# jorgeMFS/VCFX

Measured on AMD Instinct MI355X. Metric: variant-records/sec (and GB/s vs HBM roofline), 427K var × 2504 samp, higher is better.
Workload: dtype u8; 1 GPU; VCFX_allele_freq_calc -i (file path) on a device-resident 427409 x 2504 VCF shard per GPU: the walk (line ends + allele counts + rows composed in LDS) + the rows in file order; records_per_gpu=427409, samples=2504, bytes_per_gpu=4297544426, parallelism=record-sharded x1

## Files before the change

### include/vcfx_gpu.h

```cpp
#ifndef VCFX_GPU_H
#define VCFX_GPU_H
#include <stddef.h>
#include <stdint.h>

#ifdef __cplusplus
extern "C" {
#endif

typedef struct vcfxg_ctx vcfxg_ctx;

enum vcfxg_status {
    VCFXG_OK = 0,
    VCFXG_E_NODEV = -1,
    VCFXG_E_HIP = -2,
    VCFXG_E_ARG = -3,
    VCFXG_E_NOMEM = -4,
    VCFXG_E_STATE = -5,
    VCFXG_E_CAP = -6,
    VCFXG_E_DATA = -7
};

enum vcfxg_mode { VCFXG_MODE_FILE = 0, VCFXG_MODE_STDIN = 1 };

enum vcfxg_line_status {
    VCFXG_LINE_SKIP = 0,
    VCFXG_LINE_ROW = 1,
    VCFXG_LINE_DROP = 2,
    VCFXG_LINE_WARN = 3,
    VCFXG_LINE_HEADER = 4,
    VCFXG_LINE_RECHECK = 5
};

typedef struct {
    uint64_t n_lines;
    uint64_t rows;
    uint64_t data_lines;
    uint64_t warn_lines;
    uint64_t text_bytes;
    uint64_t general_records;
} vcfxg_summary;

const char *vcfxg_version(void);
int vcfxg_device_count(int *n);
int vcfxg_open(int device, vcfxg_ctx **out);
void vcfxg_close(vcfxg_ctx *ctx);
const char *vcfxg_last_error(const vcfxg_ctx *ctx);
void *vcfxg_stream(vcfxg_ctx *ctx);
int vcfxg_set_profiling(vcfxg_ctx *ctx, int enable);
int vcfxg_set_profiling_only(vcfxg_ctx *ctx, const char *kernel);
int vcfxg_kernel_ms(vcfxg_ctx *ctx, const char *kernel, float *ms);
int vcfxg_kernel_stats(vcfxg_ctx *ctx, const char *kernel, double *total_ms, uint64_t *launches);
int vcfxg_reset_kernel_stats(vcfxg_ctx *ctx);

int vcfxg_load_host(vcfxg_ctx *ctx, const char *host, size_t n);
int vcfxg_ingest_begin(vcfxg_ctx *ctx, size_t size_hint);
int vcfxg_ingest(vcfxg_ctx *ctx, const char *host, size_t n, int is_final_chunk);
int vcfxg_ingest_wait(vcfxg_ctx *ctx, size_t upto);
typedef struct {
    uint64_t src_off;
    uint32_t src_len;
    uint32_t out_len;
} vcfxg_bgzf_member;
int vcfxg_ingest_bgzf(vcfxg_ctx *ctx, const void *comp, size_t comp_n, const vcfxg_bgzf_member *members,
                      size_t n_members, const char *head, size_t head_n, uint64_t *bad_member);
int vcfxg_bgzf_stage(vcfxg_ctx *ctx, const void *host, size_t n, size_t offset, size_t comp_total);
int vcfxg_bgzf_inflate(vcfxg_ctx *ctx, const vcfxg_bgzf_member *members, size_t count);
uint64_t vcfxg_bgzf_handed_over(const vcfxg_ctx *ctx);
int vcfxg_host_alloc(vcfxg_ctx *ctx, size_t n, void **out);
void vcfxg_host_free(vcfxg_ctx *ctx, void *p);
int vcfxg_input_fetch(vcfxg_ctx *ctx, uint64_t offset, size_t n, void *host);
const void *vcfxg_input_device_ptr(vcfxg_ctx *ctx);

int vcfxg_index(vcfxg_ctx *ctx, size_t data_start, uint64_t *n_lines);
int vcfxg_line_ends(vcfxg_ctx *ctx, uint64_t first, uint64_t count, uint64_t *out);

int vcfxg_allele_freq(vcfxg_ctx *ctx, int mode, vcfxg_summary *out);
int vcfxg_allele_freq_region(vcfxg_ctx *ctx, size_t data_start, int mode, vcfxg_summary *out);
int vcfxg_genotype_query(vcfxg_ctx *ctx, const char *query, size_t qlen, int strict, int strip_cr,
                         vcfxg_summary *out);

typedef struct {
    int target;
    int op;
    int numeric;
    double value;
    const char *key;
    size_t key_len;
    const char *str;
    size_t str_len;
} vcfxg_criterion;

int vcfxg_record_filter(vcfxg_ctx *ctx, const vcfxg_criterion *crit, int n, int and_logic, vcfxg_summary *out);
#define VCFXG_RF_KEEP_CR 1
int vcfxg_record_filter_ex(vcfxg_ctx *ctx, const vcfxg_criterion *crit, int n, int and_logic, int flags,
                           vcfxg_summary *out);

int vcfxg_filter_query(vcfxg_ctx *ctx, const vcfxg_criterion *crit, int n, int and_logic, const char *query,
                       size_t qlen, int strict, vcfxg_summary *out);

int vcfxg_record_filter_region(vcfxg_ctx *ctx, size_t data_start, const vcfxg_criterion *crit, int n, int and_logic,
                               vcfxg_summary *out);
int vcfxg_genotype_query_region(vcfxg_ctx *ctx, size_t data_start, const char *query, size_t qlen, int strict,
                                int strip_cr, vcfxg_summary *out);
int vcfxg_filter_query_region(vcfxg_ctx *ctx, size_t data_start, const vcfxg_criterion *crit, int n, int and_logic,
                              const char *query, size_t qlen, int strict, vcfxg_summary *out);

int vcfxg_nonref_filter(vcfxg_ctx *ctx, int mode, vcfxg_summary *out);
int vcfxg_nonref_filter_region(vcfxg_ctx *ctx, size_t data_start, int mode, vcfxg_summary *out);

typedef struct {
    uint64_t text_offset;
    int32_t hom_ref, het, hom_alt;
    int32_t reserved;
} vcfxg_hwe_recheck;
int vcfxg_hwe_region(vcfxg_ctx *ctx, size_t data_start, int mode, vcfxg_summary *out);
int vcfxg_hwe_rechecks(vcfxg_ctx *ctx, vcfxg_hwe_recheck *out, uint64_t cap, uint64_t *n);

int vcfxg_dosage_region(vcfxg_ctx *ctx, size_t data_start, int mode, vcfxg_summary *out);

#define VCFXG_LINE_MISSING 6
int vcfxg_missing_region(vcfxg_ctx *ctx, size_t data_start, int mode, vcfxg_summary *out);

typedef struct {
    const uint32_t *sample;
    uint64_t m;
    const char *names;
    const uint64_t *name_off;
    int seq;
    int kind;
} vcfxg_ac_params;
int vcfxg_allele_counter(vcfxg_ctx *ctx, uint64_t first_line, uint64_t last_line, const vcfxg_ac_params *params,
                         vcfxg_summary *out);

typedef struct {
    uint32_t n_samples;
    const char *names;
    const uint64_t *name_off;
    int freq_mode;
    int skip_boundary;
    int count_boundary_as_used;
} vcfxg_ib_params;
int vcfxg_inbreeding_region(vcfxg_ctx *ctx, size_t data_start, int mode, const vcfxg_ib_params *params,
                            vcfxg_summary *out);
int vcfxg_inbreeding_samples(vcfxg_ctx *ctx, double *sum_exp, uint64_t *obs_het, uint64_t *used);

#define VCFXG_SX_EMPTY 0
#define VCFXG_SX_ROW 1
#define VCFXG_SX_SHORT 3
#define VCFXG_SX_HEADER 4
#define VCFXG_SX_NO_SAMPLES 5
#define VCFXG_SX_PRE 6
#define VCFXG_SX_CHROM 7
typedef struct {
    const uint32_t *cols;
    uint64_t m;
    int mode;
    int seen_chrom;
} vcfxg_sx_params;
int vcfxg_sample_extract(vcfxg_ctx *ctx, uint64_t first_line, uint64_t last_line, const vcfxg_sx_params *params,
                         vcfxg_summary *out);

#define VCFXG_MS_EMPTY 0
#define VCFXG_MS_COPY 1
#define VCFXG_MS_SPLIT 2
#define VCFXG_MS_HEADER 4
#define VCFXG_MS_INFO 0
#define VCFXG_MS_FORMAT 1
#define VCFXG_MS_NUM_OTHER 0
#define VCFXG_MS_NUM_A 1
#define VCFXG_MS_NUM_R 2
#define VCFXG_MS_NUM_G 3
#define VCFXG_MS_KEYS_LDS 32
#define VCFXG_MS_TABLE_LDS 16384
typedef struct {
    const char *id;
    uint32_t id_len;
    uint8_t section;
    uint8_t number;
} vcfxg_ms_entry;
typedef struct {
    const vcfxg_ms_entry *table;
    uint64_t n_entries;
    int mode;
} vcfxg_ms_params;
int vcfxg_multiallelic_split(vcfxg_ctx *ctx, uint64_t first_line, uint64_t last_line, const vcfxg_ms_params *params,
                             vcfxg_summary *out);
int vcfxg_ms_line_ranges(vcfxg_ctx *ctx, uint64_t first, uint64_t count, uint64_t *off);

#define VCFXG_FA_EMPTY 0
#define VCFXG_FA_COLUMN 1
#define VCFXG_FA_SKIPPED 3
#define VCFXG_FA_HEADER 4
#define VCFXG_FA_CHROM 7
#define VCFXG_FA_LINE 60
#define VCFXG_FA_TILE_SAMPLES 64
#define VCFXG_FA_TILE_COLUMNS 240
#define VCFXG_FA_TABLE 16
typedef struct {
    int mode;
    uint32_t n_samples;
    uint64_t first_col;
    uint64_t total_cols;
    const uint64_t *row_off;
    const uint64_t *skip;
} vcfxg_fa_params;
int vcfxg_fasta_scan(vcfxg_ctx *ctx, uint64_t first_line, uint64_t last_line, int mode, uint32_t n_samples,
                     vcfxg_summary *out);
int vcfxg_fasta_status(vcfxg_ctx *ctx, uint64_t first, uint64_t count, uint8_t *status, uint64_t *col);
int vcfxg_fasta_begin(vcfxg_ctx *ctx, uint64_t text_bytes);
int vcfxg_fasta(vcfxg_ctx *ctx, uint64_t first_line, uint64_t last_line, const vcfxg_fa_params *params,
                vcfxg_summary *out);

#define VCFXG_CC_CONCORDANT 1
#define VCFXG_CC_DISCORDANT 2
#define VCFXG_CC_NO_GENOTYPES 3
typedef struct {
    uint32_t n_samples;
    const uint32_t *mult;
    uint64_t n_mult;
    uint64_t threads;
} vcfxg_cc_params;
int vcfxg_concordance_region(vcfxg_ctx *ctx, size_t data_start, int mode, const vcfxg_cc_params *params,
                             vcfxg_summary *out);
int vcfxg_concordance_totals(const vcfxg_ctx *ctx, uint64_t totals[4]);
int vcfxg_chrom_lines(vcfxg_ctx *ctx, size_t data_start, uint64_t *starts, uint64_t cap, uint64_t *n);

#define VCFXG_DD_EMPTY 0
#define VCFXG_DD_KEPT 1
#define VCFXG_DD_DUP 2
#define VCFXG_DD_SHORT 3
#define VCFXG_DD_HEADER 4
#define VCFXG_DD_WINDOW 64
typedef struct {
    uint32_t hash_bits;
} vcfxg_dd_params;
int vcfxg_dedup(vcfxg_ctx *ctx, int mode, const vcfxg_dd_params *params, vcfxg_summary *out);
int vcfxg_dedup_status(vcfxg_ctx *ctx, uint64_t first, uint64_t count, uint8_t *status);
int vcfxg_dedup_counts(const vcfxg_ctx *ctx, uint64_t counts[6]);

#define VCFXG_SRT_EMPTY 0
#define VCFXG_SRT_KEPT 1
#define VCFXG_SRT_PRE 2
#define VCFXG_SRT_BAD 3
#define VCFXG_SRT_HEADER 4
#define VCFXG_SRT_WINDOW 64
typedef struct {
    int natural;
} vcfxg_srt_params;
int vcfxg_sort(vcfxg_ctx *ctx, int mode, const vcfxg_srt_params *params, vcfxg_summary *out);
int vcfxg_sort_status(vcfxg_ctx *ctx, uint64_t first, uint64_t count, uint8_t *status);
int vcfxg_sort_counts(const vcfxg_ctx *ctx, uint64_t counts[6]);
int vcfxg_sort_order(vcfxg_ctx *ctx, uint64_t first, uint64_t count, uint32_t *lines);
int vcfxg_sort_text(vcfxg_ctx *ctx, uint64_t first_out_line, uint64_t *lines_taken, uint64_t *bytes);

#define VCFXG_DF_EMPTY 0
#define VCFXG_DF_COMMON 1
#define VCFXG_DF_UNIQUE 2
#define VCFXG_DF_SKIPPED 3
#define VCFXG_DF_HEADER 4
#define VCFXG_DF_REPEAT 5
#define VCFXG_DF_WINDOW 64
#define VCFXG_DF_PATH_HASH 0
#define VCFXG_DF_PATH_BOUNDS 1
#define VCFXG_DF_PATH_WALK 2
typedef struct {
    uint64_t second_start;
    int assume_sorted;
    int natural;
    uint32_t hash_bits;
} vcfxg_df_params;
int vcfxg_diff(vcfxg_ctx *ctx, const vcfxg_df_params *params, vcfxg_summary *out);
int vcfxg_diff_status(vcfxg_ctx *ctx, uint64_t first, uint64_t count, uint8_t *status);
int vcfxg_diff_counts(const vcfxg_ctx *ctx, uint64_t counts[8]);
int vcfxg_diff_text(vcfxg_ctx *ctx, int side, uint64_t first_out, uint64_t *taken, uint64_t *bytes);

#define VCFXG_MG_EMPTY 0
#define VCFXG_MG_KEPT 1
#define VCFXG_MG_BAD 2
#define VCFXG_MG_HEADER 3
#define VCFXG_MG_DROPPED 4
#define VCFXG_MG_WINDOW 64
#define VCFXG_MG_PATH_SORT 0
#define VCFXG_MG_PATH_WALK 1
typedef struct {
    const uint64_t *file_start;
    uint32_t n_files;
    int assume_sorted;
    int natural;
} vcfxg_mg_params;
int vcfxg_merge(vcfxg_ctx *ctx, const vcfxg_mg_params *params, vcfxg_summary *out);
int vcfxg_merge_status(vcfxg_ctx *ctx, uint64_t first, uint64_t count, uint8_t *status);
int vcfxg_merge_counts(const vcfxg_ctx *ctx, uint64_t counts[8]);
int vcfxg_merge_files(vcfxg_ctx *ctx, uint64_t *first_line, uint64_t *bad);
int vcfxg_merge_order(vcfxg_ctx *ctx, uint64_t first, uint64_t count, uint32_t *lines);
int vcfxg_merge_text(vcfxg_ctx *ctx, uint64_t first_out_line, uint64_t *lines_taken, uint64_t *bytes);

int vcfxg_haplotype_phaser(vcfxg_ctx *ctx, size_t data_start, int mode, double threshold, uint32_t n_samples_hint,
                           vcfxg_summary *out);
int vcfxg_phaser_variants(vcfxg_ctx *ctx, uint8_t *flags, double *r2, uint64_t *entry_offsets);

int vcfxg_variant_count(vcfxg_ctx *ctx, int strip_cr, vcfxg_summary *out);

int vcfxg_ld_prepare(vcfxg_ctx *ctx, int n_samples, int id_dot_to_pos, const char *region_chrom, size_t region_len,
                     int has_region, int region_start, int region_end, int parse_mode, uint64_t *n_variants);
int vcfxg_ld_prepare_region(vcfxg_ctx *ctx, size_t data_start, int n_samples, int id_dot_to_pos,
                            const char *region_chrom, size_t region_len, int has_region, int region_start,
                            int region_end, int parse_mode, uint64_t *n_variants);
int vcfxg_ld_prefixes(vcfxg_ctx *ctx, char *text, size_t cap, uint64_t *offsets);
int vcfxg_ld_matrix(vcfxg_ctx *ctx, int gate, int printf4, uint64_t *cell_bytes);
int vcfxg_ld_stream_chunk(vcfxg_ctx *ctx, uint64_t j0, uint64_t j1, uint64_t window, double threshold, int max_dist,
                          uint64_t *n_pairs, uint64_t *text_bytes);
int vcfxg_ld_fetch_pairs(vcfxg_ctx *ctx, uint64_t first, uint64_t count, uint32_t *vi, uint32_t *vj, double *r2);
int vcfxg_selftest_mfma_i8(vcfxg_ctx *ctx, int *mismatches);
int vcfxg_selftest_mfma_fp4(vcfxg_ctx *ctx, int *mismatches);

int vcfxg_shard_cuts(const char *data, size_t n, size_t lo, int world, uint64_t *cuts);

typedef struct vcfxg_comm vcfxg_comm;
int vcfxg_comm_init(vcfxg_ctx *const *ctxs, int n, vcfxg_comm **out);
int vcfxg_comm_allreduce_u64(vcfxg_comm *comm, int rank, uint64_t *vals, size_t count);
int vcfxg_comm_uses_rccl(const vcfxg_comm *comm);
int vcfxg_comm_rccl_stats(vcfxg_comm *comm, uint64_t *calls, uint64_t *mismatches);
void vcfxg_comm_destroy(vcfxg_comm *comm);

int vcfxg_count_byte(vcfxg_ctx *ctx, uint64_t from, int byte, uint64_t *count);
const char *vcfxg_last_schedule(const vcfxg_ctx *ctx);
int vcfxg_last_af_depth(const vcfxg_ctx *ctx, int *rolling);

int vcfxg_fetch_text(vcfxg_ctx *ctx, char *host, size_t cap);
int vcfxg_fetch_text_range(vcfxg_ctx *ctx, uint64_t offset, size_t n, void *host);
int vcfxg_fetch_lines(vcfxg_ctx *ctx, uint64_t first, uint64_t count, int32_t *alt, int32_t *total,
                      uint8_t *status);

#ifdef __cplusplus
}
#endif
#endif
```

### vcfx_amd/csrc/gpu/vcfxg_af_walk.hip

```cpp
#include <algorithm>
#include <type_traits>

#include "vcfxg_af_walk_kernel.h"

namespace vcfxg {

#ifndef VCFXG_COMPACT_SUB
#define VCFXG_COMPACT_SUB 4
#endif
constexpr int kCompactSub = VCFXG_COMPACT_SUB, kCompactLanes = kWave / kCompactSub;
__global__ __launch_bounds__(256) void k_walk_compact(int64_t n_walkers, uint64_t cap_w,
                                                      const uint64_t *__restrict__ offs,
                                                      const uint32_t *__restrict__ wgt,
                                                      const uint64_t *__restrict__ le_b,
                                                      const int32_t *__restrict__ alt_b,
                                                      const int32_t *__restrict__ tot_b,
                                                      const int32_t *__restrict__ aux_b,
                                                      const uint32_t *__restrict__ rowpre_b,
                                                      const uint8_t *__restrict__ status_b,
                                                      const LineMeta *__restrict__ meta_b, uint64_t *line_end,
                                                      int32_t *alt, int32_t *tot, int32_t *aux, uint32_t *rowpre,
                                                      uint8_t *status, LineMeta *meta, uint64_t *n_lines,
                                                      unsigned long long *counters, const uint64_t *__restrict__ bpre) {
    __shared__ uint32_t red[256 / kWave];
    uint32_t g = 0;
    const int64_t nwaves = (int64_t)gridDim.x * (256 / kWave);
    const int sub = lane() / kCompactLanes, sl = lane() % kCompactLanes;
    for (int64_t w0 = ((int64_t)blockIdx.x * (256 / kWave) + threadIdx.x / kWave) * kCompactSub; w0 < n_walkers;
         w0 += nwaves * kCompactSub) {
        const int64_t w = w0 + sub;
        if (w >= n_walkers) continue;
        const uint64_t d0 = offs[w] + (bpre ? bpre[w / kWalkerScanBlock] : 0),
                       cnt = offs[w + 1] + (bpre ? bpre[(w + 1) / kWalkerScanBlock] : 0) - d0, s0 = (uint64_t)w * cap_w;
        g += sl == 0 ? (wgt[w] & 0xFFFFu) : 0u;
        for (uint64_t i = sl; i < cnt; i += kCompactLanes) {
            const uint64_t sl = s0 + i, d = d0 + i;
            line_end[d] = le_b[sl];
            alt[d] = alt_b[sl];
            tot[d] = tot_b[sl];
            if (aux_b) aux[d] = aux_b[sl];
            rowpre[d] = rowpre_b[sl];
            status[d] = status_b[sl];
            meta[d] = meta_b[sl];
        }
    }
    g = wave_sum(g);
    if (lane() == 0) red[threadIdx.x / kWave] = g;
    __syncthreads();
    if (threadIdx.x == 0) {
        uint32_t t = 0;
        for (int k = 0; k < 256 / kWave; k++) t += red[k];
        if (t) {
            atomicAdd(&counters[0], (unsigned long long)t);
            atomicAdd(&counters[1], (unsigned long long)t);
        }
        if (blockIdx.x == 0) *n_lines = offs[n_walkers] + (bpre ? bpre[n_walkers / kWalkerScanBlock] : 0);
    }
}

int64_t af_walkers(int64_t lo, int64_t hi, int64_t chunk) { return hi > lo ? (hi - lo + chunk - 1) / chunk : 0; }

hipError_t launch_af_walk(const char *buf, int64_t lo, int64_t hi, int64_t chunk, int mode, int64_t span0,
                          uint64_t cap_w, uint64_t *le_b, int32_t *alt_b, int32_t *tot_b, uint32_t *rowpre_b,
                          uint8_t *status_b, void *meta_b, uint64_t *wcount, uint32_t *wgt, unsigned *overflow,
                          hipStream_t s, int32_t *hwe_aux_b, const WalkTail *tail, bool dose, bool gt_first_walk,
                          bool dose_head, int depth, bool roll) {
    const WalkTail t = tail ? *tail : WalkTail{};
    const int64_t nw = af_walkers(lo, hi, chunk);
    if (!nw) return hipErrorInvalidValue;
    const bool af_gt_only = !gt_first_walk && !dose && !hwe_aux_b;
    if (roll ? !(af_gt_only && af_depth_compiled(depth)) : depth != kWalkUnroll) return hipErrorInvalidValue;
    const unsigned grid = (unsigned)((nw + kWalkWaves - 1) / kWalkWaves);
    if (gt_first_walk)
        hipLaunchKernelGGL(HIP_KERNEL_NAME(k_af_walk<AfOp, true>), dim3(grid), dim3(kWalkThreads), 0, s, buf, lo, hi,
                           chunk, nw, mode, span0, cap_w, le_b, alt_b, tot_b, nullptr, rowpre_b, status_b,
                           static_cast<LineMeta *>(meta_b), wcount, wgt, overflow, t);
    else if (dose && dose_head)
        hipLaunchKernelGGL(k_af_walk<DoseHeadOp>, dim3(grid), dim3(kWalkThreads), 0, s, buf, lo, hi, chunk, nw, mode,
                           span0, cap_w, le_b, alt_b, tot_b, nullptr, rowpre_b, status_b, static_cast<LineMeta *>(meta_b),
                           wcount, wgt, overflow, t);
    else if (dose)
        hipLaunchKernelGGL(k_af_walk<DoseWalkOp>, dim3(grid), dim3(kWalkThreads), 0, s, buf, lo, hi, chunk, nw, mode,
                           span0, cap_w, le_b, alt_b, tot_b, nullptr, rowpre_b, status_b, static_cast<LineMeta *>(meta_b),
                           wcount, wgt, overflow, t);
    else if (hwe_aux_b)
        hipLaunchKernelGGL(k_af_walk<HweOp>, dim3(grid), dim3(kWalkThreads), 0, s, buf, lo, hi, chunk, nw, mode, span0,
                           cap_w, le_b, alt_b, tot_b, hwe_aux_b, rowpre_b, status_b, static_cast<LineMeta *>(meta_b),
                           wcount, wgt, overflow, t);
    else {
        auto go = [&](auto kernel) {
            hipLaunchKernelGGL(kernel, dim3(grid), dim3(kWalkThreads), 0, s, buf, lo, hi, chunk, nw, mode, span0, cap_w,
                               le_b, alt_b, tot_b, nullptr, rowpre_b, status_b, static_cast<LineMeta *>(meta_b), wcount,
                               wgt, overflow, t);
        };
        if (!roll) go(k_af_walk<AfOp>);
        else if (depth == 6) go(k_af_walk<AfOp, false, 6, true>);
        else if (depth == 8) go(k_af_walk<AfOp, false, 8, true>);
        else if (depth == 10) go(k_af_walk<AfOp, false, 10, true>);
        else go(k_af_walk<AfOp, false, 12, true>);
    }
    return hipGetLastError();
}

hipError_t launch_walk_compact(int64_t n_walkers, uint64_t cap_w, const uint64_t *offs, const uint32_t *wgt,
                               const uint64_t *le_b, const int32_t *alt_b, const int32_t *tot_b,
                               const uint32_t *rowpre_b, const uint8_t *status_b, const void *meta_b,
                               uint64_t *line_end, int32_t *alt, int32_t *tot, uint32_t *rowpre, uint8_t *status,
                               void *meta, uint64_t *n_lines, unsigned long long *counters, hipStream_t s,
                               const int32_t *aux_b, int32_t *aux, const uint64_t *bpre) {
    const int64_t blocks = std::min<int64_t>((n_walkers + 256 / kWave - 1) / (256 / kWave), 512);
    hipLaunchKernelGGL(k_walk_compact, dim3((unsigned)std::max<int64_t>(blocks, 1)), dim3(256), 0, s, n_walkers, cap_w,
                       offs, wgt, le_b, alt_b, tot_b, aux_b, rowpre_b, status_b, static_cast<const LineMeta *>(meta_b),
                       line_end, alt, tot, aux, rowpre, status, static_cast<LineMeta *>(meta), n_lines, counters, bpre);
    return hipGetLastError();
}

}
```

### vcfx_amd/csrc/gpu/vcfxg_af_walk_kernel.h

```cpp
#pragma once
#include <algorithm>
#include <type_traits>

#include "vcfxg_device.h"
#include "vcfxg_gt.h"
#include "vcfxg_kernels.h"
#include "vcfxg_walk.h"

namespace vcfxg {

#ifndef VCFXG_WALK_UNROLL
#define VCFXG_WALK_UNROLL 6
#endif
constexpr int kWalkUnroll = VCFXG_WALK_UNROLL;
static_assert(kWalkUnroll == kAfDepthDefault, "launch_af_walk's default depth is the batch walks' unroll");
static_assert(kAfWaveStep == kWaveStep, "the host plan's wave-step");
#ifndef VCFXG_HWE_UNROLL
#define VCFXG_HWE_UNROLL 5
#endif
constexpr int kHweUnroll = VCFXG_HWE_UNROLL;
#ifndef VCFXG_CC_UNROLL
#define VCFXG_CC_UNROLL 4
#endif
constexpr int kCcUnroll = VCFXG_CC_UNROLL;
#ifndef VCFXG_GF_FLAGS
#define VCFXG_GF_FLAGS 1
#endif
constexpr bool kGfFlags = VCFXG_GF_FLAGS != 0;
#ifndef VCFXG_GF_UNROLL
#define VCFXG_GF_UNROLL 4
#endif
constexpr int kGfUnroll = VCFXG_GF_UNROLL;
#ifndef VCFXG_AF_XREC
#define VCFXG_AF_XREC 0
#endif
#ifndef VCFXG_AF_EXPT
#define VCFXG_AF_EXPT 0
#endif
#ifndef VCFXG_AF_EARLY
#define VCFXG_AF_EARLY 0
#endif
#define VCFXG_STR2(x) #x
#define VCFXG_STR(x) VCFXG_STR2(x)

template <class Op>
struct WalkRed;
template <>
struct WalkRed<AfOp> {
    static constexpr bool kAux = false;
    __device__ static AfOp make(const char *buf, int64_t ae) { return AfOp{buf, ae, 0}; }
    __device__ static void out(const AfOp &op, uint32_t &a, uint32_t &b, uint32_t &) {
        a = op.alt;
        b = op.tot;
    }
};
template <>
struct WalkRed<HweOp> {
    static constexpr bool kAux = true;
    __device__ static HweOp make(const char *buf, int64_t ae) { return HweOp{buf, ae}; }
    __device__ static void out(const HweOp &op, uint32_t &a, uint32_t &b, uint32_t &c) {
        a = op.c0;
        b = op.c1;
        c = op.c2;
    }
};

template <>
struct WalkRed<CcOp> {
    static constexpr bool kAux = false;
    __device__ static CcOp make(const char *, int64_t) { return CcOp{}; }
    __device__ static void out(const CcOp &op, uint32_t &a, uint32_t &b, uint32_t &) {
        a = op.N;
        b = op.U;
    }
};

template <>
struct WalkRed<DoseWalkOp> {
    static constexpr bool kAux = false;
    __device__ static DoseWalkOp make(const char *buf, int64_t ae) { return DoseWalkOp{buf, ae}; }
    __device__ static void out(const DoseWalkOp &op, uint32_t &a, uint32_t &b, uint32_t &) {
        a = op.ns;
        b = op.na;
    }
};

template <>
struct WalkRed<DoseHeadOp> : WalkRed<DoseWalkOp> {
    __device__ static DoseHeadOp make(const char *buf, int64_t ae) { return DoseHeadOp{{buf, ae}}; }
};

#ifndef VCFXG_AF_MINW
#define VCFXG_AF_MINW 5
#endif
#ifndef VCFXG_AF_DEEP_MINW
#define VCFXG_AF_DEEP_MINW 4
#endif
constexpr int af_walk_waves(bool gf, int depth) { return gf ? 4 : depth >= 10 ? VCFXG_AF_DEEP_MINW : VCFXG_AF_MINW; }
template <class Op, bool kGF = false, int kDepth = kWalkUnroll, bool kRoll = false>
__global__ __launch_bounds__(kWalkThreads)
#ifdef VCFXG_WALK_MAXW
__attribute__((amdgpu_waves_per_eu(1, VCFXG_WALK_MAXW)))
#else
__attribute__((amdgpu_waves_per_eu(af_walk_waves(kGF, kDepth))))
#endif
void k_af_walk(const char *__restrict__ buf, int64_t lo, int64_t hi, int64_t chunk, int64_t n_walkers, int mode,
               int64_t span0, uint64_t cap_w, uint64_t *__restrict__ le_o, int32_t *__restrict__ alt_o,
               int32_t *__restrict__ tot_o, int32_t *__restrict__ aux_o, uint32_t *__restrict__ rowpre_o,
               uint8_t *__restrict__ status_o, LineMeta *__restrict__ meta_o, uint64_t *__restrict__ wcount,
               uint32_t *__restrict__ wgt, unsigned *overflow, WalkTail tail) {
    typedef WalkRed<Op> R;
    constexpr bool kCc = std::is_same<Op, CcOp>::value;
    static_assert((kDepth == kWalkUnroll && !kRoll) || (std::is_same<Op, AfOp>::value && !kGF),
                  "k_af_walk: a depth of its own for the AF GT-only walk alone");
    static_assert((kDepth == kWalkUnroll && !kRoll) || !(VCFXG_AF_XREC || VCFXG_AF_EARLY),
                  "k_af_walk: the carried / early loads are batch-path experiments at kWalkUnroll");
    __shared__ uint4 win[kWalkWaves][2][kWave];
    constexpr bool kStageLds = std::is_same<Op, AfOp>::value;
    constexpr uint32_t kStgCap = kStageLds ? 2048u : 16u;
    __shared__ __attribute__((aligned(16))) char stg[kStageLds ? kWalkWaves : 1][kStgCap];
    const int wv = threadIdx.x / kWave;
    const int64_t wk = uniform64((int64_t)walk_block() * kWalkWaves + wv);
    if (wk >= n_walkers) return;
    const int strip_cr = mode == 0 ? 1 : 0;
    const int64_t cs = lo + wk * chunk;
    const int64_t ce = std::min<int64_t>(cs + chunk, hi);
    int64_t L, ce2;
    walker_lines(buf, lo, hi, cs, ce, L, ce2, chunk);
    const int64_t L0 = L;
    uint64_t wtext = 0;
    int64_t span = span0;
    uint8_t cr_prev = 0;
    uint64_t n = 0;
    uint32_t ngt = 0, ngf = 0;
    bool dirty = false;
    const uint64_t base = (uint64_t)wk * cap_w;
    uint64_t r_le = 0, r_S = 0;
    uint32_t r_alt = 0, r_tot = 0, r_aux = 0, r_pre = 0, r_k = 0;
    uint32_t r_h = 0;
    auto flush = [&](uint64_t first, uint32_t cnt) {
        if ((uint32_t)lane() < cnt) {
            const uint64_t o = base + first + lane();
            const uint8_t kind = (uint8_t)r_k;
            LineMeta m{};
            m.kind = kind;
            m.cr = (uint8_t)(r_k >> 16);
            m.pad = (R::kAux || kCc || std::is_same<Op, DoseHeadOp>::value) ? (uint8_t)r_h : 0;
            if (kind == kMetaGt) {
                m.S = r_S;
                m.rowpre = r_pre;
                m.sep = (uint8_t)(r_k >> 8);
            }
            le_o[o] = r_le;
            alt_o[o] = (int32_t)r_alt;
            tot_o[o] = (int32_t)r_tot;
            if (R::kAux) aux_o[o] = (int32_t)r_aux;
            rowpre_o[o] = kind == kMetaGt ? r_pre : 0u;
            status_o[o] = (uint8_t)(r_k >> 24);
            meta_o[o] = m;
        }
    };
    constexpr bool kXrec = VCFXG_AF_XREC && std::is_same<Op, AfOp>::value && !kGF;
    uint4 xv[kXrec ? kWalkUnroll : 1];
    int64_t xvb = -1;
    int cur = 0;
    int64_t A = L & ~(int64_t)15;
    if (L < ce2) prefetch_window(buf, A, hi, win[wv][cur]);
    constexpr bool kEarly = VCFXG_AF_EARLY && std::is_same<Op, AfOp>::value && !kGF && !kXrec;
    uint4 ev[kEarly ? kWalkUnroll : 1];
    const int64_t hlast = (hi - 1) & ~(int64_t)15;
    while (L < ce2) {
        if (n >= cap_w) {
            if (lane() == 0) atomicOr(overflow, 1u);
            break;
        }
        if constexpr (kEarly) {
#pragma unroll
            for (int u = 0; u < kWalkUnroll; u++) {
                const int64_t g = A + u * kWaveStep + kBlockBytes * lane();
                ev[u] = load16(buf, g < hi ? g : hlast);
            }
        }
        int64_t eA = kEarly ? A : -1;
        const int Lr = (int)(L - A);
        const uint4 *cw = win[wv][cur];
        int hr, N1r, r3 = 0, r4 = 0, r7 = 0, r8 = 0;
        uint32_t ntab, first, hflags = 0;
        auto take = [&](const int(&rt)[9], bool comma) {
            r4 = rt[4];
            r7 = rt[7];
            r8 = rt[8];
            if (R::kAux) {
                const bool empty = rt[0] == Lr || rt[1] == rt[0] + 1 || r4 == rt[3] + 1;
                hflags = (comma ? kHweAltComma : 0u) | (empty ? kHweEmptyField : 0u);
            }
            if (kCc) {
                r3 = rt[3];
                hflags = rt[0] == Lr ? kCcEmptyChrom : 0u;
            }
        };
        uint32_t w4 = 0;
        bool long_head = false;
        {
            if constexpr (kEarly) asm volatile("s_waitcnt vmcnt(" VCFXG_STR(VCFXG_WALK_UNROLL) ")" ::: "memory");
            else asm volatile("s_waitcnt vmcnt(0)" ::: "memory");
            w4 = reinterpret_cast<const uint32_t *>(cw)[lane()];
            hr = (int)std::min<int64_t>(hi - A, kWin);
            const uint32_t rg = range4(Lr, hr);
            N1r = first_match<4>(zero_bytes(w4 ^ kRepNl) & rg);
            int rt[9] = {};
            ntab = first_tabs<4>(zero_bytes(w4 ^ kRepTab) & rg, N1r >= 0 ? N1r : hr, rt);
            first = dword_byte(w4, Lr);
            if (ntab >= 9) take(rt, R::kAux && __ballot((zero_bytes(w4 ^ 0x2C2C2C2Cu) & range4(rt[3] + 1, rt[4])) != 0u));
        }
        if (N1r < 0 && ntab < 9 && first != '#' && hr == kWin) {
            prefetch_window(buf, A, hi, win[wv][cur], kWaveStep);
            long_head = true;
            const uint4 W = read_window(cw);
            const int b = 16 * lane();
            hr = (int)std::min<int64_t>(hi - A, kWaveStep);
            N1r = first_match<16>(eq_mask16(W, kRepNl) & range16(b, Lr, hr));
            int rt[9] = {};
            ntab = first_tabs<16>(eq_mask16(W, kRepTab) & range16(b, Lr, hr), N1r >= 0 ? N1r : hr, rt);
            if (ntab >= 9) take(rt, R::kAux && __ballot((eq_mask16(W, 0x2C2C2C2Cu) & range16(b, rt[3] + 1, rt[4])) != 0u));
        }
        auto wbyte = [&](int o) { return long_head ? slot_byte(cw, o) : dword_byte(w4, o); };
        const int64_t wend = A + hr;
        int64_t t4 = -1, t8 = -1;
        bool gt_head = false, gt_only = false;
        if (ntab >= 9 && first != '#') {
            t4 = A + r4;
            t8 = A + r8;
            if (r8 - r7 >= 3 && wbyte(r7 + 1) == 'G' && wbyte(r7 + 2) == 'T') {
                gt_only = r8 - r7 == 3;
                gt_head = gt_only || wbyte(r7 + 3) == ':';
            }
        }
        uint32_t cc_max = 0;
        if constexpr (kCc) {
            const int as = r3 + 1;
            if (gt_head && r4 > as && wbyte(as) != '.') {
                cc_max = 1;
                if (r4 - as > 1) {
                    const uint32_t cm = long_head ? eq_mask16(cw[lane()], 0x2C2C2C2Cu) & range16(16 * lane(), as, r4)
                                                  : zero_bytes(w4 ^ 0x2C2C2C2Cu) & range4(as, r4);
                    cc_max += wave_sum32((uint32_t)__popc(cm));
                }
            }
        }
        int64_t E;
        uint8_t cr = 0;
        bool predicted = false;
        const bool gf = kGF && N1r < 0 && gt_head && !gt_only;
        if (N1r >= 0) {
            E = A + N1r;
            cr = strip_cr && E > L && wbyte(N1r - 1) == '\r';
        } else if (gf) {
            E = hi;
        } else if (gt_only && span > 0 && t8 + 1 + span <= hi) {
            E = t8 + 1 + span;
            cr = cr_prev;
            predicted = true;
        } else {
            E = scan_nl(buf, wend, hi);
            cr = strip_cr && E > L && __builtin_amdgcn_readfirstlane(byte_at(buf, E - 1)) == '\r';
        }
        const uint32_t sep_w = gt_head && t8 + 2 < wend ? wbyte((int)(t8 + 2 - A)) : 0u;
        const int nxt = cur ^ 1;
        int64_t An = std::max<int64_t>(E - 1, 0) & ~(int64_t)15;
        bool pending = true;
        auto pre = [&]() {
            prefetch_window(buf, An, hi, win[wv][nxt]);
            pending = false;
        };
        uint8_t st = 0, kind = 0, sep = 0;
        uint32_t alt = 0, tot = 0, aux = 0, rowpre = 0;
        int64_t S = 0;
        bool ok = false;
        bool skip = std::is_same<Op, DoseHeadOp>::value && predicted;
        int64_t xuse = xvb;
        xvb = -1;
        auto sweep = [&]() {
            if constexpr (kGF) {
              if (gf) {
                S = t8 + 1;
                Op op = R::make(buf, hi);
                int64_t Eo = hi;
                uint8_t cro = 0;
                auto pre_e = [&](int64_t e) {
                    An = std::max<int64_t>(e - 1, 0) & ~(int64_t)15;
                    pre();
                };
                if constexpr (std::is_same<Op, AfOp>::value && kGfFlags)
                    ok = gt_first_af<kGfUnroll>(buf, S, hi, strip_cr, op, pre_e, Eo, cro);
                else
                    ok = gt_first<kWalkUnroll>(buf, S, hi, strip_cr, op, pre_e, Eo, cro);
                E = Eo;
                cr = cro;
                const int64_t ae = E - cr;
                kind = t8 < ae ? kMetaGt : kMetaFull;
                ok = ok && kind == kMetaGt;
                if (kind == kMetaGt) {
                    rowpre = (uint32_t)(t4 - L + 1);
                    sep = t8 + 2 >= ae ? 0
                          : t8 + 2 < wend ? (uint8_t)sep_w
                                          : (uint8_t)__builtin_amdgcn_readfirstlane(byte_at(buf, t8 + 2));
                    R::out(op, alt, tot, aux);
                }
                return;
              }
            }
            const int64_t ae = E - cr;
            if (ae <= L) kind = kMetaEmpty;
            else if (first == '#') kind = kMetaHeader;
            else if (gt_head && t8 < ae) kind = kMetaGt;
            else kind = kMetaFull;
            ok = false;
            if (kind == kMetaGt) {
                S = t8 + 1;
                rowpre = (uint32_t)(t4 - L + 1);
                sep = t8 + 2 >= ae ? 0
                      : t8 + 2 < wend ? (uint8_t)sep_w
                                      : (uint8_t)__builtin_amdgcn_readfirstlane(byte_at(buf, t8 + 2));
                Op op = R::make(buf, ae);
                if constexpr (kCc) op.max_allele = cc_max;
                if constexpr (kXrec) {
                    const int64_t use = xuse >= 0 && xuse <= S ? xuse : -1;
                    xuse = -1;
                    const int64_t nb = E + 1 < ce2 ? (E + 1) & ~(int64_t)15 : -1;
                    int64_t vbo;
                    ok = af_fixed_x<kWalkUnroll>(buf, S, ae, hi, op, sep, pre, xv, use, nb, vbo);
                    xvb = vbo;
                } else if constexpr (kEarly) {
                    const bool mine = eA >= 0 && eA <= S;
                    ok = af_fixed<kWalkUnroll>(buf, S, ae, op, sep, pre, mine ? ev : nullptr, mine ? eA : -1);
                    eA = -1;
                } else if constexpr (std::is_same<Op, AfOp>::value)
                    ok = af_fixed < kGF ? kGfUnroll : kDepth, kRoll > (buf, S, ae, op, sep, pre);
                else if constexpr (std::is_same<Op, DoseHeadOp>::value) {
                    if (skip) {
                        ok = (sep == '/' || sep == '|') && ae - S >= 3 && ((ae - S + 1) & 3) == 0;
                        op.ns = ok ? (uint32_t)((ae - S + 1) >> 2) : 0u;
                        op.na = 0;
                    } else {
                        ok = gt_fast<kWalkUnroll>(buf, S, ae, op, sep, pre);
                    }
                } else ok = gt_fast < std::is_same<Op, HweOp>::value ? kHweUnroll : kCc ? kCcUnroll : kWalkUnroll > (buf, S, ae, op, sep, pre);
                R::out(op, alt, tot, aux);
            }
        };
        sweep();
        if (pending) pre();
        if (predicted) {
            const uint4 *nw = win[wv][nxt];
            asm volatile("s_waitcnt vmcnt(0)" ::: "memory");
            const uint32_t be = slot_byte(nw, (int)(E - An)), be1 = slot_byte(nw, (int)(E - 1 - An));
            const bool endok = (E < hi ? be == '\n' : true) && ((strip_cr && be1 == '\r') == (cr != 0));
            if (!(ok && endok)) {
                const int64_t Et = scan_nl(buf, wend, hi);
                if (Et != E || !endok) {
                    skip = false;
                    E = Et;
                    cr = strip_cr && E > L && __builtin_amdgcn_readfirstlane(byte_at(buf, E - 1)) == '\r';
                    An = std::max<int64_t>(E - 1, 0) & ~(int64_t)15;
                    pending = true;
                    sweep();
                    if (pending) pre();
                }
            }
        }
        if constexpr (std::is_same<Op, DoseHeadOp>::value)
            if (skip && kind == kMetaGt) hflags |= kWalkUnswept;
        if (kind == kMetaGt) {
            if (ok) {
                st = 1;
                span = E - S;
                cr_prev = cr;
            } else {
                st = kAfPending;
            }
        }
        if ((uint32_t)lane() == (uint32_t)(n & 63)) {
            r_le = (uint64_t)E;
            r_S = (uint64_t)S;
            r_alt = alt;
            r_tot = tot;
            r_aux = aux;
            r_h = hflags;
            r_pre = rowpre;
            r_k = (uint32_t)kind | ((uint32_t)sep << 8) | ((uint32_t)cr << 16) | ((uint32_t)st << 24);
        }
        if constexpr (std::is_same<Op, AfOp>::value) {
            if (tail.stage && !(VCFXG_AF_EXPT & 1)) {
                if (kind == kMetaGt && ok && wtext + rowpre + 7u <= std::min<uint32_t>(tail.stage_cap, kStgCap)) {
                    uint32_t flo = 0x30303030u, fhi = 0x0A3030u;
                    if (!(VCFXG_AF_EXPT & 2)) af_freq_text(mode, (int32_t)alt, (int32_t)tot, flo, fhi);
                    auto *dst = reinterpret_cast<__attribute__((address_space(3))) char *>(
                                    reinterpret_cast<__attribute__((address_space(3))) char *>(
                                        (__attribute__((address_space(3))) void *)stg[kStageLds ? wv : 0])) +
                                wtext;
                    const unsigned char *src = reinterpret_cast<const unsigned char *>(cw) + (L - A);
                    for (uint32_t j0 = 0; j0 < rowpre + 7u; j0 += kWave) {
                        const uint32_t j = j0 + (uint32_t)lane();
                        if (j < rowpre) dst[j] = (char)src[j];
                        else if (j < rowpre + 7u) {
                            const uint32_t q = j - rowpre;
                            dst[j] = (char)((q < 4u ? flo >> (8u * q) : fhi >> (8u * (q - 4u))) & 0xFFu);
                        }
                    }
                } else if (kind == kMetaGt || kind == kMetaFull) {
                    dirty = true;
                }
            }
        }
        ngt += kind == kMetaGt ? 1u : 0u;
        if constexpr (kGF) ngf += gf && kind == kMetaGt && ok ? 1u : 0u;
        if (tail.wtext) {
            if (kind == kMetaGt) wtext += (uint64_t)rowpre + 7u;
            if (kind == kMetaFull || (kind == kMetaGt && !ok)) {
                if (lane() == 0) {
                    const unsigned long long e = atomicAdd(tail.cx_n, 1ull);
                    if (e < tail.cx_cap) tail.cx_list[e] = base + n;
                }
            }
        }
        n++;
        if ((n & 63) == 0) flush(n - 64, 64);
        L = E + 1;
        A = An;
        cur = nxt;
    }
// ... 25 lines not shown
```

### vcfx_amd/csrc/gpu/vcfxg_api.hip

```cpp
#include <hip/hip_runtime.h>
#include <hipcub/hipcub.hpp>

#include <fcntl.h>
#include <unistd.h>

#include "vcfxg_ctx.h"
#include "vcfxg_ld.h"

namespace vcfxg {

int fail(vcfxg_ctx *c, hipError_t e, const char *what) {
    if (c) {
        c->err = std::string(what) + ": " + hipGetErrorString(e);
    }
    return e == hipErrorOutOfMemory ? VCFXG_E_NOMEM : VCFXG_E_HIP;
}

int ensure(vcfxg_ctx *c, DevBuf &b, size_t bytes) {
    if (bytes <= b.cap) return VCFXG_OK;
    size_t nc = bytes < 4096 ? 4096 : bytes + bytes / 8;
    if (b.p) {
        HIPCHK(c, hipStreamSynchronize(c->stream));
        HIPCHK(c, hipFree(b.p));
        b.p = nullptr;
// ... 249 lines not shown
int vcfxg_load_host(vcfxg_ctx *c, const char *host, size_t n) {
    if (!c || (!host && n)) return VCFXG_E_ARG;
    int r = vcfxg_ingest_begin(c, n);
    if (!r) r = vcfxg_ingest(c, host, n, 1);
    return r;
}

int vcfxg_ingest_begin(vcfxg_ctx *c, size_t size_hint) {
    if (c) c->dense_pending = false;
    if (!c) return VCFXG_E_ARG;
    HIPCHK(c, hipSetDevice(c->device));
    if (c->copy_stream) HIPCHK(c, hipStreamSynchronize(c->copy_stream));
    for (int k = 0; k < vcfxg_ctx::kBgzStreams; k++)
        if (c->bgz_stream[k]) HIPCHK(c, hipStreamSynchronize(c->bgz_stream[k]));
    if (c->bgz_side.aux) HIPCHK(c, hipStreamSynchronize(c->bgz_side.aux));
    c->bgz_total = c->bgz_staged = 0;
    size_t fr = 0, tot = 0;
    if (hipMemGetInfo(&fr, &tot) == hipSuccess && size_hint > (fr + c->input.cap) / 2)
        size_hint = (fr + c->input.cap) / 2;
    int r = ensure(c, c->input, size_hint + kPad);
    if (r) return r;
    c->loaded = false;
    c->indexed = false;
    c->n = 0;
    c->ingesting = true;
    reset_hints(c);
    c->hints_pending = true;
    return VCFXG_OK;
}

static int ingest_mark(vcfxg_ctx *c, size_t upto);

int vcfxg_ingest(vcfxg_ctx *c, const char *host, size_t n, int is_final_chunk) {
    if (!c || (!host && n)) return VCFXG_E_ARG;
    if (!c->ingesting) return VCFXG_E_STATE;
    HIPCHK(c, hipSetDevice(c->device));
    if (c->n + n + kPad > c->input.cap) {
        size_t nc = std::max(c->input.cap * 2, c->n + n + kPad);
        void *np = nullptr;
        HIPCHK(c, hipMalloc(&np, nc));
        if (c->n) HIPCHK(c, hipMemcpyAsync(np, c->input.p, c->n, hipMemcpyDeviceToDevice, c->stream));
        HIPCHK(c, hipStreamSynchronize(c->stream));
        HIPCHK(c, hipFree(c->input.p));
        c->input.p = np;
        c->input.cap = nc;
    }
    if (n) HIPCHK(c, hipMemcpyAsync(static_cast<char *>(c->input.p) + c->n, host, n, hipMemcpyHostToDevice, c->stream));
    if (n && !is_final_chunk) {
        int r = ingest_mark(c, c->n + n);
        if (r) return r;
    }
    if (n && c->hints_pending) c->hints_pending = !load_hints(c, host, n);
    c->n += n;
    if (n) c->last_byte = (unsigned char)host[n - 1];
    if (!is_final_chunk) return VCFXG_OK;
    if (!c->n) c->last_byte = -1;
    HIPCHK(c, hipMemsetAsync(static_cast<char *>(c->input.p) + c->n, 0, kPad, c->stream));
    HIPCHK(c, hipStreamSynchronize(c->stream));
    for (auto &pe : c->ingest_ev) c->ingest_ev_free.push_back(pe.second);
    c->ingest_ev.clear();
    c->hints_pending = false;
    c->ingesting = false;
    c->loaded = true;
    c->indexed = false;
    return VCFXG_OK;
}

static int ingest_mark(vcfxg_ctx *c, size_t upto) {
    hipEvent_t e = nullptr;
    if (!c->ingest_ev_free.empty()) {
        e = c->ingest_ev_free.back();
        c->ingest_ev_free.pop_back();
    } else {
        HIPCHK(c, hipEventCreateWithFlags(&e, hipEventDisableTiming));
    }
    HIPCHK(c, hipEventRecord(e, c->stream));
    c->ingest_ev.push_back({upto, e});
    return VCFXG_OK;
}

int vcfxg_ingest_wait(vcfxg_ctx *c, size_t upto) {
    if (!c) return VCFXG_E_ARG;
    size_t k = 0;
    while (k < c->ingest_ev.size() && c->ingest_ev[k].first <= upto) k++;
    if (k == 0) return VCFXG_OK;
    HIPCHK(c, hipEventSynchronize(c->ingest_ev[k - 1].second));
    for (size_t i = 0; i < k; i++) c->ingest_ev_free.push_back(c->ingest_ev[i].second);
    c->ingest_ev.erase(c->ingest_ev.begin(), c->ingest_ev.begin() + (long)k);
    return VCFXG_OK;
}

int vcfxg_count_byte(vcfxg_ctx *c, uint64_t from, int byte, uint64_t *count) {
    if (!c || !count || byte < 0 || byte > 255) return VCFXG_E_ARG;
    if (!c->loaded) return VCFXG_E_STATE;
    HIPCHK(c, hipSetDevice(c->device));
    *count = 0;
    if (from >= c->n) return VCFXG_OK;
    int r = ensure(c, c->byte_cnt, 8);
    if (r) return r;
    HIPCHK(c, hipMemsetAsync(c->byte_cnt.p, 0, 8, c->stream));
    prof_begin(c, "count_byte");
    HIPCHK(c, vcfxg::launch_count_byte(P<uint8_t>(c->input), from, c->n, (uint8_t)byte,
                                       P<unsigned long long>(c->byte_cnt), c->stream));
    prof_end(c, "count_byte");
    static thread_local uint64_t h;
    HIPCHK(c, hipMemcpyAsync(&h, c->byte_cnt.p, 8, hipMemcpyDeviceToHost, c->stream));
    HIPCHK(c, hipStreamSynchronize(c->stream));
    prof_collect(c);
    *count = h;
    return VCFXG_OK;
}

int vcfxg_host_alloc(vcfxg_ctx *c, size_t n, void **out) {
    if (!c || !out) return VCFXG_E_ARG;
    *out = nullptr;
    HIPCHK(c, hipSetDevice(c->device));
    HIPCHK(c, hipHostMalloc(out, n ? n : 1, hipHostMallocDefault));
    return VCFXG_OK;
}

void vcfxg_host_free(vcfxg_ctx *c, void *p) {
    if (c && p) (void)hipHostFree(p);
}

int vcfxg_input_fetch(vcfxg_ctx *c, uint64_t offset, size_t n, void *host) {
    if (!c || (!host && n)) return VCFXG_E_ARG;
    if (!c->loaded) return VCFXG_E_STATE;
    if (offset > c->n || n > c->n - offset) return VCFXG_E_ARG;
    if (!n) return VCFXG_OK;
    HIPCHK(c, hipSetDevice(c->device));
    HIPCHK(c, hipMemcpyAsync(host, static_cast<const char *>(c->input.p) + offset, n, hipMemcpyDeviceToHost, c->stream));
    HIPCHK(c, hipStreamSynchronize(c->stream));
    return VCFXG_OK;
}

const void *vcfxg_input_device_ptr(vcfxg_ctx *c) { return c && c->loaded ? c->input.p : nullptr; }

int vcfxg_index(vcfxg_ctx *c, size_t data_start, uint64_t *n_lines) {
    if (c) c->dense_pending = false;
    if (!c) return VCFXG_E_ARG;
    c->dd_done = false;
    c->srt_done = false;
    c->df_done = false;
    c->mg_done = false;
    c->ms_done = false;
    c->fa_scanned = c->fa_begun = false;
    if (!c->loaded) return VCFXG_E_STATE;
    if (data_start > c->n) data_start = c->n;
    HIPCHK(c, hipSetDevice(c->device));
    const int64_t lo = (int64_t)data_start, hi = (int64_t)c->n;
    const int64_t nc = vcfxg::idx_wchunks(lo, hi);
    int r = ensure(c, c->idx_counts, sizeof(uint32_t) * (size_t)(nc + 1));
    if (!r) r = ensure(c, c->idx_offs, sizeof(uint64_t) * (size_t)(nc + 1));
    if (!r) r = ensure(c, c->idx_pos, sizeof(uint64_t) * (size_t)nc * vcfxg::idx_pos_cap() + 64);
    if (r) return r;
    const char *buf = P<char>(c->input);
    unsigned *overflow = reinterpret_cast<unsigned *>(P<uint64_t>(c->idx_pos) + (size_t)nc * vcfxg::idx_pos_cap());
    HIPCHK(c, hipMemsetAsync(overflow, 0, 8, c->stream));
    prof_begin(c, "line_count");
    HIPCHK(c, vcfxg::launch_idx_count(buf, lo, hi, P<uint32_t>(c->idx_counts), P<uint64_t>(c->idx_pos), overflow,
                                      c->stream));
    prof_end(c, "line_count");
    HIPCHK(c, hipMemsetAsync(P<uint32_t>(c->idx_counts) + nc, 0, sizeof(uint32_t), c->stream));
    r = exclusive_scan(c, P<uint32_t>(c->idx_counts), P<uint64_t>(c->idx_offs), (size_t)nc + 1);
    if (r) return r;
    static thread_local uint64_t total;
    static thread_local unsigned ovf;
    HIPCHK(c, hipMemcpyAsync(&total, P<uint64_t>(c->idx_offs) + nc, sizeof total, hipMemcpyDeviceToHost, c->stream));
    HIPCHK(c, hipMemcpyAsync(&ovf, overflow, sizeof ovf, hipMemcpyDeviceToHost, c->stream));
    HIPCHK(c, hipStreamSynchronize(c->stream));
    const bool tail = hi > lo && c->last_byte != '\n';
    const uint64_t nl = total + (tail ? 1 : 0);
    r = ensure(c, c->line_end, sizeof(uint64_t) * (size_t)(nl + 1));
    if (r) return r;
    if (ovf) {
        prof_begin(c, "line_emit");
        HIPCHK(c, vcfxg::launch_idx_emit(buf, lo, hi, P<uint64_t>(c->idx_offs), P<uint64_t>(c->line_end), c->stream));
        prof_end(c, "line_emit");
    } else {
        prof_begin(c, "line_compact");
        HIPCHK(c, vcfxg::launch_nl_compact(lo, hi, P<uint32_t>(c->idx_counts), P<uint64_t>(c->idx_offs),
                                           P<uint64_t>(c->idx_pos), P<uint64_t>(c->line_end), c->stream));
        prof_end(c, "line_compact");
    }
    static thread_local uint64_t tail_end, nl_host;
    tail_end = (uint64_t)hi;
    nl_host = nl;
    if (tail)
        HIPCHK(c, hipMemcpyAsync(P<uint64_t>(c->line_end) + total, &tail_end, sizeof(uint64_t), hipMemcpyHostToDevice,
                                 c->stream));
    HIPCHK(c, hipMemcpyAsync(c->d_nlines.p, &nl_host, sizeof(uint64_t), hipMemcpyHostToDevice, c->stream));
    HIPCHK(c, hipStreamSynchronize(c->stream));
    prof_collect(c);
    c->data_start = data_start;
    c->n_lines = nl;
    c->indexed = true;
    if (n_lines) *n_lines = nl;
    return VCFXG_OK;
}

int vcfxg_line_ends(vcfxg_ctx *c, uint64_t first, uint64_t count, uint64_t *out) {
    if (!c || (!out && count)) return VCFXG_E_ARG;
    if (!c->indexed) return VCFXG_E_STATE;
    DENSE(c);
    if (first + count > c->n_lines) return VCFXG_E_ARG;
    if (!count) return VCFXG_OK;
    HIPCHK(c, hipMemcpyAsync(out, P<uint64_t>(c->line_end) + first, count * sizeof(uint64_t), hipMemcpyDeviceToHost,
                             c->stream));
    HIPCHK(c, hipStreamSynchronize(c->stream));
    return VCFXG_OK;
}

int vcfxg_selftest_mfma_i8(vcfxg_ctx *c, int *mismatches) {
    if (!c || !mismatches) return VCFXG_E_ARG;
    HIPCHK(c, hipSetDevice(c->device));
    std::vector<int8_t> A(32 * 32), B(32 * 32);
    for (int i = 0; i < 32 * 32; i++) {
        A[i] = (int8_t)((i * 7 + 3) % 5 - 2);
        B[i] = (int8_t)((i * 11 + 1) % 7 - 3);
    }
    int r = ensure(c, c->scan_tmp, 8192);
    if (r) return r;
    char *d = P<char>(c->scan_tmp);
    HIPCHK(c, hipMemcpyAsync(d, A.data(), 1024, hipMemcpyHostToDevice, c->stream));
    HIPCHK(c, hipMemcpyAsync(d + 1024, B.data(), 1024, hipMemcpyHostToDevice, c->stream));
    HIPCHK(c, vcfxg::launch_mfma_i8_selftest((int8_t *)d, (int8_t *)(d + 1024), (int *)(d + 2048), c->stream));
    std::vector<int> C(32 * 32);
    HIPCHK(c, hipMemcpyAsync(C.data(), d + 2048, 4096, hipMemcpyDeviceToHost, c->stream));
    HIPCHK(c, hipStreamSynchronize(c->stream));
    int bad = 0;
    for (int i = 0; i < 32; i++)
        for (int j = 0; j < 32; j++) {
            int s = 0;
            for (int k = 0; k < 32; k++) s += A[i * 32 + k] * B[j * 32 + k];
            bad += s != C[i * 32 + j];
        }
    *mismatches = bad;
    return VCFXG_OK;
}

int vcfxg_selftest_mfma_fp4(vcfxg_ctx *c, int *mismatches) {
    if (!c || !mismatches) return VCFXG_E_ARG;
    HIPCHK(c, hipSetDevice(c->device));
    std::vector<int> A(32 * 64), B(32 * 64);
    for (int i = 0; i < 32 * 64; i++) {
        A[i] = (i * 7 + 3) % 3;
        B[i] = (i * 11 + i / 64 + 1) % 3;
    }
    std::vector<uint8_t> Ap(1024), Bp(1024);
    for (int i = 0; i < 1024; i++) {
        Ap[i] = (uint8_t)((2 * A[2 * i]) | ((2 * A[2 * i + 1]) << 4));
        Bp[i] = (uint8_t)((2 * B[2 * i]) | ((2 * B[2 * i + 1]) << 4));
    }
    int r = ensure(c, c->scan_tmp, 8192);
    if (r) return r;
    char *d = P<char>(c->scan_tmp);
    HIPCHK(c, hipMemcpyAsync(d, Ap.data(), 1024, hipMemcpyHostToDevice, c->stream));
    HIPCHK(c, hipMemcpyAsync(d + 1024, Bp.data(), 1024, hipMemcpyHostToDevice, c->stream));
    HIPCHK(c, vcfxg::launch_mfma_f4_selftest((uint8_t *)d, (uint8_t *)(d + 1024), (float *)(d + 2048), c->stream));
    std::vector<float> C(32 * 32);
    HIPCHK(c, hipMemcpyAsync(C.data(), d + 2048, 4096, hipMemcpyDeviceToHost, c->stream));
    HIPCHK(c, hipStreamSynchronize(c->stream));
    int bad = 0;
    for (int i = 0; i < 32; i++)
        for (int j = 0; j < 32; j++) {
            int sum = 0;
            for (int k = 0; k < 64; k++) sum += A[i * 64 + k] * B[j * 64 + k];
            bad += (float)sum != C[i * 32 + j];
        }
    *mismatches = bad;
    return VCFXG_OK;
}

int vcfxg_fetch_text(vcfxg_ctx *c, char *host, size_t cap) {
    if (!c || (!host && c->text_bytes)) return VCFXG_E_ARG;
    if (cap < c->text_bytes) return VCFXG_E_CAP;
    if (!c->text_bytes) return VCFXG_OK;
    HIPCHK(c, hipMemcpyAsync(host, c->text.p, c->text_bytes, hipMemcpyDeviceToHost, c->stream));
    HIPCHK(c, hipStreamSynchronize(c->stream));
    return VCFXG_OK;
}

int vcfxg_shard_cuts(const char *data, size_t n, size_t lo, int world, uint64_t *cuts) {
    if ((!data && n) || world < 1 || !cuts || lo > n) return VCFXG_E_ARG;
    cuts[0] = lo;
    for (int i = 1; i < world; i++) {
        size_t p = lo + (size_t)((unsigned __int128)(n - lo) * (unsigned)i / (unsigned)world);
        if (p < cuts[i - 1]) p = cuts[i - 1];
        if (p > lo && p < n && data[p - 1] != '\n') {
            const void *nl = memchr(data + p, '\n', n - p);
            p = nl ? (size_t)((const char *)nl - data) + 1 : n;
        }
        cuts[i] = p < n ? p : n;
    }
    cuts[world] = n;
    return VCFXG_OK;
}

const char *vcfxg_last_schedule(const vcfxg_ctx *c) { return c ? c->last_schedule : ""; }
int vcfxg_last_af_depth(const vcfxg_ctx *c, int *rolling) {
    if (rolling) *rolling = c && c->last_af_roll ? 1 : 0;
    return c ? c->last_af_depth : 0;
}
uint64_t vcfxg_bgzf_handed_over(const vcfxg_ctx *c) { return c ? c->bgz_handed : 0; }

int vcfxg_fetch_text_range(vcfxg_ctx *c, uint64_t offset, size_t n, void *host) {
    if (!c || (!host && n)) return VCFXG_E_ARG;
    if (offset > c->text_bytes || n > c->text_bytes - offset) return VCFXG_E_ARG;
    if (!n) return VCFXG_OK;
    HIPCHK(c, hipMemcpyAsync(host, P<char>(c->text) + offset, n, hipMemcpyDeviceToHost, c->stream));
    HIPCHK(c, hipStreamSynchronize(c->stream));
    return VCFXG_OK;
}

int vcfxg_fetch_lines(vcfxg_ctx *c, uint64_t first, uint64_t count, int32_t *alt, int32_t *total, uint8_t *status) {
    if (!c) return VCFXG_E_ARG;
    if (!c->indexed) return VCFXG_E_STATE;
    DENSE(c);
    if (first + count > c->n_lines) return VCFXG_E_ARG;
    if (!count) return VCFXG_OK;
    if (alt) HIPCHK(c, hipMemcpyAsync(alt, P<int32_t>(c->alt) + first, 4 * count, hipMemcpyDeviceToHost, c->stream));
    if (total) HIPCHK(c, hipMemcpyAsync(total, P<int32_t>(c->tot) + first, 4 * count, hipMemcpyDeviceToHost, c->stream));
    if (status) HIPCHK(c, hipMemcpyAsync(status, P<uint8_t>(c->status) + first, count, hipMemcpyDeviceToHost, c->stream));
    HIPCHK(c, hipStreamSynchronize(c->stream));
    return VCFXG_OK;
}

}
```

### vcfx_amd/csrc/gpu/vcfxg_api_af.hip

```cpp
#include "vcfxg_ctx.h"

namespace vcfxg {

int ensure_dense(vcfxg_ctx *c) {
    if (!c->dense_pending) return VCFXG_OK;
    c->dense_pending = false;
    const uint64_t L = c->n_lines;
    int r = dense_buffers(c, L);
    if (!r) r = ensure(c, c->scratch_small, 64);
    if (r) return r;
    return walk_compact(c, c->dense_nw, c->dense_cap_w, P<unsigned long long>(c->scratch_small), false,
                        P<uint64_t>(c->wk_bs));
}

}

using namespace vcfxg;

extern "C" {

static int af_rows(vcfxg_ctx *c, int mode, vcfxg_summary *out);

int vcfxg_allele_freq(vcfxg_ctx *c, int mode, vcfxg_summary *out) {
    if (!c || (mode != VCFXG_MODE_FILE && mode != VCFXG_MODE_STDIN)) return VCFXG_E_ARG;
    if (!c->indexed) return VCFXG_E_STATE;
    DENSE(c);
    HIPCHK(c, hipSetDevice(c->device));
    const uint64_t L = c->n_lines;
    int r = af_buffers(c, L);
    if (r) return r;
    const char *buf = P<char>(c->input);
    const uint64_t *nl_dev = P<uint64_t>(c->d_nlines);
    HIPCHK(c, hipMemsetAsync(c->counters.p, 0, 64, c->stream));
    r = ensure(c, c->af_meta, vcfxg::af_meta_bytes() * (L + 1));
    if (r) return r;
    prof_begin(c, "af_records");
    HIPCHK(c, vcfxg::launch_af_meta_sweep(buf, (int64_t)c->data_start, P<uint64_t>(c->line_end), nl_dev, L, mode,
                                          c->af_meta.p, P<int32_t>(c->alt), P<int32_t>(c->tot), P<uint32_t>(c->rowpre),
                                          P<uint8_t>(c->status), P<unsigned long long>(c->counters), c->stream));
    prof_end(c, "af_records");
    return af_rows(c, mode, out);
}


static int af_region_async(vcfxg_ctx *c, size_t data_start, int mode, vcfxg_summary *out) {
    if (c) c->dense_pending = false;
    HIPCHK(c, hipSetDevice(c->device));
    const int64_t lo = (int64_t)data_start, hi = (int64_t)c->n;
    const int64_t nc = vcfxg::idx_wchunks(lo, hi);
    if (!nc) {
        int r = vcfxg_index(c, data_start, nullptr);
        return r ? r : vcfxg_allele_freq(c, mode, out);
    }
    const size_t pcap = (size_t)vcfxg::idx_pos_cap();
    const uint64_t bound = (uint64_t)nc * pcap + 2;
    const uint64_t cap = c->af_line_cap ? std::min<uint64_t>(c->af_line_cap + 1, bound) : bound;
    int r = ensure(c, c->idx_counts, sizeof(uint32_t) * (size_t)(nc + 1));
    if (!r) r = ensure(c, c->idx_offs, sizeof(uint64_t) * (size_t)(nc + 1));
    if (!r) r = ensure(c, c->idx_pos, sizeof(uint64_t) * (size_t)nc * pcap + 64);
    if (!r) r = ensure(c, c->line_end, 8 * (cap + 1));
    if (!r) r = af_buffers(c, cap);
    if (!r) r = ensure(c, c->af_meta, vcfxg::af_meta_bytes() * (cap + 1));
    if (!r) r = ensure(c, c->async_small, 128);
    if (r) return r;
    const char *buf = P<char>(c->input);
    uint64_t *small = P<uint64_t>(c->async_small);
    unsigned *idx_ovf = reinterpret_cast<unsigned *>(small + 2), *failf = idx_ovf + 1;
    HIPCHK(c, hipMemsetAsync(small, 0, 32, c->stream));
    HIPCHK(c, hipMemsetAsync(c->counters.p, 0, 64, c->stream));
    prof_begin(c, "line_count");
    HIPCHK(c, vcfxg::launch_idx_count(buf, lo, hi, P<uint32_t>(c->idx_counts), P<uint64_t>(c->idx_pos), idx_ovf,
                                      c->stream));
    prof_end(c, "line_count");
    HIPCHK(c, hipMemsetAsync(P<uint32_t>(c->idx_counts) + nc, 0, sizeof(uint32_t), c->stream));
    r = exclusive_scan(c, P<uint32_t>(c->idx_counts), P<uint64_t>(c->idx_offs), (size_t)nc + 1);
    if (r) return r;
    prof_begin(c, "line_compact");
    HIPCHK(c, vcfxg::launch_nl_compact_cap(lo, hi, P<uint32_t>(c->idx_counts), P<uint64_t>(c->idx_offs),
                                           P<uint64_t>(c->idx_pos), P<uint64_t>(c->line_end), cap, c->stream));
    HIPCHK(c, vcfxg::launch_idx_finish(P<uint64_t>(c->idx_offs), nc, idx_ovf, c->last_byte != '\n' ? 1 : 0, hi, cap,
                                       P<uint64_t>(c->line_end), small + 1, failf, c->stream));
    HIPCHK(c, hipMemcpyAsync(c->d_nlines.p, small + 1, 8, hipMemcpyDeviceToDevice, c->stream));
    prof_end(c, "line_compact");
    prof_begin(c, "af_records");
    HIPCHK(c, vcfxg::launch_af_meta_sweep_range(buf, lo, P<uint64_t>(c->line_end), small, cap, mode, c->af_meta.p,
                                                P<int32_t>(c->alt), P<int32_t>(c->tot), P<uint32_t>(c->rowpre),
                                                P<uint8_t>(c->status), P<unsigned long long>(c->counters), c->stream));
    HIPCHK(c, vcfxg::launch_af_complex(buf, lo, P<uint64_t>(c->line_end), P<uint64_t>(c->d_nlines), cap, mode,
                                       c->af_meta.p, P<int32_t>(c->alt), P<int32_t>(c->tot), P<uint32_t>(c->rowpre),
                                       P<uint8_t>(c->status), P<unsigned long long>(c->counters), c->stream));
    prof_end(c, "af_records");
    prof_begin(c, "af_rows");
    HIPCHK(c, vcfxg::launch_af_rowlen(P<uint32_t>(c->rowpre), P<uint8_t>(c->status), P<uint64_t>(c->d_nlines), cap,
                                      P<uint64_t>(c->rowlen), c->stream));
    r = exclusive_scan(c, P<uint64_t>(c->rowlen), P<uint64_t>(c->rowoff), (size_t)cap + 1);
    if (r) return r;
    HIPCHK(c, vcfxg::launch_af_summary(P<uint64_t>(c->d_nlines), P<uint64_t>(c->rowoff),
                                       P<unsigned long long>(c->counters), failf, small + 4, c->stream));
    prof_end(c, "af_rows");
    static thread_local uint64_t sm[7];
    HIPCHK(c, hipMemcpyAsync(sm, small + 4, sizeof sm, hipMemcpyDeviceToHost, c->stream));
    HIPCHK(c, hipStreamSynchronize(c->stream));
    if (sm[6]) {
        prof_collect(c);
        c->af_line_cap = 0;
        r = vcfxg_index(c, data_start, nullptr);
        if (!r) r = vcfxg_allele_freq(c, mode, out);
        if (!r) c->af_line_cap = c->n_lines;
        return r;
    }
    const uint64_t L = sm[0], text = sm[1];
    c->af_line_cap = std::max<uint64_t>(c->af_line_cap, L);
    r = ensure(c, c->text, text + 1);
    if (r) return r;
    prof_begin(c, "af_format");
    HIPCHK(c, vcfxg::launch_af_format(buf, lo, P<uint64_t>(c->line_end), P<uint64_t>(c->d_nlines), L, mode,
                                      P<int32_t>(c->alt), P<int32_t>(c->tot), P<uint32_t>(c->rowpre),
                                      P<uint8_t>(c->status), P<uint64_t>(c->rowoff), P<char>(c->text), c->stream));
    prof_end(c, "af_format");
    prof_collect(c);
    c->data_start = data_start;
    c->n_lines = L;
    c->indexed = true;
    c->text_bytes = text;
    if (out) {
        out->n_lines = L;
        out->rows = sm[2];
        out->data_lines = sm[3];
        out->warn_lines = sm[4];
        out->general_records = sm[5];
        out->text_bytes = text;
    }
    return VCFXG_OK;
}

static int af_region_walk(vcfxg_ctx *c, size_t data_start, int mode, vcfxg_summary *out, bool gf = false) {
    if (c) c->dense_pending = false;
    HIPCHK(c, hipSetDevice(c->device));
    const WalkPlan pl = walk_plan(c, data_start);
    const int64_t lo = pl.lo, hi = pl.hi, C = pl.C, nw = pl.nw;
    if (!nw) {
        int r = vcfxg_index(c, data_start, nullptr);
        return r ? r : vcfxg_allele_freq(c, mode, out);
    }
    const uint64_t cap_w = pl.cap_w, cap = pl.cap;
    if (!pl.fits_gt16) {
        c->walk_overflowed = true;
        return note_schedule(c, "af_two_sweep"), af_region_async(c, data_start, mode, out);
    }
    int r = walk_buffers(c, pl);
    if (!r) r = ensure(c, c->wk_text, 8 * (size_t)(nw + 1));
    if (!r) r = ensure(c, c->wk_toff, 8 * (size_t)(nw + 1));
    if (!r) r = ensure(c, c->wk_start, 8 * (size_t)(nw + 1));
    if (!r) r = ensure(c, c->wk_cx, 8 * cap);
    const int64_t nbs = (nw + vcfxg::kWalkerScanBlock - 1) / vcfxg::kWalkerScanBlock;
    if (!r) r = ensure(c, c->wk_bs, 8 * (size_t)(5 * nbs + 4));
    if (!r) r = ensure(c, c->af_small, 128);
    constexpr uint32_t kStageCap = 2048;
    if (!r) r = ensure(c, c->wk_stage, (size_t)kStageCap * (size_t)nw);
    if (!r) r = ensure(c, c->wk_dirty, (size_t)nw);
    if (r) return r;
    r = ensure_sum_host(c);
    if (r) return r;
    const char *buf = P<char>(c->input);
    uint64_t *bpre_a = P<uint64_t>(c->wk_bs), *bpre_b = bpre_a + nbs + 1, *bsum = bpre_b + nbs + 1;
    uint64_t *small = P<uint64_t>(c->af_small);
    unsigned *ovf = reinterpret_cast<unsigned *>(small);
    unsigned long long *cx_n = reinterpret_cast<unsigned long long *>(small + 1);
    unsigned long long *cnt = reinterpret_cast<unsigned long long *>(small + 2);
    if (c->af_small_dirty) HIPCHK(c, hipMemsetAsync(small, 0, 128, c->stream));
    c->af_small_dirty = true;
    vcfxg::WalkTail tail;
    tail.wtext = P<uint64_t>(c->wk_text);
    tail.wstart = P<uint64_t>(c->wk_start);
    tail.cx_list = P<uint64_t>(c->wk_cx);
    tail.cx_n = cx_n;
    tail.cx_cap = cap;
    tail.stage = P<char>(c->wk_stage);
    tail.stage_cap = kStageCap;
    tail.wdirty = P<uint8_t>(c->wk_dirty);
    const int depth = gf ? vcfxg::kAfDepthDefault : pl.af_depth;
    const bool roll = !gf && pl.af_roll;
    if (!gf) c->last_af_depth = depth, c->last_af_roll = roll;
    prof_begin(c, "af_walk");
    HIPCHK(c, vcfxg::launch_af_walk(buf, lo, hi, C, mode, c->hint_span, cap_w, P<uint64_t>(c->wk_le),
                                    P<int32_t>(c->wk_alt), P<int32_t>(c->wk_tot), P<uint32_t>(c->wk_rowpre),
                                    P<uint8_t>(c->wk_status), c->wk_meta.p, P<uint64_t>(c->wk_count),
                                    P<uint32_t>(c->wk_gt), ovf, c->stream, nullptr, &tail, false, gf, false, depth,
                                    roll));
    prof_end(c, "af_walk");
    prof_begin(c, "af_complex");
    const uint64_t cx_grid_lines = std::min<uint64_t>(cap, std::max<uint64_t>(c->cx_hint, 64));
    HIPCHK(c, vcfxg::launch_af_cx(buf, mode, cap_w, tail.cx_list, cx_n, cap, cx_grid_lines, tail.wstart,
                                  P<uint64_t>(c->wk_le), c->wk_meta.p, P<int32_t>(c->wk_alt), P<int32_t>(c->wk_tot),
                                  P<uint32_t>(c->wk_rowpre), P<uint8_t>(c->wk_status), tail.wtext, cnt, c->stream));
    prof_end(c, "af_complex");
    prof_begin(c, "af_rows");
    uint64_t *sm = c->sum_host;
    HIPCHK(c, vcfxg::launch_walker_scan(nw, P<uint64_t>(c->wk_count), tail.wtext, P<uint32_t>(c->wk_gt),
                                        P<uint64_t>(c->wk_offs), P<uint64_t>(c->wk_toff), bpre_a, bpre_b, bsum,
                                        reinterpret_cast<unsigned *>(small + 6), cnt, ovf, P<uint64_t>(c->d_nlines),
                                        c->sum_dev, c->stream, small));
    prof_end(c, "af_rows");
    const uint64_t tcap = std::max<uint64_t>(c->text_hint, 1u << 16);
    r = ensure(c, c->text, tcap + 1);
    if (r) return r;
    prof_begin(c, "af_format");
    HIPCHK(c, vcfxg::launch_af_format_w(buf, mode, nw, cap_w, P<uint64_t>(c->wk_count), P<uint64_t>(c->wk_toff),
                                        bpre_b, tail.wstart, P<uint64_t>(c->wk_le), P<int32_t>(c->wk_alt),
                                        P<int32_t>(c->wk_tot), P<uint32_t>(c->wk_rowpre), P<uint8_t>(c->wk_status),
                                        P<char>(c->text), tcap, c->stream, &tail));
    prof_end(c, "af_format");
    HIPCHK(c, hipStreamSynchronize(c->stream));
    c->af_small_dirty = false;
    c->cx_hint = sm[7];
    if (sm[6]) {
        prof_collect(c);
        c->walk_overflowed = true;
        return af_region_async(c, data_start, mode, out);
    }
    const uint64_t L = sm[0], text = sm[1];
    c->text_hint = text;
    if (text > tcap) {
        r = ensure(c, c->text, text + 1);
        if (r) return r;
        prof_begin(c, "af_format");
        HIPCHK(c, vcfxg::launch_af_format_w(buf, mode, nw, cap_w, P<uint64_t>(c->wk_count), P<uint64_t>(c->wk_toff),
                                            bpre_b, tail.wstart, P<uint64_t>(c->wk_le), P<int32_t>(c->wk_alt),
                                            P<int32_t>(c->wk_tot), P<uint32_t>(c->wk_rowpre),
                                            P<uint8_t>(c->wk_status), P<char>(c->text), ~0ull, c->stream, &tail));
        prof_end(c, "af_format");
    }
    prof_collect(c);
    c->data_start = data_start;
    c->n_lines = L;
    c->indexed = true;
    c->text_bytes = text;
    c->dense_nw = nw;
    c->dense_cap_w = cap_w;
    c->dense_pending = true;
    if (out) {
        out->n_lines = L;
        out->rows = sm[2];
        out->data_lines = sm[3];
        out->warn_lines = sm[4];
        out->general_records = sm[5];
        out->text_bytes = text;
    }
    return VCFXG_OK;
}

int vcfxg_allele_freq_region(vcfxg_ctx *c, size_t data_start, int mode, vcfxg_summary *out) {
    if (!c || (mode != VCFXG_MODE_FILE && mode != VCFXG_MODE_STDIN)) return VCFXG_E_ARG;
    if (!c->loaded) return VCFXG_E_STATE;
    if (data_start > c->n) data_start = c->n;
    if (c->af_path == 7) return note_schedule(c, "af_walk"), af_region_walk(c, data_start, mode, out);
    if (c->af_path == 8) return note_schedule(c, "af_two_sweep"), af_region_async(c, data_start, mode, out);
    if (c->af_path == 3) {
        note_schedule(c, "af_two_sweep_sync");
        int r = vcfxg_index(c, data_start, nullptr);
        return r ? r : vcfxg_allele_freq(c, mode, out);
    }
    if (walk_wanted(c, true))
        return note_schedule(c, "af_walk"), af_region_walk(c, data_start, mode, out);
    static const bool gf_ok = [] {
        const char *e = getenv("VCFXG_AF_GF_WALK");
        return !(e && e[0] == '0');
    }();
    if (gf_ok && c->hint_gt_first && walk_wanted(c, false))
        return note_schedule(c, "af_walk_gt_first"), af_region_walk(c, data_start, mode, out, true);
    return note_schedule(c, "af_two_sweep"), af_region_async(c, data_start, mode, out);
}

static int af_rows(vcfxg_ctx *c, int mode, vcfxg_summary *out) {
    const uint64_t L = c->n_lines;
    const char *buf = P<char>(c->input);
    const uint64_t *nl_dev = P<uint64_t>(c->d_nlines);
    int r;
    prof_begin(c, "af_rows");
    HIPCHK(c, vcfxg::launch_af_rowlen(P<uint32_t>(c->rowpre), P<uint8_t>(c->status), nl_dev, L, P<uint64_t>(c->rowlen),
                                      c->stream));
    HIPCHK(c, hipMemsetAsync(P<uint64_t>(c->rowlen) + L, 0, 8, c->stream));
    r = exclusive_scan(c, P<uint64_t>(c->rowlen), P<uint64_t>(c->rowoff), (size_t)L + 1);
    if (r) return r;
    prof_end(c, "af_rows");
    static thread_local uint64_t host_tail[5];
    HIPCHK(c, hipMemcpyAsync(&host_tail[0], P<uint64_t>(c->rowoff) + L, 8, hipMemcpyDeviceToHost, c->stream));
    HIPCHK(c, hipMemcpyAsync(&host_tail[1], c->counters.p, 32, hipMemcpyDeviceToHost, c->stream));
    HIPCHK(c, hipStreamSynchronize(c->stream));
    const uint64_t text = host_tail[0];
    r = ensure(c, c->text, text + 1);
    if (r) return r;
    prof_begin(c, "af_format");
    HIPCHK(c, vcfxg::launch_af_format(buf, (int64_t)c->data_start, P<uint64_t>(c->line_end), nl_dev, L, mode,
                                      P<int32_t>(c->alt), P<int32_t>(c->tot), P<uint32_t>(c->rowpre),
                                      P<uint8_t>(c->status), P<uint64_t>(c->rowoff), P<char>(c->text), c->stream));
    prof_end(c, "af_format");
    HIPCHK(c, hipStreamSynchronize(c->stream));
    prof_collect(c);
    c->text_bytes = text;
    if (out) {
        out->n_lines = L;
        out->rows = host_tail[1];
        out->data_lines = host_tail[2];
        out->warn_lines = host_tail[3];
        out->general_records = host_tail[4];
        out->text_bytes = text;
    }
    return VCFXG_OK;
}

}
```

### vcfx_amd/csrc/gpu/vcfxg_api_walk.hip

```cpp
#include "vcfxg_ctx.h"

#ifndef VCFXG_AF_DEPTH_LIVE
#define VCFXG_AF_DEPTH_LIVE 0
#endif

namespace vcfxg {

WalkPlan walk_plan(const vcfxg_ctx *c, size_t data_start, int64_t chunk) {
    WalkPlan p;
    p.lo = (int64_t)data_start;
    p.hi = (int64_t)c->n;
    p.C = chunk ? chunk : c->walk_chunk;
    p.nw = af_walkers(p.lo, p.hi, p.C);
    p.cap_w = (uint64_t)(2 * p.C / std::max<int64_t>(c->hint_line, 64)) + 16;
    p.cap = (uint64_t)p.nw * p.cap_w;
    p.fits_gt16 = p.cap_w <= 0xFFFF;
    int knob = c->af_depth_knob;
#if VCFXG_AF_DEPTH_LIVE
    knob = getenv("VCFXG_AF_DEPTH") ? atoi(getenv("VCFXG_AF_DEPTH")) : 0;
#endif
    af_sweep_plan(c->hint_span, knob, p.af_depth, p.af_roll);
    return p;
}

static constexpr int kMeasuredDepth[kAfDepthMax + 1] = {0, 0, 0, 0, 0, 0, 0, 0, 0, 0, 10, 0, 0};
void af_sweep_plan(int64_t span, int knob, int &depth, bool &roll) {
    depth = kAfDepthDefault;
    roll = false;
#if VCFXG_AF_DEPTH_LIVE
    if (knob == 1) return;
#endif
    if (af_depth_compiled(knob)) {
        depth = knob;
        roll = true;
        return;
    }
    if (span <= 0) return;
    const int64_t steps = (span + 15 + kAfWaveStep - 1) / kAfWaveStep;
    if (steps <= kAfDepthMax && af_depth_compiled(kMeasuredDepth[steps])) {
        depth = kMeasuredDepth[steps];
        roll = true;
    }
}

bool walk_wanted(const vcfxg_ctx *c, bool need_gt_only) {
    return c->hint_line >= 512 && (!need_gt_only || c->hint_gt_only) && !c->walk_overflowed;
}

bool af_knob_allows_walk(const vcfxg_ctx *c) { return c->af_path != 3 && c->af_path != 8; }

int af_buffers(vcfxg_ctx *c, uint64_t L) {
    int r = ensure(c, c->alt, 4 * (L + 1));
    if (!r) r = ensure(c, c->tot, 4 * (L + 1));
    if (!r) r = ensure(c, c->rowpre, 4 * (L + 1));
    if (!r) r = ensure(c, c->status, L + 1);
    if (!r) r = ensure(c, c->rowlen, 8 * (L + 1));
    if (!r) r = ensure(c, c->rowoff, 8 * (L + 1));
    return r;
}

int ensure_sum_host(vcfxg_ctx *c) {
    if (c->sum_host) return VCFXG_OK;
    HIPCHK(c, hipHostMalloc(reinterpret_cast<void **>(&c->sum_host), 256, hipHostMallocMapped | hipHostMallocCoherent));
    std::memset(c->sum_host, 0, 256);
    HIPCHK(c, hipHostGetDevicePointer(reinterpret_cast<void **>(&c->sum_dev), c->sum_host, 0));
    return VCFXG_OK;
}

int walk_buffers(vcfxg_ctx *c, const WalkPlan &p) {
    int r = ensure(c, c->wk_le, 8 * p.cap);
    if (!r) r = ensure(c, c->wk_alt, 4 * p.cap);
    if (!r) r = ensure(c, c->wk_tot, 4 * p.cap);
    if (!r) r = ensure(c, c->wk_rowpre, 4 * p.cap);
    if (!r) r = ensure(c, c->wk_status, p.cap);
    if (!r) r = ensure(c, c->wk_meta, af_meta_bytes() * p.cap);
    if (!r) r = ensure(c, c->wk_count, 8 * (size_t)(p.nw + 1));
    if (!r) r = ensure(c, c->wk_offs, 8 * (size_t)(p.nw + 1));
    if (!r) r = ensure(c, c->wk_gt, 4 * (size_t)p.nw);
    return r;
}

int dense_buffers(vcfxg_ctx *c, uint64_t L) {
    int r = ensure(c, c->line_end, 8 * (L + 1));
    if (!r) r = af_buffers(c, L);
    if (!r) r = ensure(c, c->af_meta, af_meta_bytes() * (L + 1));
    return r;
}

int walk_compact(vcfxg_ctx *c, int64_t nw, uint64_t cap_w, unsigned long long *counters, bool aux,
                 const uint64_t *bpre) {
    HIPCHK(c, launch_walk_compact(nw, cap_w, P<uint64_t>(c->wk_offs), P<uint32_t>(c->wk_gt), P<uint64_t>(c->wk_le),
                                  P<int32_t>(c->wk_alt), P<int32_t>(c->wk_tot), P<uint32_t>(c->wk_rowpre),
                                  P<uint8_t>(c->wk_status), c->wk_meta.p, P<uint64_t>(c->line_end), P<int32_t>(c->alt),
                                  P<int32_t>(c->tot), P<uint32_t>(c->rowpre), P<uint8_t>(c->status), c->af_meta.p,
                                  P<uint64_t>(c->d_nlines), counters, c->stream, aux ? P<int32_t>(c->wk_aux) : nullptr,
                                  aux ? P<int32_t>(c->hwe_aux) : nullptr, bpre));
    return VCFXG_OK;
}

int af_walk_to_dense(vcfxg_ctx *c, const WalkPlan &p, int mode, const char *prof_name, size_t small_zero, bool aux,
                     bool dose, bool head, bool cc) {
    int r = walk_buffers(c, p);
    if (!r && aux) r = ensure(c, c->wk_aux, 4 * p.cap);
    if (!r) r = ensure(c, c->wk_small, 128);
    if (!r) r = dense_buffers(c, p.cap);
    if (!r && aux) r = ensure(c, c->hwe_aux, 4 * (p.cap + 1));
    if (r) return r;
    HIPCHK(c, hipMemsetAsync(c->wk_small.p, 0, small_zero, c->stream));
    HIPCHK(c, hipMemsetAsync(P<uint64_t>(c->wk_count) + p.nw, 0, 8, c->stream));
    prof_begin(c, prof_name);
    if (cc)
        HIPCHK(c, launch_cc_walk(P<char>(c->input), p.lo, p.hi, p.C, mode, c->hint_span, p.cap_w, P<uint64_t>(c->wk_le),
                                 P<int32_t>(c->wk_alt), P<int32_t>(c->wk_tot), P<uint32_t>(c->wk_rowpre),
                                 P<uint8_t>(c->wk_status), c->wk_meta.p, P<uint64_t>(c->wk_count), P<uint32_t>(c->wk_gt),
                                 P<unsigned>(c->wk_small), c->stream));
    else
        HIPCHK(c, launch_af_walk(P<char>(c->input), p.lo, p.hi, p.C, mode, c->hint_span, p.cap_w, P<uint64_t>(c->wk_le),
                             P<int32_t>(c->wk_alt), P<int32_t>(c->wk_tot), P<uint32_t>(c->wk_rowpre),
                             P<uint8_t>(c->wk_status), c->wk_meta.p, P<uint64_t>(c->wk_count), P<uint32_t>(c->wk_gt),
                             P<unsigned>(c->wk_small), c->stream, aux ? P<int32_t>(c->wk_aux) : nullptr, nullptr, dose,
                             false, head, kAfDepthDefault, false));
    prof_end(c, prof_name);
    prof_begin(c, "walk_compact");
    r = exclusive_scan(c, P<uint64_t>(c->wk_count), P<uint64_t>(c->wk_offs), (size_t)p.nw + 1);
    if (r) return r;
    r = walk_compact(c, p.nw, p.cap_w, P<unsigned long long>(c->counters), aux, nullptr);
    if (r) return r;
    prof_end(c, "walk_compact");
    return VCFXG_OK;
}

int fq_walk_to_dense(vcfxg_ctx *c, const WalkPlan &p, int what, int strip_cr, const RfArgs &ra, const char *q_dev,
                     int qlen, int strict, int qa, int qb, const char *walk_name, const char *rest_name) {
    const bool tabs = what == kFqRF || what == kFqBoth, meta = what != kFqRF;
    const size_t mb = af_meta_bytes();
    int r = ensure(c, c->wk_le, 8 * p.cap);
    if (!r) r = ensure(c, c->wk_status, p.cap);
    if (!r && meta) r = ensure(c, c->wk_meta, mb * p.cap);
    if (!r && tabs) r = ensure(c, c->wk_tabs, 16 * p.cap);
    if (!r && tabs) r = ensure(c, c->rf_tabs, 16 * (p.cap + 1));
    if (!r) r = ensure(c, c->wk_count, 8 * (size_t)(p.nw + 1));
    if (!r) r = ensure(c, c->wk_offs, 8 * (size_t)(p.nw + 1));
    if (!r) r = ensure(c, c->fq_small, 128);
    if (!r) r = ensure(c, c->line_end, 8 * (p.cap + 1));
    if (!r) r = ensure(c, c->status, p.cap + 1);
    if (!r && meta) r = ensure(c, c->af_meta, mb * (p.cap + 1));
    if (!r) r = ensure_sum_host(c);
    if (r) return r;
    if (c->fq_small_dirty) HIPCHK(c, hipMemsetAsync(c->fq_small.p, 0, 128, c->stream));
    c->fq_small_dirty = true;
    prof_begin(c, walk_name);
    HIPCHK(c, launch_fq_walk(what, P<char>(c->input), p.lo, p.hi, p.C, strip_cr, c->hint_span, p.cap_w, ra,
                             q_dev, qlen, strict, qa, qb, P<uint64_t>(c->wk_le), P<uint8_t>(c->wk_status),
                             c->wk_meta.p, c->wk_tabs.p, P<uint64_t>(c->wk_count), P<unsigned>(c->fq_small), c->stream));
    prof_end(c, walk_name);
    prof_begin(c, rest_name);
    r = exclusive_scan(c, P<uint64_t>(c->wk_count), P<uint64_t>(c->wk_offs), (size_t)p.nw + 1);
    if (r) return r;
    HIPCHK(c, launch_fq_compact(what, p.nw, p.cap_w, P<uint64_t>(c->wk_offs), P<uint64_t>(c->wk_le),
                                P<uint8_t>(c->wk_status), c->wk_meta.p, c->wk_tabs.p, P<uint64_t>(c->line_end),
                                P<uint8_t>(c->status), c->af_meta.p, c->rf_tabs.p, P<uint64_t>(c->d_nlines), c->stream));
    return VCFXG_OK;
}

int fq_walk_done(vcfxg_ctx *c) {
    HIPCHK(c, launch_fq_done(P<unsigned long long>(c->fq_small) + 1, P<uint64_t>(c->d_nlines), P<uint64_t>(c->fq_small),
                             c->sum_dev + 8, c->stream));
    HIPCHK(c, hipStreamSynchronize(c->stream));
    c->fq_small_dirty = false;
    return VCFXG_OK;
}

}
```

### vcfx_amd/csrc/gpu/vcfxg_cc.hip

```cpp
#include "vcfx_gpu.h"
#include "vcfxg_af_walk_kernel.h"

namespace vcfxg {

constexpr int kCcThreads = 256;
constexpr int kCcWaves = kCcThreads / kWave;
constexpr int kCcSetWords = 128 * 128 / 32;
constexpr uint32_t kCcInvalid = ~0u, kCcEnd = 0x100u;

__device__ __forceinline__ uint32_t cc_parse(const char *__restrict__ buf, int64_t p, int64_t ae, uint32_t max_allele) {
    auto at = [&](int64_t q) -> uint32_t {
        if (q >= ae) return kCcEnd;
        const uint32_t c = byte_at(buf, q);
        return c == ':' || c == '\t' ? kCcEnd : c;
    };
    uint32_t c = at(p);
    if (c == kCcEnd || c == '.') return kCcInvalid;
    uint32_t a1 = 0, a2 = 0;
    while (c - '0' < 10u) {
        a1 = a1 * 10u + (c - '0');
        if (a1 > 1000u) a1 = 1000u;
        c = at(++p);
    }
    if (c != '/' && c != '|') return kCcInvalid;
    c = at(++p);
    if (c == kCcEnd || c == '.') return kCcInvalid;
    while (c - '0' < 10u) {
        a2 = a2 * 10u + (c - '0');
        if (a2 > 1000u) a2 = 1000u;
        c = at(++p);
    }
    if (a1 > max_allele || a2 > max_allele || a1 > 127u || a2 > 127u) return kCcInvalid;
    const uint32_t lo = a1 < a2 ? a1 : a2, hi = a1 < a2 ? a2 : a1;
    return (lo << 7) | hi;
}

__device__ __forceinline__ void cc_line(const char *__restrict__ buf, int64_t ls, int64_t le, int mode, uint32_t ns,
                                        const uint32_t *__restrict__ mult, uint32_t n_mult, int64_t *lds,
                                        uint32_t *set, bool &data, uint8_t &st, uint32_t &N, uint32_t &U,
                                        uint32_t &rowpre) {
    data = false;
    st = 0;
    N = U = rowpre = 0;
    int64_t ae = le;
    if (mode == VCFXG_MODE_FILE && ae > ls && byte_at(buf, ae - 1) == '\r') ae--;
    if (ae <= ls || byte_at(buf, ls) == '#') return;
    data = true;
    int64_t t[5];
    const int nt5 = head_tabs(buf, ls, ae, 5, t, lds);
    if (nt5 < 4) return;
    if (mode == VCFXG_MODE_FILE) {
        if (nt5 == 4 && t[3] + 1 >= ae) return;
        if (t[0] == ls) return;
    }
    const int64_t alt_s = t[3] + 1, alt_e = nt5 >= 5 ? t[4] : ae;
    uint32_t max_allele = 0;
    if (alt_e > alt_s && byte_at(buf, alt_s) != '.') {
        max_allele = 1;
        for (int64_t w = alt_s; w < alt_e; w += kWave) {
            const int64_t p = w + lane();
            max_allele += (uint32_t)__popcll(__ballot(p < alt_e && byte_at(buf, p) == ','));
        }
    }
    uint32_t n_valid = 0, n_new = 0, tabs = 0;
    for (int64_t w = ls & ~(int64_t)15; w < ae; w += kWaveStep) {
        const int64_t blk = w + (int64_t)lane() * kBlockBytes;
        uint32_t m = 0;
        if (blk < ae) m = eq_mask16(load16(buf, blk), kRepTab) & range_mask16(blk, ls, ae);
        const uint32_t c = (uint32_t)__popc(m);
        const uint32_t incl = wave_incl_scan(c);
        uint32_t k = tabs + incl - c;
        tabs += wave_bcast(incl, kWave - 1);
        while (m) {
            const int j = __builtin_ctz(m);
            m &= m - 1u;
            const uint32_t col = k + 1;
            k++;
            if (col < 9) continue;
            const uint32_t s = col - 9;
            const uint32_t mu = mult ? (s < n_mult ? mult[s] : 0u) : (s < ns ? 1u : 0u);
            if (!mu) continue;
            const uint32_t key = cc_parse(buf, blk + j + 1, ae, max_allele);
            if (key == kCcInvalid) continue;
            n_valid += mu;
            const uint32_t bit = 1u << (key & 31u);
            if (!(atomicOr(&set[key >> 5], bit) & bit)) n_new++;
        }
    }
    __builtin_amdgcn_fence(__ATOMIC_RELEASE, "wavefront");
    __builtin_amdgcn_wave_barrier();
    for (int k = lane(); k < kCcSetWords; k += kWave) set[k] = 0u;
    __builtin_amdgcn_fence(__ATOMIC_RELEASE, "wavefront");
    __builtin_amdgcn_wave_barrier();
    if (mode == VCFXG_MODE_STDIN) {
        const uint32_t need = ns + 9u > 8u ? ns + 9u : 8u;
        if (tabs + 1u < need) return;
    }
    N = wave_sum(n_valid);
    U = wave_sum(n_new);
    st = N == 0 ? kCcNoGt : (U == 1 ? kCcSame : kCcDiff);
    rowpre = (uint32_t)(alt_e - ls);
}

__global__ __launch_bounds__(kCcThreads) void k_cc_lines(const char *__restrict__ buf, int64_t data_start,
                                                         const uint64_t *__restrict__ line_end,
                                                         const uint64_t *n_lines_p, int mode, uint32_t ns,
                                                         const uint32_t *__restrict__ mult, uint32_t n_mult,
                                                         const LineMeta *__restrict__ meta, int32_t *__restrict__ n_o,
                                                         int32_t *__restrict__ u_o, uint32_t *__restrict__ rowpre_o,
                                                         uint8_t *__restrict__ status_o, uint32_t *__restrict__ isdata_o,
                                                         unsigned long long *__restrict__ counters) {
    __shared__ int64_t scratch[kCcWaves][16];
    __shared__ uint32_t sets[kCcWaves][kCcSetWords];
    const int wv = threadIdx.x / kWave;
    int64_t *lds = scratch[wv];
    uint32_t *set = sets[wv];
    for (int k = lane(); k < kCcSetWords; k += kWave) set[k] = 0u;
    __builtin_amdgcn_fence(__ATOMIC_RELEASE, "wavefront");
    __builtin_amdgcn_wave_barrier();
    const uint64_t n_lines = *n_lines_p;
    const uint64_t wid = (uint64_t)uniform64((int64_t)((blockIdx.x * (uint64_t)blockDim.x + threadIdx.x) / kWave));
    const uint64_t nw = (gridDim.x * (uint64_t)blockDim.x) / kWave;
    uint32_t cnt[4] = {0, 0, 0, 0};
    for (uint64_t l0 = wid * kWave; l0 < n_lines; l0 += nw * kWave) {
        const uint64_t mine = l0 + lane();
        bool todo_me = mine < n_lines;
        if (meta && todo_me) {
            const LineMeta m = meta[mine];
            const uint8_t ws = status_o[mine];
            if (m.kind == kMetaEmpty || m.kind == kMetaHeader) {
                todo_me = false;
                status_o[mine] = 0;
                isdata_o[mine] = 0u;
            } else if (m.kind == kMetaGt && ws == 1) {
                const int64_t ae = (int64_t)line_end[mine] - m.cr;
                if ((uint64_t)(ae - (int64_t)m.S + 1) == 4ull * ns) {
                    todo_me = false;
                    uint8_t st = 0;
                    if (!(mode == VCFXG_MODE_FILE && (m.pad & kCcEmptyChrom))) {
                        const uint32_t N = (uint32_t)n_o[mine], U = (uint32_t)u_o[mine];
                        st = N == 0 ? kCcNoGt : (U == 1 ? kCcSame : kCcDiff);
                        cnt[0] += st == kCcSame;
                        cnt[1] += st == kCcDiff;
                        cnt[2] += st == kCcNoGt;
                    }
                    status_o[mine] = st;
                    rowpre_o[mine] = m.rowpre - 1u;
                    isdata_o[mine] = 1u;
                }
            }
        }
        uint64_t todo = __ballot(todo_me);
        while (todo) {
            const int k = __builtin_ctzll(todo);
            todo &= todo - 1ull;
            const uint64_t li = l0 + k;
            const int64_t ls = li ? (int64_t)line_end[li - 1] + 1 : data_start, le = (int64_t)line_end[li];
            bool data;
            uint8_t st;
            uint32_t N, U, rp;
            cc_line(buf, ls, le, mode, ns, mult, n_mult, lds, set, data, st, N, U, rp);
            if (lane() == 0) {
                cnt[0] += st == kCcSame;
                cnt[1] += st == kCcDiff;
                cnt[2] += st == kCcNoGt;
                cnt[3] += data ? 1u : 0u;
                status_o[li] = st;
                n_o[li] = (int32_t)N;
                u_o[li] = (int32_t)U;
                rowpre_o[li] = rp;
                isdata_o[li] = data ? 1u : 0u;
            }
        }
    }
    __shared__ uint32_t red[kCcWaves][4];
    for (int k = 0; k < 4; k++) {
        const uint32_t t = wave_sum(cnt[k]);
        if (lane() == 0) red[wv][k] = t;
    }
    __syncthreads();
    if (threadIdx.x < 4) {
        uint32_t t = 0;
        for (int k = 0; k < kCcWaves; k++) t += red[k][threadIdx.x];
        if (t) atomicAdd(&counters[threadIdx.x], (unsigned long long)t);
    }
}

__global__ void k_cc_chrom(const char *__restrict__ buf, int64_t data_start, const uint64_t *__restrict__ line_end,
                           const uint64_t *n_lines_p, uint64_t *__restrict__ out, uint64_t cap, unsigned long long *n) {
    const uint64_t n_lines = *n_lines_p;
    for (uint64_t i = blockIdx.x * (uint64_t)blockDim.x + threadIdx.x; i < n_lines;
         i += gridDim.x * (uint64_t)blockDim.x) {
        const int64_t ls = i ? (int64_t)line_end[i - 1] + 1 : data_start, le = (int64_t)line_end[i];
        if (le - ls < 6 || buf[ls] != '#' || buf[ls + 1] != 'C' || buf[ls + 2] != 'H' || buf[ls + 3] != 'R' ||
            buf[ls + 4] != 'O' || buf[ls + 5] != 'M')
            continue;
        const unsigned long long k = atomicAdd(n, 1ull);
        if (k < cap) out[k] = (uint64_t)ls;
    }
}

__device__ __forceinline__ uint32_t dec_digits(uint32_t v) {
    uint32_t d = 1;
    while (v >= 10u) {
        v /= 10u;
        d++;
    }
    return d;
}

__device__ __forceinline__ uint64_t cc_rank(uint64_t o, uint64_t n, uint64_t T) {
    if (!T) return o;
    const uint64_t Te = T < n ? T : n, q = n / Te, r = n % Te, t = o % Te;
    return t * q + (t < r ? t : r) + o / Te;
}

__global__ void k_cc_rowlen(const uint64_t *n_lines_p, uint64_t T, const uint64_t *__restrict__ ord,
                            const uint32_t *__restrict__ isdata, const uint8_t *__restrict__ status,
                            const int32_t *__restrict__ nn, const int32_t *__restrict__ uu,
                            const uint32_t *__restrict__ rowpre, uint64_t *__restrict__ len) {
    const uint64_t n_lines = *n_lines_p;
    const uint64_t nd = ord[n_lines];
    for (uint64_t i = blockIdx.x * (uint64_t)blockDim.x + threadIdx.x; i < n_lines;
         i += gridDim.x * (uint64_t)blockDim.x) {
        if (!isdata[i]) continue;
        uint64_t l = 0;
        const uint8_t st = status[i];
        if (st == kCcNoGt) l = (uint64_t)rowpre[i] + 3u + 2u + 12u + 1u;
        else if (st) l = (uint64_t)rowpre[i] + 3u + dec_digits((uint32_t)nn[i]) + dec_digits((uint32_t)uu[i]) + 10u + 1u;
        len[cc_rank(ord[i], nd, T)] = l;
    }
}

__global__ void k_cc_summary(const uint64_t *n_lines_p, const uint64_t *__restrict__ ord,
                             const uint64_t *__restrict__ off, const unsigned long long *__restrict__ counters,
                             const unsigned *fail, uint64_t *__restrict__ out) {
    const uint64_t n_lines = *n_lines_p, nd = ord[n_lines];
    out[0] = nd;
    out[1] = off[nd];
    for (int k = 0; k < 4; k++) out[2 + k] = counters[k];
    out[6] = n_lines;
    out[7] = fail ? *fail : 0u;
}

__device__ __forceinline__ char *put_dec(char *o, uint32_t v) {
    const uint32_t d = dec_digits(v);
    for (uint32_t k = d; k-- > 0;) {
        o[k] = (char)('0' + v % 10u);
        v /= 10u;
    }
    return o + d;
}

__global__ void k_cc_format(const char *__restrict__ buf, int64_t data_start, const uint64_t *__restrict__ line_end,
                            const uint64_t *n_lines_p, uint64_t T, const uint64_t *__restrict__ ord,
                            const uint8_t *__restrict__ status, const int32_t *__restrict__ nn,
                            const int32_t *__restrict__ uu, const uint32_t *__restrict__ rowpre,
                            const uint64_t *__restrict__ off, char *__restrict__ out, uint64_t cap) {
    const uint64_t n_lines = *n_lines_p;
    const uint64_t nd = ord[n_lines];
    for (uint64_t i = blockIdx.x * (uint64_t)blockDim.x + threadIdx.x; i < n_lines;
         i += gridDim.x * (uint64_t)blockDim.x) {
        const uint8_t st = status[i];
        if (!st) continue;
        const int64_t ls = i ? (int64_t)line_end[i - 1] + 1 : data_start;
        const uint64_t rk = cc_rank(ord[i], nd, T);
        if (off[rk + 1] > cap) continue;
        char *o = out + off[rk];
        const uint32_t pl = rowpre[i];
        for (uint32_t k = 0; k < pl; k++) o[k] = buf[ls + k];
        o += pl;
        *o++ = '\t';
        o = put_dec(o, st == kCcNoGt ? 0u : (uint32_t)nn[i]);
        *o++ = '\t';
        o = put_dec(o, st == kCcNoGt ? 0u : (uint32_t)uu[i]);
        *o++ = '\t';
        const char *w = st == kCcSame ? "CONCORDANT" : (st == kCcDiff ? "DISCORDANT" : "NO_GENOTYPES");
        while (*w) *o++ = *w++;
        *o = '\n';
    }
}

static unsigned cc_grid(uint64_t n, uint64_t per, unsigned cap) {
    uint64_t g = (n + per - 1) / per;
    if (g < 1) g = 1;
    return (unsigned)(g > cap ? cap : g);
}

hipError_t launch_cc_walk(const char *buf, int64_t lo, int64_t hi, int64_t chunk, int mode, int64_t span0,
                          uint64_t cap_w, uint64_t *le_b, int32_t *alt_b, int32_t *tot_b, uint32_t *rowpre_b,
                          uint8_t *status_b, void *meta_b, uint64_t *wcount, uint32_t *wgt, unsigned *overflow,
                          hipStream_t s) {
    const int64_t nw = af_walkers(lo, hi, chunk);
    if (!nw) return hipErrorInvalidValue;
    hipLaunchKernelGGL(k_af_walk<CcOp>, dim3((unsigned)((nw + kWalkWaves - 1) / kWalkWaves)), dim3(kWalkThreads), 0, s,
                       buf, lo, hi, chunk, nw, mode, span0, cap_w, le_b, alt_b, tot_b, nullptr, rowpre_b, status_b,
                       static_cast<LineMeta *>(meta_b), wcount, wgt, overflow, WalkTail{});
    return hipGetLastError();
}

hipError_t launch_cc_lines(const char *buf, int64_t data_start, const uint64_t *line_end, const uint64_t *n_lines_dev,
                           uint64_t n_lines_host, int mode, uint32_t ns, const uint32_t *mult, uint32_t n_mult,
                           const void *meta, int32_t *n_o, int32_t *u_o, uint32_t *rowpre, uint8_t *status,
                           uint32_t *isdata, unsigned long long *counters, hipStream_t s) {
    if (!n_lines_host) return hipSuccess;
    const unsigned grid = cc_grid((n_lines_host + kWave - 1) / kWave, kCcWaves, meta ? 1024 : 8192);
    hipLaunchKernelGGL(k_cc_lines, dim3(grid), dim3(kCcThreads), 0, s, buf, data_start, line_end, n_lines_dev, mode, ns,
                       mult, n_mult, static_cast<const LineMeta *>(meta), n_o, u_o, rowpre, status, isdata, counters);
    return hipGetLastError();
}

hipError_t launch_cc_chrom(const char *buf, int64_t data_start, const uint64_t *line_end, const uint64_t *n_lines_dev,
                           uint64_t n_lines_host, uint64_t *out, uint64_t cap, unsigned long long *n, hipStream_t s) {
    if (!n_lines_host) return hipSuccess;
    hipLaunchKernelGGL(k_cc_chrom, dim3(cc_grid(n_lines_host, 256, 1024)), dim3(256), 0, s, buf, data_start, line_end,
                       n_lines_dev, out, cap, n);
    return hipGetLastError();
}

hipError_t launch_cc_rowlen(const uint64_t *n_lines_dev, uint64_t n_lines_host, uint64_t T, const uint64_t *ord,
                            const uint32_t *isdata, const uint8_t *status, const int32_t *nn, const int32_t *uu,
                            const uint32_t *rowpre, uint64_t *len, hipStream_t s) {
    if (!n_lines_host) return hipSuccess;
    hipLaunchKernelGGL(k_cc_rowlen, dim3(cc_grid(n_lines_host, 256, 1024)), dim3(256), 0, s, n_lines_dev, T, ord, isdata,
                       status, nn, uu, rowpre, len);
    return hipGetLastError();
}

hipError_t launch_cc_summary(const uint64_t *n_lines_dev, const uint64_t *ord, const uint64_t *off,
                             const unsigned long long *counters, const unsigned *fail, uint64_t *out, hipStream_t s) {
    hipLaunchKernelGGL(k_cc_summary, dim3(1), dim3(1), 0, s, n_lines_dev, ord, off, counters, fail, out);
    return hipGetLastError();
}

hipError_t launch_cc_format(const char *buf, int64_t data_start, const uint64_t *line_end, const uint64_t *n_lines_dev,
                            uint64_t n_lines_host, uint64_t T, const uint64_t *ord, const uint8_t *status,
                            const int32_t *nn, const int32_t *uu, const uint32_t *rowpre, const uint64_t *off, char *out,
                            uint64_t text_cap, hipStream_t s) {
    if (!n_lines_host) return hipSuccess;
    hipLaunchKernelGGL(k_cc_format, dim3(cc_grid(n_lines_host, 256, 4096)), dim3(256), 0, s, buf, data_start, line_end,
                       n_lines_dev, T, ord, status, nn, uu, rowpre, off, out, text_cap);
    return hipGetLastError();
}

}
```

### vcfx_amd/csrc/gpu/vcfxg_ctx.h

```cpp
#pragma once
#include <hip/hip_runtime.h>

#include <algorithm>
#include <cstdio>
#include <cstdlib>
#include <cstring>
#include <map>
#include <string>
#include <vector>

#include "vcfx_gpu.h"
#include "vcfxg_kernels.h"
#include "vcfxg_rf.h"

struct DevBuf {
    void *p = nullptr;
    size_t cap = 0;
};

struct vcfxg_ctx {
    int device = 0;
    hipStream_t stream = nullptr;
    std::string err;
    DevBuf input;
    size_t n = 0;
    int last_byte = -1;
    bool loaded = false;
    bool ingesting = false;
    bool hints_pending = false;
    const char *last_schedule = "";
    std::vector<std::pair<size_t, hipEvent_t>> ingest_ev;
    std::vector<hipEvent_t> ingest_ev_free;
    DevBuf idx_counts, idx_offs, idx_pos, line_end, d_nlines, scan_tmp;
    size_t data_start = 0;
    uint64_t n_lines = 0;
    bool indexed = false;
    DevBuf alt, tot, rowpre, status, rowlen, rowoff, text, counters, query, crit, pool;
    std::string query_host, crit_host, pool_host;
    DevBuf ld_G, ld_lines, ld_vidx, ld_valid, ld_Gc, ld_vars, ld_plen, ld_poff, ld_prefix, ld_cid, ld_blocks, ld_cnt,
        ld_off, ld_pairs, ld_fast, ld_gflag, ld_Gp, ld_rowoff, ld_Gv, ld_Gq, dose_meta;
    DevBuf ld_wcnt, ld_wval, ld_vbase, ld_small, ld_pend;
    size_t bgz_total = 0, bgz_staged = 0;
    uint64_t bgz_handed = 0;
    uint64_t bgz_launched = 0, bgz_out = 0;
    hipStream_t copy_stream = nullptr;
    hipEvent_t bgz_copy_ev = nullptr;
    static constexpr int kBgzStreams = 2;
    hipStream_t bgz_stream[kBgzStreams] = {};
    hipEvent_t bgz_ev[kBgzStreams] = {};
    int bgz_next = 0;
    bool ld_gc_ready = false;
    bool ld_vq = false;
    int n_cu = 0;
    DevBuf async_small;
    DevBuf ld_temp, ld_quarters, ld_stage_ctr;
    uint64_t ld_temp_cap = 0;
    uint64_t ld_stage_cap_fixed = getenv("VCFXG_LD_STAGE_CAP") ? strtoull(getenv("VCFXG_LD_STAGE_CAP"), nullptr, 10) : 0;
    DevBuf af_meta;
    DevBuf wk_le, wk_alt, wk_tot, wk_rowpre, wk_status, wk_meta, wk_count, wk_offs, wk_gt, wk_small;
    DevBuf wk_tabs, rf_tabs;
    DevBuf wk_text, wk_toff, wk_start, wk_cx, wk_bs, scratch_small, byte_cnt;
    DevBuf af_small;
    bool af_small_dirty = true;
    DevBuf wk_stage, wk_dirty;
    uint64_t *sum_host = nullptr, *sum_dev = nullptr;
    uint64_t cx_hint = ~0ull;
    DevBuf fq_small;
    bool fq_small_dirty = true;
    uint64_t fq_lines_hint = 0;
    std::string query_dev, crit_dev, pool_dev;
    void *query_dev_p = nullptr, *crit_dev_p = nullptr, *pool_dev_p = nullptr;
    bool dense_pending = false;
    int64_t dense_nw = 0;
    uint64_t dense_cap_w = 0;
    DevBuf hwe_aux, wk_aux, hwe_rc;
    DevBuf ac_eff, ac_noff, ac_names, ac_scratch, ac_etab, ac_nib;
    std::vector<uint32_t> ac_eff_host;
    std::vector<uint64_t> ac_noff_host;
    std::string ac_names_host;
    std::vector<uint8_t> ac_etab_host;
    DevBuf ph_G, ph_isvar, ph_info, ph_vnum, ph_vline, ph_flags, ph_r2;
    uint64_t ph_nvar = 0;
    uint64_t hwe_rc_n = 0;
    DevBuf ib_codes, ib_meta, ib_tab, ib_packed, ib_cnt, ib_offs, ib_sum, ib_obs, ib_used, ib_carried, ib_small;
    uint32_t ib_ns = 0;
    DevBuf sx_mask;
    std::vector<uint32_t> sx_mask_host;
    uint64_t sx_block = getenv("VCFXG_SX_BLOCK")
                            ? std::min<uint64_t>(std::max<uint64_t>(strtoull(getenv("VCFXG_SX_BLOCK"), nullptr, 10), 1), 1u << 24)
                            : 65536;
    DevBuf cc_mult, cc_isdata, cc_ord, cc_chrom, cc_small;
    uint64_t cc_totals[4] = {0, 0, 0, 0};
    DevBuf dd_tabs, dd_pos, dd_hash, dd_queue, dd_isdata, dd_ord, dd_k0, dd_k1, dd_v0, dd_v1, dd_tmp, dd_hp, dd_head,
        dd_left;
    uint64_t dd_counts[6] = {0, 0, 0, 0, 0, 0};
    bool dd_done = false;
    DevBuf srt_pos, srt_aux, srt_w0, srt_queue, srt_written, srt_ord, srt_k0, srt_k1, srt_v0, srt_v1, srt_tmp, srt_len,
        srt_off, srt_src;
    uint64_t srt_counts[6] = {0, 0, 0, 0, 0, 0};
    uint64_t srt_nw = 0;
    bool srt_done = false, srt_in_v1 = false;
    std::vector<uint64_t> srt_off_host;
    uint64_t srt_block = getenv("VCFXG_SRT_BLOCK")
                             ? std::min<uint64_t>(std::max<uint64_t>(strtoull(getenv("VCFXG_SRT_BLOCK"), nullptr, 10), 1), 1ull << 36)
                             : 256ull << 20;
    int srt_nt = getenv("VCFXG_SRT_NT") ? atoi(getenv("VCFXG_SRT_NT")) & 3 : 3;
    DevBuf df_tabs, df_klen, df_koff, df_ntok, df_posv, df_natv, df_nsuf, df_hash, df_isdata, df_ord, df_queue, df_ktext,
        df_line, df_k0, df_k1, df_v0, df_v1, df_tmp, df_hp, df_head, df_rep, df_first2, df_left, df_state, df_uflag, df_uord,
        df_len, df_off, df_src, df_sum;
    uint64_t df_counts[8] = {0, 0, 0, 0, 0, 0, 0, 0};
    uint64_t df_nu = 0, df_nu1 = 0;
    bool df_done = false;
    std::vector<uint64_t> df_off_host;
    uint64_t df_block = getenv("VCFXG_DF_BLOCK")
                            ? std::min<uint64_t>(std::max<uint64_t>(strtoull(getenv("VCFXG_DF_BLOCK"), nullptr, 10), 1), 1ull << 36)
                            : 256ull << 20;
    uint64_t df_walk_steps = getenv("VCFXG_DF_WALK_STEPS")
                                 ? std::min<uint64_t>(std::max<uint64_t>(strtoull(getenv("VCFXG_DF_WALK_STEPS"), nullptr, 10), 1), 1ull << 24)
                                 : 1ull << 20;
    DevBuf mg_file, mg_pos, mg_w0, mg_ks, mg_kl, mg_pn, mg_num, mg_queue, mg_written, mg_ord, mg_fmeta, mg_k0, mg_k1, mg_v0,
        mg_v1, mg_tmp, mg_len, mg_off, mg_src, mg_state;
    uint64_t mg_counts[8] = {0, 0, 0, 0, 0, 0, 0, 0};
    uint64_t mg_nw = 0;
    uint32_t mg_files = 0;
    bool mg_done = false, mg_in_v1 = false;
    std::vector<uint64_t> mg_off_host;
    uint64_t mg_walk_steps = getenv("VCFXG_MG_WALK_STEPS")
                                 ? std::min<uint64_t>(std::max<uint64_t>(strtoull(getenv("VCFXG_MG_WALK_STEPS"), nullptr, 10), 1), 1ull << 24)
                                 : 1ull << 20;
    DevBuf ms_tab, ms_geom, ms_cost, ms_costoff, ms_rowbase, ms_lineoff, ms_small;
    std::vector<uint32_t> ms_tab_host;
    uint64_t ms_l0 = 0, ms_n = 0;
    bool ms_done = false;
    uint64_t ms_block = getenv("VCFXG_MS_BLOCK")
                            ? std::min<uint64_t>(std::max<uint64_t>(strtoull(getenv("VCFXG_MS_BLOCK"), nullptr, 10), 1), 1u << 24)
                            : 65536;
    DevBuf fa_flag, fa_col, fa_meta, fa_M, fa_rowoff, fa_skip;
    uint64_t fa_l0 = 0, fa_n = 0, fa_cols = 0, fa_text = 0;
    bool fa_scanned = false, fa_begun = false;
    uint64_t fa_block = getenv("VCFXG_FA_BLOCK")
                            ? std::min<uint64_t>(std::max<uint64_t>(strtoull(getenv("VCFXG_FA_BLOCK"), nullptr, 10), 1), 1u << 24)
                            : 65536;
    uint64_t ms_bytes = getenv("VCFXG_MS_BYTES") ? std::max<uint64_t>(strtoull(getenv("VCFXG_MS_BYTES"), nullptr, 10), 1)
                                                 : 512ull << 20;
    uint64_t ib_block = getenv("VCFXG_IB_BLOCK")
                            ? std::min<uint64_t>(std::max<uint64_t>(strtoull(getenv("VCFXG_IB_BLOCK"), nullptr, 10), 1), 1u << 24)
                            : 65536;
    int64_t hwe_ulps = getenv("VCFXG_HWE_ULPS") ? atoll(getenv("VCFXG_HWE_ULPS")) : 16;
    int64_t walk_chunk = getenv("VCFXG_WALK_CHUNK")
                             ? std::min<int64_t>(std::max<int64_t>(atol(getenv("VCFXG_WALK_CHUNK")), 4096), 8 << 20)
                             : 128 * 1024;
    bool walk_overflowed = false;
    bool dose_head_failed = false;
    bool ph_head_failed = false;
    int64_t hint_span = 0, hint_line = 0;
    bool hint_gt_only = false;
    bool hint_gt_first = false;
    uint64_t af_line_cap = 0;
    int af_path = getenv("VCFXG_AF_FUSED") ? atoi(getenv("VCFXG_AF_FUSED")) : 0;
    int af_depth_knob = getenv("VCFXG_AF_DEPTH") ? atoi(getenv("VCFXG_AF_DEPTH")) : 0;
    int last_af_depth = 0;
    bool last_af_roll = false;
    int fq_path = getenv("VCFXG_FQ_WALK") ? atoi(getenv("VCFXG_FQ_WALK")) : 0;
    std::vector<uint8_t> ld_gflag_host;
    uint64_t ld_m = 0, ld_prefix_bytes = 0, ld_np = 0;
    int ld_kpad = 64, ld_ns = 0, ld_kp4 = 64;
    bool ld_chrom_ids = false;
    std::vector<uint32_t> ld_cid_host, ld_blocks_host;
    uint64_t ld_plan_key[5] = {0, 0, 0, 0, 0};
    std::vector<uint8_t> ld_plan_gf;
    uint32_t ld_plan_n[4] = {0, 0, 0, 0};
    bool ld_sp = false;
    uint64_t ld_mp = 0;
    DevBuf ld_moff, ld_midx, ld_mvar, ld_gt16, ld_sprec, ld_midx16;
    DevBuf bgz_in, bgz_mem, bgz_off, bgz_stat, bgz_small, bgz_perm;
    DevBuf bgz_tok[kBgzStreams + 1];
    vcfxg::InflateSide bgz_side;
    void *ld_plan_dev = nullptr;
    uint64_t text_bytes = 0;
    uint64_t text_hint = 0;
    bool profiling = false;
    std::string prof_only;
    struct ProfRec {
        const char *name;
        hipEvent_t a, b;
    };
    std::vector<hipEvent_t> ev_free;
    std::vector<ProfRec> ev_open, pending;
    std::map<std::string, float> ms;
    std::map<std::string, std::pair<double, uint64_t>> acc;
};

namespace vcfxg {

constexpr size_t kPad = 256;

int fail(vcfxg_ctx *c, hipError_t e, const char *what);
#define HIPCHK(ctx, x)                                          \
    do {                                                        \
        hipError_t e_ = (x);                                    \
        if (e_ != hipSuccess) return vcfxg::fail(ctx, e_, #x);  \
    } while (0)
int ensure(vcfxg_ctx *c, DevBuf &b, size_t bytes);
template <typename T>
T *P(DevBuf &b) {
    return reinterpret_cast<T *>(b.p);
}
void prof_begin(vcfxg_ctx *c, const char *name);
void prof_end(vcfxg_ctx *c, const char *name);
void prof_collect(vcfxg_ctx *c);
int exclusive_scan(vcfxg_ctx *c, const uint32_t *in, uint64_t *out, size_t n);
int exclusive_scan(vcfxg_ctx *c, const uint64_t *in, uint64_t *out, size_t n);
void note_schedule(vcfxg_ctx *c, const char *what);
bool load_hints(vcfxg_ctx *c, const char *h, size_t n);

int ensure_dense(vcfxg_ctx *c);
#define DENSE(c)                          \
    do {                                  \
        int rd_ = vcfxg::ensure_dense(c); \
        if (rd_) return rd_;              \
    } while (0)

int af_buffers(vcfxg_ctx *c, uint64_t L);
int ensure_sum_host(vcfxg_ctx *c);
struct WalkPlan {
    int64_t lo, hi, C, nw;
    uint64_t cap_w, cap;
    bool fits_gt16;
    int af_depth;
    bool af_roll;
};
WalkPlan walk_plan(const vcfxg_ctx *c, size_t data_start, int64_t chunk = 0);
void af_sweep_plan(int64_t span, int knob, int &depth, bool &roll);
bool walk_wanted(const vcfxg_ctx *c, bool need_gt_only);
bool af_knob_allows_walk(const vcfxg_ctx *c);
int walk_buffers(vcfxg_ctx *c, const WalkPlan &p);
int dense_buffers(vcfxg_ctx *c, uint64_t L);
int walk_compact(vcfxg_ctx *c, int64_t nw, uint64_t cap_w, unsigned long long *counters, bool aux,
                 const uint64_t *bpre);
int af_walk_to_dense(vcfxg_ctx *c, const WalkPlan &p, int mode, const char *prof_name, size_t small_zero, bool aux,
                     bool dose, bool head, bool cc = false);
int fq_walk_to_dense(vcfxg_ctx *c, const WalkPlan &p, int what, int strip_cr, const RfArgs &ra, const char *q_dev,
                     int qlen, int strict, int qa, int qb, const char *walk_name, const char *rest_name);
int fq_walk_done(vcfxg_ctx *c);

}
```

### vcfx_amd/csrc/gpu/vcfxg_kernels.h

```cpp
#pragma once
#include <hip/hip_runtime.h>
#include <stdint.h>

namespace vcfxg {

enum : uint8_t { kMetaEmpty = 0, kMetaGt = 1, kMetaFull = 2, kMetaHeader = 3, kMetaGated = 4 };
struct LineMeta {
    uint64_t S;
    uint32_t rowpre;
    uint8_t kind;
    uint8_t sep;
    uint8_t cr;
    uint8_t pad;
};
constexpr uint8_t kAfPending = 0xFF;
constexpr uint8_t kGqPending = 0xFE;
constexpr uint8_t kRfPending = 0xFD;
constexpr uint8_t kGqFull = 0xFC;
constexpr uint8_t kHweAltComma = 1, kHweEmptyField = 2;
constexpr uint8_t kWalkUnswept = 4;
constexpr uint8_t kCcEmptyChrom = 8;

int idx_pos_cap();
struct BgzfMember {
    uint64_t src_off;
    uint32_t src_len;
    uint32_t out_len;
};
struct Crc1k {
    uint32_t v[32];
};
void crc32_zero1k_basis(Crc1k *z);
struct InflateSide {
    hipStream_t aux = nullptr;
    hipEvent_t ev[2] = {};
};
hipError_t launch_inflate(int which, const uint8_t *comp, const BgzfMember *mem, const uint64_t *out_off,
                          uint64_t n_members, uint8_t *out, uint32_t *mstat, unsigned long long *first_bad,
                          const Crc1k &z1k, hipStream_t s, uint64_t mbase = 0, uint32_t *tok = nullptr,
                          uint64_t tok_members = 0, const uint32_t *perm = nullptr, const InflateSide *side = nullptr);
constexpr uint32_t kTokCap = 6144;
hipError_t launch_count_byte(const uint8_t *buf, uint64_t lo, uint64_t hi, uint8_t byte, unsigned long long *out,
                             hipStream_t s);
int64_t idx_wchunks(int64_t lo, int64_t hi);
hipError_t launch_idx_count(const char *buf, int64_t lo, int64_t hi, uint32_t *counts, uint64_t *pos,
                            unsigned *overflow, hipStream_t s);
hipError_t launch_idx_emit(const char *buf, int64_t lo, int64_t hi, const uint64_t *offs, uint64_t *line_end,
                           hipStream_t s);
hipError_t launch_nl_compact(int64_t lo, int64_t hi, const uint32_t *counts, const uint64_t *offs, const uint64_t *pos,
                             uint64_t *line_end, hipStream_t s);
hipError_t launch_af_records(const char *buf, int64_t data_start, const uint64_t *line_end, const uint64_t *n_lines_dev,
                             uint64_t n_lines_host, int mode, int32_t *alt, int32_t *tot, uint32_t *rowpre,
                             uint8_t *status, unsigned long long *counters, hipStream_t s);
size_t af_meta_bytes();
hipError_t launch_af_meta_sweep(const char *buf, int64_t data_start, const uint64_t *line_end,
                                const uint64_t *n_lines_dev, uint64_t n_lines_host, int mode, void *meta, int32_t *alt,
                                int32_t *tot, uint32_t *rowpre, uint8_t *status, unsigned long long *counters,
                                hipStream_t s);
hipError_t launch_af_meta_sweep_range(const char *buf, int64_t data_start, const uint64_t *line_end,
                                      const uint64_t *range, uint64_t max_lines, int mode, void *meta, int32_t *alt,
                                      int32_t *tot, uint32_t *rowpre, uint8_t *status, unsigned long long *counters,
                                      hipStream_t s);
int64_t idx_wchunk_bytes();
int64_t af_walkers(int64_t lo, int64_t hi, int64_t chunk);
struct WalkTail {
    uint64_t *wtext = nullptr;
    uint64_t *wstart = nullptr;
    uint64_t *cx_list = nullptr;
    unsigned long long *cx_n = nullptr;
    uint64_t cx_cap = 0;
    char *stage = nullptr;
    uint32_t stage_cap = 0;
    uint8_t *wdirty = nullptr;
};
constexpr int kAfDepthDefault = 6, kAfDepthMax = 12;
constexpr int kAfWaveStep = 1024;
constexpr bool af_depth_compiled(int d) { return d == 6 || d == 8 || d == 10 || d == 12; }
hipError_t launch_af_walk(const char *buf, int64_t lo, int64_t hi, int64_t chunk, int mode, int64_t span0,
                          uint64_t cap_w, uint64_t *le_b, int32_t *alt_b, int32_t *tot_b, uint32_t *rowpre_b,
                          uint8_t *status_b, void *meta_b, uint64_t *wcount, uint32_t *wgt, unsigned *overflow,
                          hipStream_t s, int32_t *hwe_aux_b = nullptr, const WalkTail *tail = nullptr,
                          bool dose = false, bool gt_first_walk = false, bool dose_head = false,
                          int depth = kAfDepthDefault, bool roll = false);
hipError_t launch_cc_walk(const char *buf, int64_t lo, int64_t hi, int64_t chunk, int mode, int64_t span0,
                          uint64_t cap_w, uint64_t *le_b, int32_t *alt_b, int32_t *tot_b, uint32_t *rowpre_b,
                          uint8_t *status_b, void *meta_b, uint64_t *wcount, uint32_t *wgt, unsigned *overflow,
                          hipStream_t s);
hipError_t launch_af_cx(const char *buf, int mode, uint64_t cap_w, const uint64_t *list, const unsigned long long *list_n,
                        uint64_t list_cap, uint64_t list_cap_host, const uint64_t *wstart, const uint64_t *le_b,
                        const void *meta_b, int32_t *alt_b, int32_t *tot_b, uint32_t *rowpre_b, uint8_t *status_b,
                        uint64_t *wtext, unsigned long long *counters, hipStream_t s);
constexpr int kWalkerScanBlock = 1024;
hipError_t launch_walker_scan(int64_t nw, const uint64_t *wcount, const uint64_t *wtext, const uint32_t *wgt,
                              uint64_t *woff, uint64_t *wtoff, uint64_t *bpre_a, uint64_t *bpre_b, uint64_t *bsum,
                              unsigned *done, unsigned long long *counters, const unsigned *fail, uint64_t *n_lines,
                              uint64_t *summary, hipStream_t s, uint64_t *reset = nullptr);
hipError_t launch_af_format_w(const char *buf, int mode, int64_t nw, uint64_t cap_w, const uint64_t *wcount,
                              const uint64_t *wtoff, const uint64_t *bpre_b, const uint64_t *wstart,
                              const uint64_t *le_b, const int32_t *alt_b, const int32_t *tot_b, const uint32_t *rowpre_b,
                              const uint8_t *status_b, char *out, uint64_t cap, hipStream_t s, const WalkTail *tail = nullptr);
hipError_t launch_walk_compact(int64_t n_walkers, uint64_t cap_w, const uint64_t *offs, const uint32_t *wgt,
                               const uint64_t *le_b, const int32_t *alt_b, const int32_t *tot_b,
                               const uint32_t *rowpre_b, const uint8_t *status_b, const void *meta_b,
                               uint64_t *line_end, int32_t *alt, int32_t *tot, uint32_t *rowpre, uint8_t *status,
                               void *meta, uint64_t *n_lines, unsigned long long *counters, hipStream_t s,
                               const int32_t *aux_b = nullptr, int32_t *aux = nullptr, const uint64_t *bpre = nullptr);
hipError_t launch_af_complex(const char *buf, int64_t data_start, const uint64_t *line_end,
                             const uint64_t *n_lines_dev, uint64_t n_lines_host, int mode, const void *meta,
                             int32_t *alt, int32_t *tot, uint32_t *rowpre, uint8_t *status,
                             unsigned long long *counters, hipStream_t s);
hipError_t launch_nr_complex(const char *buf, int64_t data_start, const uint64_t *line_end,
                             const uint64_t *n_lines_dev, uint64_t n_lines_host, int mode, uint8_t *status,
                             unsigned long long *counters, hipStream_t s);
hipError_t launch_nr_records(const char *buf, int64_t data_start, const uint64_t *line_end,
                             const uint64_t *n_lines_dev, uint64_t n_lines_host, int mode, uint8_t *status,
                             unsigned long long *counters, hipStream_t s);
hipError_t launch_gq_records(const char *buf, int64_t data_start, const uint64_t *line_end,
                             const uint64_t *n_lines_dev, uint64_t n_lines_host, int strip_cr, const char *q_dev,
                             int qlen, int strict, int qa, int qb, uint8_t *status, unsigned long long *counters,
                             hipStream_t s, const uint8_t *gate, void *meta = nullptr);
hipError_t launch_gq_complex(const char *buf, int64_t data_start, const uint64_t *line_end,
                             const uint64_t *n_lines_dev, uint64_t n_lines_host, int strip_cr, const char *q_dev,
                             int qlen, int strict, int qa, int qb, const void *meta, uint8_t *status,
                             unsigned long long *counters, const uint8_t *gate, hipStream_t s);
hipError_t launch_nl_compact_cap(int64_t lo, int64_t hi, const uint32_t *counts, const uint64_t *offs,
                                 const uint64_t *pos, uint64_t *line_end, uint64_t cap, hipStream_t s);
hipError_t launch_idx_finish(const uint64_t *offs, int64_t nchunks, const unsigned *idx_overflow, int tail, int64_t hi,
                             uint64_t cap, uint64_t *line_end, uint64_t *n_lines, unsigned *fail, hipStream_t s);
hipError_t launch_af_summary(const uint64_t *n_lines, const uint64_t *rowoff, const unsigned long long *counters,
                             const unsigned *fail, uint64_t *out, hipStream_t s);
hipError_t launch_af_rowlen(const uint32_t *rowpre, const uint8_t *status, const uint64_t *n_lines_dev,
                            uint64_t n_lines_host, uint64_t *len, hipStream_t s);
hipError_t launch_hwe_lines(const char *buf, int64_t data_start, const uint64_t *line_end, const uint64_t *n_lines_dev,
                            uint64_t n_lines_host, int mode, const void *meta, int32_t *c0, int32_t *c1, int32_t *c2,
                            uint32_t *rowpre, uint8_t *status, unsigned long long *counters, hipStream_t s);
hipError_t launch_hwe_rowlen(const uint64_t *n_lines_dev, uint64_t n_lines_host, int mode, const void *meta,
                             const uint32_t *rowpre, uint8_t *status, uint64_t *len, unsigned long long *counters,
                             hipStream_t s);
hipError_t launch_hwe_format(const char *buf, int64_t data_start, const uint64_t *line_end, const uint64_t *n_lines_dev,
                             uint64_t n_lines_host, int mode, const int32_t *c0, const int32_t *c1, const int32_t *c2,
                             const uint32_t *rowpre, const uint8_t *status, const uint64_t *off, char *out,
                             uint64_t text_cap, int64_t ulps, void *rc, unsigned long long *rc_n, uint64_t rc_cap,
                             hipStream_t s);
size_t dose_meta_bytes();
hipError_t launch_dose_len(const char *buf, int64_t data_start, const uint64_t *line_end, const uint64_t *n_lines_dev,
                           uint64_t n_lines_host, int mode, uint8_t *status, uint64_t *len, void *meta,
                           unsigned long long *counters, hipStream_t s, bool pending_only = false);
hipError_t launch_dose_from_walk(const uint64_t *line_end, const uint64_t *n_lines_dev, uint64_t n_lines_host,
                                 const void *walk_meta, const int32_t *ns, const int32_t *na, uint8_t *status,
                                 uint64_t *len, void *meta, unsigned long long *counters, hipStream_t s);
hipError_t launch_dose_fmt(const char *buf, int64_t data_start, const uint64_t *line_end, const uint64_t *n_lines_dev,
                           uint64_t n_lines_host, const uint8_t *status, const void *meta, const uint64_t *off,
                           char *out, uint64_t cap, uint64_t slow_rows, hipStream_t s, unsigned *bad = nullptr,
                           uint64_t na_rows = ~0ull);
constexpr uint8_t kMdFlag = 6;
hipError_t launch_md_lines(const char *buf, int64_t data_start, int64_t n_input, const uint64_t *line_end,
                           const uint64_t *n_lines_dev, uint64_t n_lines_host, int mode, uint8_t *status,
                           int32_t *info_s, int32_t *info_e, unsigned long long *counters, hipStream_t s,
                           int walk = 0);
size_t ac_meta_bytes();
int ac_threads();
hipError_t launch_ac_len(const char *buf, int64_t data_start, const uint64_t *line_end, uint64_t l0, uint64_t l1,
                         unsigned blocks, const uint32_t *eff, const uint64_t *noff, const char *names,
                         uint32_t *scratch, uint32_t m, uint32_t scap, int seq, int kind, int ident, int direct,
                         uint32_t *nib, uint8_t *status, uint64_t *len, void *meta, unsigned long long *counters,
                         hipStream_t s);
hipError_t launch_ac_fmt(const char *buf, int64_t data_start, const uint64_t *line_end, uint64_t l0, uint64_t l1,
                         unsigned blocks, const uint32_t *eff, const uint64_t *noff, const char *names,
                         uint32_t *scratch, uint32_t m, uint32_t scap, int seq, int kind, uint32_t sel_lds,
                         int ident, int direct, const uint8_t *status, const void *meta, const uint64_t *off,
                         char *out, hipStream_t s);
hipError_t launch_ac_rows(const char *buf, int64_t data_start, const uint64_t *line_end, uint64_t l0, uint64_t l1,
                          unsigned blocks, const uint32_t *eff, uint32_t m, int ident, const void *etab, uint32_t L,
                          const uint32_t *nib, const void *meta, const uint64_t *off, char *out, hipStream_t s);
size_t ac_rows_lds(uint32_t m, int ident);
size_t ac_rows_lds_max();
int ac_rows_threads();
enum : uint8_t { kPhSkip = 0, kPhVar = 1, kPhFew = 3, kPhHeader = 4, kPhPos = 7, kPhNoGt = 8 };
size_t ph_line_bytes();
hipError_t launch_ph_lines(const char *buf, int64_t data_start, const uint64_t *line_end, const uint64_t *n_lines_dev,
                           uint64_t n_lines_host, int mode, uint32_t kpad, int8_t *G, uint8_t *status, uint32_t *isvar,
                           void *info, unsigned long long *counters, hipStream_t s, const void *walk_meta = nullptr,
                           unsigned *bad = nullptr);
hipError_t launch_ph_compact(const uint32_t *isvar, const uint64_t *vnum, const uint64_t *n_lines_dev,
                             uint64_t n_lines_host, uint64_t *vline, uint64_t *n_var, hipStream_t s);
hipError_t launch_ph_pairs(const char *buf, const uint64_t *vline, const uint64_t *n_var_dev, uint64_t n_var_host,
                           const void *info, const int8_t *G, uint32_t kpad, double thr, uint8_t *flags, uint64_t *len,
                           double *r2, hipStream_t s);
hipError_t launch_ph_fmt(const char *buf, const uint64_t *vline, const uint64_t *n_var_dev, uint64_t n_var_host,
                         const void *info, const uint64_t *off, char *out, hipStream_t s);
hipError_t launch_af_format(const char *buf, int64_t data_start, const uint64_t *line_end, const uint64_t *n_lines_dev,
                            uint64_t n_lines_host, int mode, const int32_t *alt, const int32_t *tot,
                            const uint32_t *rowpre, const uint8_t *status, const uint64_t *off, char *out,
                            hipStream_t s, uint64_t text_cap = ~0ull);

size_t ib_meta_bytes();
size_t ib_rec_bytes();
hipError_t launch_ib_walk(const char *buf, int64_t lo, int64_t hi, int64_t chunk, int64_t w0, int64_t nw, uint32_t G,
                          uint32_t cap_w, int mode, uint32_t ns, uint32_t ld, int8_t *codes, void *meta, uint32_t *cnt,
                          unsigned *ovf, unsigned long long *counters, hipStream_t s);
hipError_t launch_ib_lines(const char *buf, int64_t data_start, const uint64_t *line_end, uint64_t l0, uint32_t n,
                           int mode, uint32_t ns, uint32_t ld, int8_t *codes, void *meta, uint32_t *cnt,
                           unsigned long long *counters, hipStream_t s);
hipError_t launch_ib_table(const void *meta, const uint32_t *cnt, uint32_t *offs, uint32_t G, uint32_t cap_w,
                           int global_freq, void *rec, hipStream_t s);
size_t ib_packed_bytes(uint64_t slots, uint32_t ns);
hipError_t launch_ib_pack(const int8_t *codes, uint32_t ld, const void *rec, const uint32_t *n_rec, uint64_t slots,
                          void *packed, uint32_t ns, hipStream_t s);
hipError_t launch_ib_chain(const void *rec, const uint32_t *n_rec, uint64_t slots, const void *packed, uint32_t ns,
                           int mode, int skip_boundary, int count_boundary, double *sum_exp, uint64_t *obs_het,
                           uint64_t *used, int32_t *carried, hipStream_t s);
hipError_t launch_ib_rows(const double *sum_exp, const uint64_t *obs_het, const uint64_t *used, uint32_t ns,
                          const char *names, const uint64_t *noff, char *out, uint64_t *text_bytes, hipStream_t s);

enum : uint8_t { kSxEmpty = 0, kSxRow = 1, kSxShort = 3, kSxHeader = 4, kSxNoSample = 5, kSxPre = 6, kSxChrom = 7 };
int sx_threads();
uint32_t sx_stage_bytes();
hipError_t launch_sx_len(const char *buf, int64_t data_start, const uint64_t *line_end, uint64_t l0, uint64_t l1,
                         unsigned blocks, const uint32_t *mask, uint32_t nwords, uint32_t lastk, uint32_t m,
                         int stdin_mode, int seen, uint8_t *status, uint64_t *len, unsigned long long *counters,
                         hipStream_t s);
hipError_t launch_sx_write(const char *buf, int64_t data_start, const uint64_t *line_end, uint64_t l0, uint64_t l1,
                           unsigned blocks, const uint32_t *mask, uint32_t nwords, uint32_t lastk, uint32_t m,
                           int stdin_mode, int seen, const uint8_t *status, const uint64_t *off, char *out,
                           hipStream_t s);

enum : uint8_t { kCcSame = 1, kCcDiff = 2, kCcNoGt = 3 };
hipError_t launch_cc_lines(const char *buf, int64_t data_start, const uint64_t *line_end, const uint64_t *n_lines_dev,
                           uint64_t n_lines_host, int mode, uint32_t ns, const uint32_t *mult, uint32_t n_mult,
                           const void *meta, int32_t *n_o, int32_t *u_o, uint32_t *rowpre, uint8_t *status,
                           uint32_t *isdata, unsigned long long *counters, hipStream_t s);
hipError_t launch_cc_chrom(const char *buf, int64_t data_start, const uint64_t *line_end, const uint64_t *n_lines_dev,
                           uint64_t n_lines_host, uint64_t *out, uint64_t cap, unsigned long long *n, hipStream_t s);
hipError_t launch_cc_rowlen(const uint64_t *n_lines_dev, uint64_t n_lines_host, uint64_t T, const uint64_t *ord,
                            const uint32_t *isdata, const uint8_t *status, const int32_t *nn, const int32_t *uu,
                            const uint32_t *rowpre, uint64_t *len, hipStream_t s);
hipError_t launch_cc_summary(const uint64_t *n_lines_dev, const uint64_t *ord, const uint64_t *off,
                             const unsigned long long *counters, const unsigned *fail, uint64_t *out, hipStream_t s);
hipError_t launch_cc_format(const char *buf, int64_t data_start, const uint64_t *line_end, const uint64_t *n_lines_dev,
                            uint64_t n_lines_host, uint64_t T, const uint64_t *ord, const uint8_t *status,
                            const int32_t *nn, const int32_t *uu, const uint32_t *rowpre, const uint64_t *off, char *out,
                            uint64_t text_cap, hipStream_t s);

enum : uint8_t { kDdEmpty = 0, kDdKept = 1, kDdDup = 2, kDdShort = 3, kDdHeader = 4 };
constexpr int kDdWindow = 64;
hipError_t launch_dd_key(const char *buf, int64_t data_start, int64_t n, const uint64_t *line_end, uint64_t L,
                         int stdin_mode, uint8_t *status, uint32_t *isdata, uint64_t *tabs, int32_t *pos, uint64_t *hash,
                         uint32_t *queue, unsigned long long *counters, hipStream_t s);
hipError_t launch_dd_gather(uint64_t L, const uint32_t *isdata, const uint64_t *ord, const uint64_t *hash,
                            uint32_t hash_bits, uint64_t *keys, uint32_t *vals, hipStream_t s);
hipError_t launch_dd_heads(uint64_t nd, const uint64_t *keys, uint32_t *hp, hipStream_t s);
hipError_t launch_dd_verify(const char *buf, int64_t data_start, const uint64_t *line_end, int stdin_mode,
                            const uint64_t *tabs, const int32_t *pos, uint64_t nd, const uint64_t *keys, const uint32_t *vals,
                            const uint32_t *head, uint8_t *status, uint8_t *left, unsigned long long *counters,
                            hipStream_t s);
hipError_t launch_dd_count(uint64_t L, const uint8_t *status, unsigned long long *counters, hipStream_t s);

enum : uint8_t { kMsEmpty = 0, kMsCopy = 1, kMsSplit = 2, kMsHeader = 4 };
enum : uint32_t { kMsOther = 0, kMsA = 1, kMsR = 2, kMsG = 3 };
enum : uint32_t { kMsInfo = 0, kMsFormat = 1 };
constexpr uint32_t kMsKeysLds = 32;
constexpr uint32_t kMsTableLds = 16384;
constexpr int kMsGeom = 10;
hipError_t launch_ms_scan(const char *buf, int64_t data_start, const uint64_t *line_end, uint64_t l0, uint64_t n,
                          int stdin_mode, uint8_t *status, int32_t *alt, uint32_t *geom, uint64_t *cost, hipStream_t s);
hipError_t launch_ms_cut(const uint64_t *costoff, const uint64_t *rowbase, uint64_t n, uint64_t budget, uint64_t *small,
                         hipStream_t s);
hipError_t launch_ms_len(const char *buf, int64_t data_start, const uint64_t *line_end, uint64_t l0, uint64_t n,
                         int stdin_mode, const uint32_t *table, uint32_t table_bytes, uint32_t entries, uint64_t rows,
                         const uint64_t *rowbase, const int32_t *alt, const uint32_t *geom, uint64_t *len,
                         unsigned long long *counters, hipStream_t s);
hipError_t launch_ms_write(const char *buf, int64_t data_start, const uint64_t *line_end, uint64_t l0, uint64_t n,
                           int stdin_mode, const uint32_t *table, uint32_t table_bytes, uint32_t entries, uint64_t rows,
                           const uint64_t *rowbase, const int32_t *alt, const uint32_t *geom, const uint64_t *off,
                           char *out, hipStream_t s);
hipError_t launch_ms_ranges(uint64_t l0, uint64_t n, const uint8_t *status, const uint64_t *rowbase,
                            const uint64_t *rowoff, uint64_t *lineoff, unsigned long long *counters, hipStream_t s);

enum : uint8_t { kFaEmpty = 0, kFaColumn = 1, kFaSkipped = 3, kFaHeader = 4, kFaChrom = 7 };
constexpr uint32_t kFaLine = 60;
constexpr uint32_t kFaTileSamples = 64;
constexpr uint32_t kFaTileCols = 240;
constexpr uint32_t kFaTable = 16;
struct FaMeta {
    uint32_t S, E, alt_s, alt_e;
    int32_t gi;
    uint32_t pad[3];
    uint8_t tab[16];
};
static_assert(sizeof(FaMeta) == 48, "FaMeta: twelve words");
hipError_t launch_fa_scan(const char *buf, int64_t data_start, const uint64_t *line_end, uint64_t l0, uint64_t n,
                          int stdin_mode, uint32_t n_samples, uint8_t *status, uint32_t *flag, FaMeta *meta,
                          unsigned long long *counters, hipStream_t s);
hipError_t launch_fa_bases(const char *buf, int64_t data_start, const uint64_t *line_end, uint64_t l0, uint64_t n,
                           const uint8_t *status, const uint64_t *col, const FaMeta *meta, uint32_t n_samples,
                           uint64_t pitch, uint8_t *M, unsigned long long *counters, hipStream_t s);
hipError_t launch_fa_transpose(const uint8_t *M, uint64_t pitch, uint64_t ncols, uint32_t n_samples, uint64_t first_col,
                               uint64_t total_cols, const uint64_t *row_off, const uint64_t *skip, char *text,
                               hipStream_t s);

enum : uint8_t { kSrtEmpty = 0, kSrtKept = 1, kSrtPre = 2, kSrtBad = 3, kSrtHeader = 4 };
constexpr int kSrtWindow = 64;
hipError_t launch_srt_key(const char *buf, int64_t data_start, const uint64_t *line_end, uint64_t L, int stdin_mode,
                          int natural, uint8_t *status, int32_t *pos, uint32_t *aux, uint64_t *w0, uint32_t *queue,
                          unsigned long long *counters, hipStream_t s);
hipError_t launch_srt_class(uint64_t L, int stdin_mode, int natural, uint8_t *status, const uint32_t *aux,
                            uint32_t *written, unsigned long long *counters, hipStream_t s);
hipError_t launch_srt_scatter(uint64_t L, int stdin_mode, int natural, const uint8_t *status, const uint32_t *written,
                              const uint64_t *ord, const int32_t *pos, const uint32_t *aux, uint64_t *keys,
                              uint32_t *vals, hipStream_t s);
hipError_t launch_srt_word(const char *buf, int64_t data_start, const uint64_t *line_end, uint64_t nw, int stdin_mode,
                           uint32_t w, uint32_t shift, const uint32_t *vals, const uint8_t *status, const uint32_t *aux,
                           const uint64_t *w0, uint64_t *keys, hipStream_t s);
hipError_t launch_srt_len(int64_t data_start, const uint64_t *line_end, uint64_t nw, const uint32_t *order,
                          uint64_t *len, uint64_t *src, hipStream_t s);
hipError_t launch_srt_gather(const char *buf, const uint64_t *off, const uint64_t *src, uint64_t first, uint64_t k,
                             uint64_t bytes, int nt, char *text, hipStream_t s);

enum : uint8_t { kDfEmpty = 0, kDfCommon = 1, kDfUnique = 2, kDfSkipped = 3, kDfHeader = 4, kDfRepeat = 5, kDfData = 6 };
constexpr int kDfWindow = 64;
struct DfLines {
    const char *buf;
    int64_t data_start;
    const uint64_t *line_end;
    uint64_t L;
    uint8_t *status;
    uint32_t *isdata, *ntok;
    uint64_t *tabs, *klen, *nsuf;
    int64_t *posv, *natv;
};
hipError_t launch_df_cut(const uint64_t *line_end, int64_t data_start, uint64_t L, uint64_t second_start,
                         unsigned long long *counters, hipStream_t s);
hipError_t launch_df_key(const DfLines &D, int natural, uint32_t *queue, unsigned long long *counters, hipStream_t s);
hipError_t launch_df_text(const DfLines &D, const uint64_t *ord, const uint64_t *koff, char *ktext, uint64_t *hash,
                          uint32_t *line, uint32_t *queue, unsigned long long *counters, hipStream_t s);
hipError_t launch_df_pairs(uint64_t nd, const uint32_t *line, const uint64_t *hash, uint32_t hash_bits, uint64_t *keys,
                           uint32_t *vals, hipStream_t s);
hipError_t launch_df_classes(const char *ktext, const uint64_t *koff, const uint64_t *klen, uint64_t nd, const uint64_t *keys,
                             const uint32_t *vals, const uint32_t *head, uint32_t *rep, uint32_t *first2, uint8_t *left,
                             uint8_t *status, unsigned long long *counters, hipStream_t s);
hipError_t launch_df_ordered(const DfLines &D, int natural, const uint32_t *line, uint64_t n1, uint64_t nd,
                             unsigned long long *counters, hipStream_t s);
hipError_t launch_df_bounds(const DfLines &D, int natural, const uint32_t *line, uint64_t n1, uint64_t nd, hipStream_t s);
hipError_t launch_df_walk(const DfLines &D, int natural, const uint32_t *line, uint64_t n1, uint64_t nd, uint64_t steps,
                          uint64_t *state, hipStream_t s);
hipError_t launch_df_drain(const uint32_t *line, uint64_t n1, uint64_t nd, const uint64_t *state, uint8_t *status,
                           hipStream_t s);
hipError_t launch_df_flag(uint64_t L, const uint8_t *status, uint32_t *uflag, hipStream_t s);
hipError_t launch_df_place(uint64_t L, const uint32_t *uflag, const uint64_t *uord, const uint64_t *koff,
                           const uint64_t *klen, uint64_t *len, uint64_t *src, hipStream_t s);
hipError_t launch_df_sum(uint64_t L, const uint64_t *ord, const uint64_t *uord, const unsigned long long *counters,
                         uint64_t *sum, hipStream_t s);

enum : uint8_t { kMgEmpty = 0, kMgKept = 1, kMgBad = 2, kMgHeader = 3, kMgDropped = 4 };
enum { kMgPartPos = 0, kMgPartLen = 1, kMgPartWord = 2, kMgPartNum = 3, kMgPartPrefix = 4 };
constexpr int kMgWindow = 64;
struct MgLines {
    const char *buf;
    const uint64_t *line_end;
    uint64_t L;
    uint32_t K;
    int sorted, natural;
    uint8_t *status;
    uint32_t *file, *pn;
    uint64_t *w0, *ks, *kl, *num;
    int64_t *pos;
    const uint64_t *file_start;
    uint64_t *first_line, *first_hash, *first_data, *bad, *cur, *end;
};
hipError_t launch_mg_cut(const MgLines &M, hipStream_t s);
hipError_t launch_mg_key(const MgLines &M, uint32_t *queue, unsigned long long *counters, hipStream_t s);
hipError_t launch_mg_class(const MgLines &M, uint32_t *written, unsigned long long *counters, hipStream_t s);
hipError_t launch_mg_scatter(uint64_t L, const uint32_t *written, const uint64_t *ord, uint32_t *vals, hipStream_t s);
hipError_t launch_mg_part(const MgLines &M, uint64_t nw, int part, uint64_t w, uint32_t shift, const uint32_t *vals,
                          uint64_t *keys, hipStream_t s);
hipError_t launch_mg_ordered(const MgLines &M, uint64_t nw, const uint32_t *line, unsigned long long *counters,
                             hipStream_t s);
hipError_t launch_mg_walk_init(const MgLines &M, const uint64_t *ord, const uint32_t *line, uint32_t *out,
                               const unsigned long long *counters, uint64_t *state, hipStream_t s);
hipError_t launch_mg_walk(const MgLines &M, const uint32_t *line, uint32_t *out, uint64_t steps, uint64_t *state,
                          hipStream_t s);

}
```

### vcfx_amd/engine.py

```python
import ctypes
import os

from . import GPU_LIB

VCFXG_OK = 0
MODE_FILE, MODE_STDIN = 0, 1
STATUS = {0: "skip", 1: "row", 2: "drop", 3: "warn", 4: "header"}


class Summary(ctypes.Structure):
    _fields_ = [("n_lines", ctypes.c_uint64), ("rows", ctypes.c_uint64), ("data_lines", ctypes.c_uint64),
                ("warn_lines", ctypes.c_uint64), ("text_bytes", ctypes.c_uint64),
                ("general_records", ctypes.c_uint64)]


class AcParams(ctypes.Structure):
    _fields_ = [("sample", ctypes.c_void_p), ("m", ctypes.c_uint64), ("names", ctypes.c_char_p),
                ("name_off", ctypes.c_void_p), ("seq", ctypes.c_int), ("kind", ctypes.c_int)]


class IbParams(ctypes.Structure):
    _fields_ = [("n_samples", ctypes.c_uint32), ("names", ctypes.c_char_p), ("name_off", ctypes.c_void_p),
                ("freq_mode", ctypes.c_int), ("skip_boundary", ctypes.c_int),
                ("count_boundary_as_used", ctypes.c_int)]


class SxParams(ctypes.Structure):
    _fields_ = [("cols", ctypes.c_void_p), ("m", ctypes.c_uint64), ("mode", ctypes.c_int),
                ("seen_chrom", ctypes.c_int)]


class MsEntry(ctypes.Structure):
    _fields_ = [("id", ctypes.c_char_p), ("id_len", ctypes.c_uint32), ("section", ctypes.c_uint8),
                ("number", ctypes.c_uint8)]


class MsParams(ctypes.Structure):
    _fields_ = [("table", ctypes.c_void_p), ("n_entries", ctypes.c_uint64), ("mode", ctypes.c_int)]


class FaParams(ctypes.Structure):
    _fields_ = [("mode", ctypes.c_int), ("n_samples", ctypes.c_uint32), ("first_col", ctypes.c_uint64),
                ("total_cols", ctypes.c_uint64), ("row_off", ctypes.c_void_p), ("skip", ctypes.c_void_p)]


class DfParams(ctypes.Structure):
    _fields_ = [("second_start", ctypes.c_uint64), ("assume_sorted", ctypes.c_int), ("natural", ctypes.c_int),
                ("hash_bits", ctypes.c_uint32)]


class MgParams(ctypes.Structure):
    _fields_ = [("file_start", ctypes.c_void_p), ("n_files", ctypes.c_uint32), ("assume_sorted", ctypes.c_int),
                ("natural", ctypes.c_int)]


class CcParams(ctypes.Structure):
    _fields_ = [("n_samples", ctypes.c_uint32), ("mult", ctypes.c_void_p), ("n_mult", ctypes.c_uint64),
                ("threads", ctypes.c_uint64)]


class Criterion(ctypes.Structure):
    _fields_ = [("target", ctypes.c_int), ("op", ctypes.c_int), ("numeric", ctypes.c_int), ("value", ctypes.c_double),
                ("key", ctypes.c_char_p), ("key_len", ctypes.c_size_t), ("str", ctypes.c_char_p),
                ("str_len", ctypes.c_size_t)]


POS, QUAL, FILTER, INFO = 0, 1, 2, 3
GT, GE, LT, LE, EQ, NE = 0, 1, 2, 3, 4, 5


_P, _VP, _S, _U64, _I = ctypes.c_char_p, ctypes.c_void_p, ctypes.c_size_t, ctypes.c_uint64, ctypes.c_int
SIGNATURES = {
    "vcfxg_version": (_P, []),
    "vcfxg_device_count": (_I, [ctypes.POINTER(_I)]),
    "vcfxg_open": (_I, [_I, ctypes.POINTER(_VP)]),
    "vcfxg_close": (None, [_VP]),
    "vcfxg_last_error": (_P, [_VP]),
    "vcfxg_stream": (_VP, [_VP]),
    "vcfxg_set_profiling": (_I, [_VP, _I]),
    "vcfxg_set_profiling_only": (_I, [_VP, _P]),
    "vcfxg_kernel_ms": (_I, [_VP, _P, ctypes.POINTER(ctypes.c_float)]),
    "vcfxg_kernel_stats": (_I, [_VP, _P, ctypes.POINTER(ctypes.c_double), ctypes.POINTER(_U64)]),
    "vcfxg_reset_kernel_stats": (_I, [_VP]),
    "vcfxg_load_host": (_I, [_VP, _VP, _S]),
    "vcfxg_ingest_begin": (_I, [_VP, _S]),
    "vcfxg_ingest": (_I, [_VP, _VP, _S, _I]),
    "vcfxg_ingest_wait": (_I, [_VP, _S]),
    "vcfxg_ingest_bgzf": (_I, [_VP, _VP, _S, _VP, _S, _VP, _S, ctypes.POINTER(_U64)]),
    "vcfxg_bgzf_stage": (_I, [_VP, _VP, _S, _S, _S]),
    "vcfxg_bgzf_inflate": (_I, [_VP, _VP, _S]),
    "vcfxg_host_alloc": (_I, [_VP, _S, ctypes.POINTER(_VP)]),
    "vcfxg_host_free": (None, [_VP, _VP]),
    "vcfxg_input_device_ptr": (_VP, [_VP]),
    "vcfxg_input_fetch": (_I, [_VP, _U64, _S, _VP]),
    "vcfxg_index": (_I, [_VP, _S, ctypes.POINTER(_U64)]),
    "vcfxg_line_ends": (_I, [_VP, _U64, _U64, _VP]),
    "vcfxg_allele_freq": (_I, [_VP, _I, ctypes.POINTER(Summary)]),
    "vcfxg_allele_freq_region": (_I, [_VP, _S, _I, ctypes.POINTER(Summary)]),
    "vcfxg_genotype_query": (_I, [_VP, _P, _S, _I, _I, ctypes.POINTER(Summary)]),
    "vcfxg_record_filter": (_I, [_VP, _VP, _I, _I, ctypes.POINTER(Summary)]),
    "vcfxg_record_filter_ex": (_I, [_VP, _VP, _I, _I, _I, ctypes.POINTER(Summary)]),
    "vcfxg_variant_count": (_I, [_VP, _I, ctypes.POINTER(Summary)]),
    "vcfxg_nonref_filter": (_I, [_VP, _I, ctypes.POINTER(Summary)]),
    "vcfxg_nonref_filter_region": (_I, [_VP, _S, _I, ctypes.POINTER(Summary)]),
    "vcfxg_hwe_region": (_I, [_VP, _S, _I, ctypes.POINTER(Summary)]),
    "vcfxg_hwe_rechecks": (_I, [_VP, _VP, _U64, ctypes.POINTER(_U64)]),
    "vcfxg_dosage_region": (_I, [_VP, _S, _I, ctypes.POINTER(Summary)]),
    "vcfxg_missing_region": (_I, [_VP, _S, _I, ctypes.POINTER(Summary)]),
    "vcfxg_allele_counter": (_I, [_VP, _U64, _U64, _VP, ctypes.POINTER(Summary)]),
    "vcfxg_inbreeding_region": (_I, [_VP, _S, _I, _VP, ctypes.POINTER(Summary)]),
    "vcfxg_inbreeding_samples": (_I, [_VP, _VP, _VP, _VP]),
    "vcfxg_sample_extract": (_I, [_VP, _U64, _U64, _VP, ctypes.POINTER(Summary)]),
    "vcfxg_concordance_region": (_I, [_VP, _S, _I, _VP, ctypes.POINTER(Summary)]),
    "vcfxg_concordance_totals": (_I, [_VP, _VP]),
    "vcfxg_chrom_lines": (_I, [_VP, _S, _VP, _U64, ctypes.POINTER(_U64)]),
    "vcfxg_dedup": (_I, [_VP, _I, _VP, ctypes.POINTER(Summary)]),
    "vcfxg_dedup_status": (_I, [_VP, _U64, _U64, _VP]),
    "vcfxg_dedup_counts": (_I, [_VP, _VP]),
    "vcfxg_sort": (_I, [_VP, _I, _VP, ctypes.POINTER(Summary)]),
    "vcfxg_sort_status": (_I, [_VP, _U64, _U64, _VP]),
    "vcfxg_sort_counts": (_I, [_VP, _VP]),
    "vcfxg_sort_order": (_I, [_VP, _U64, _U64, _VP]),
    "vcfxg_sort_text": (_I, [_VP, _U64, ctypes.POINTER(_U64), ctypes.POINTER(_U64)]),
    "vcfxg_diff": (_I, [_VP, _VP, ctypes.POINTER(Summary)]),
    "vcfxg_diff_status": (_I, [_VP, _U64, _U64, _VP]),
    "vcfxg_diff_counts": (_I, [_VP, _VP]),
    "vcfxg_diff_text": (_I, [_VP, _I, _U64, ctypes.POINTER(_U64), ctypes.POINTER(_U64)]),
    "vcfxg_merge": (_I, [_VP, _VP, ctypes.POINTER(Summary)]),
    "vcfxg_merge_status": (_I, [_VP, _U64, _U64, _VP]),
    "vcfxg_merge_counts": (_I, [_VP, _VP]),
    "vcfxg_merge_files": (_I, [_VP, _VP, _VP]),
    "vcfxg_merge_order": (_I, [_VP, _U64, _U64, _VP]),
    "vcfxg_merge_text": (_I, [_VP, _U64, ctypes.POINTER(_U64), ctypes.POINTER(_U64)]),
    "vcfxg_multiallelic_split": (_I, [_VP, _U64, _U64, _VP, ctypes.POINTER(Summary)]),
    "vcfxg_ms_line_ranges": (_I, [_VP, _U64, _U64, _VP]),
    "vcfxg_fasta_scan": (_I, [_VP, _U64, _U64, _I, ctypes.c_uint32, ctypes.POINTER(Summary)]),
    "vcfxg_fasta_status": (_I, [_VP, _U64, _U64, _VP, _VP]),
    "vcfxg_fasta_begin": (_I, [_VP, _U64]),
    "vcfxg_fasta": (_I, [_VP, _U64, _U64, _VP, ctypes.POINTER(Summary)]),
    "vcfxg_fetch_text_range": (_I, [_VP, _U64, _S, _VP]),
    "vcfxg_shard_cuts": (_I, [_VP, _S, _S, _I, _VP]),
    "vcfxg_comm_init": (_I, [_VP, _I, ctypes.POINTER(_VP)]),
    "vcfxg_comm_allreduce_u64": (_I, [_VP, _I, _VP, _S]),
    "vcfxg_comm_uses_rccl": (_I, [_VP]),
    "vcfxg_comm_destroy": (None, [_VP]),
    "vcfxg_comm_rccl_stats": (_I, [_VP, ctypes.POINTER(_U64), ctypes.POINTER(_U64)]),
    "vcfxg_last_schedule": (_P, [_VP]),
    "vcfxg_last_af_depth": (_I, [_VP, ctypes.POINTER(_I)]),
    "vcfxg_bgzf_handed_over": (_U64, [_VP]),
    "vcfxg_count_byte": (_I, [_VP, _U64, _I, ctypes.POINTER(_U64)]),
    "vcfxg_haplotype_phaser": (_I, [_VP, _S, _I, ctypes.c_double, ctypes.c_uint32, ctypes.POINTER(Summary)]),
    "vcfxg_phaser_variants": (_I, [_VP, _VP, _VP, _VP]),
    "vcfxg_ld_prepare": (_I, [_VP, _I, _I, _P, _S, _I, _I, _I, _I, ctypes.POINTER(_U64)]),
    "vcfxg_ld_prepare_region": (_I, [_VP, _S, _I, _I, _P, _S, _I, _I, _I, _I, ctypes.POINTER(_U64)]),
    "vcfxg_ld_prefixes": (_I, [_VP, _VP, _S, _VP]),
    "vcfxg_ld_matrix": (_I, [_VP, _I, _I, ctypes.POINTER(_U64)]),
    "vcfxg_ld_stream_chunk": (_I, [_VP, _U64, _U64, _U64, ctypes.c_double, _I, ctypes.POINTER(_U64),
                                   ctypes.POINTER(_U64)]),
    "vcfxg_ld_fetch_pairs": (_I, [_VP, _U64, _U64, _VP, _VP, _VP]),
    "vcfxg_selftest_mfma_i8": (_I, [_VP, ctypes.POINTER(_I)]),
    "vcfxg_selftest_mfma_fp4": (_I, [_VP, ctypes.POINTER(_I)]),
    "vcfxg_filter_query": (_I, [_VP, _VP, _I, _I, _P, _S, _I, ctypes.POINTER(Summary)]),
    "vcfxg_record_filter_region": (_I, [_VP, _S, _VP, _I, _I, ctypes.POINTER(Summary)]),
    "vcfxg_genotype_query_region": (_I, [_VP, _S, _P, _S, _I, _I, ctypes.POINTER(Summary)]),
    "vcfxg_filter_query_region": (_I, [_VP, _S, _VP, _I, _I, _P, _S, _I, ctypes.POINTER(Summary)]),
    "vcfxg_fetch_text": (_I, [_VP, _VP, _S]),
    "vcfxg_fetch_lines": (_I, [_VP, _U64, _U64, _VP, _VP, _VP]),
}

_lib = None


def lib():
    global _lib
    if _lib is None:
        if not os.path.exists(GPU_LIB):
            raise RuntimeError("libvcfx_gpu.so not built (run `make` or __graft_entry__.build())")
        _lib = ctypes.CDLL(GPU_LIB)
        for name, (res, args) in SIGNATURES.items():
            if os.environ.get("VCFXG_GPU_LIB") and not hasattr(_lib, name):
                continue
            f = getattr(_lib, name)
            f.restype = res
            f.argtypes = args
    return _lib


class EngineError(RuntimeError):
    pass


class Engine:

    def __init__(self, device=0):
        self.L = lib()
        h = ctypes.c_void_p()
        rc = self.L.vcfxg_open(device, ctypes.byref(h))
        if rc != VCFXG_OK:
            raise EngineError("vcfxg_open(%d) failed rc=%d: no usable gfx950 device" % (device, rc))
        self.h = h
        self._buf = None

    def close(self):
        if self.h:
            self.L.vcfxg_close(self.h)
            self.h = None

    def __del__(self):
        try:
            self.close()
        except Exception:
            pass

    def _chk(self, rc, what):
        if rc != VCFXG_OK:
            raise EngineError("%s failed rc=%d: %s" % (what, rc, self.L.vcfxg_last_error(self.h).decode()))

    @property
    def stream(self):
        return self.L.vcfxg_stream(self.h)

    def set_profiling(self, on=True):
        self._chk(self.L.vcfxg_set_profiling(self.h, int(on)), "set_profiling")

    def set_profiling_only(self, name=None):
        if not hasattr(self.L, "vcfxg_set_profiling_only"):
            return
        self._chk(self.L.vcfxg_set_profiling_only(self.h, name.encode() if name else None), "set_profiling_only")

    def kernel_ms(self, name):
        v = ctypes.c_float()
        rc = self.L.vcfxg_kernel_ms(self.h, name.encode(), ctypes.byref(v))
        return v.value if rc == VCFXG_OK else None

    def kernel_stats(self, name):
        t = ctypes.c_double()
        n = ctypes.c_uint64()
        self._chk(self.L.vcfxg_kernel_stats(self.h, name.encode(), ctypes.byref(t), ctypes.byref(n)), "kernel_stats")
        return t.value, n.value

    def reset_kernel_stats(self):
        self._chk(self.L.vcfxg_reset_kernel_stats(self.h), "reset_kernel_stats")

    def load(self, data):
        import numpy as np
        arr = np.frombuffer(data, np.uint8) if not isinstance(data, np.ndarray) else data
        self._buf = arr
        self._chk(self.L.vcfxg_load_host(self.h, arr.ctypes.data, arr.size), "load_host")

    def ingest(self, chunks):
        import numpy as np
        arrs = [np.frombuffer(c, np.uint8) if not isinstance(c, np.ndarray) else c for c in chunks]
        self._buf = arrs
        self._chk(self.L.vcfxg_ingest_begin(self.h, 0), "ingest_begin")
        if not arrs:
            self._chk(self.L.vcfxg_ingest(self.h, None, 0, 1), "ingest")
        for i, a in enumerate(arrs):
            self._chk(self.L.vcfxg_ingest(self.h, a.ctypes.data, a.size, int(i == len(arrs) - 1)), "ingest")

    def load_bgzf(self, comp, members=None, head=b""):
        import numpy as np
        arr = np.frombuffer(comp, np.uint8) if not isinstance(comp, np.ndarray) else comp
        mem = bgzf_members(arr) if members is None else members
        hd = np.frombuffer(head, np.uint8) if head else None
        self._buf = (arr, mem, hd)
        total = int(mem["out_len"].sum()) if len(mem) else 0
        self._chk(self.L.vcfxg_ingest_begin(self.h, total), "ingest_begin")
        bad = ctypes.c_uint64()
        rc = self.L.vcfxg_ingest_bgzf(self.h, arr.ctypes.data, arr.size, mem.ctypes.data if len(mem) else None,
                                      len(mem), hd.ctypes.data if hd is not None else None,
                                      0 if hd is None else hd.size, ctypes.byref(bad))
        if rc == -7:
            return bad.value, self.L.vcfxg_last_error(self.h).decode()
        self._chk(rc, "ingest_bgzf")
        self._chk(self.L.vcfxg_ingest(self.h, None, 0, 1), "ingest")
        return None

    def bgzf_handed_over(self):
        return int(self.L.vcfxg_bgzf_handed_over(self.h))

    def input_bytes(self, offset, n):
        b = ctypes.create_string_buffer(max(1, n))
        self._chk(self.L.vcfxg_input_fetch(self.h, offset, n, b), "input_fetch")
        return b.raw[:n]

    def index(self, data_start):
        n = ctypes.c_uint64()
        self._chk(self.L.vcfxg_index(self.h, data_start, ctypes.byref(n)), "index")
        return n.value

    def allele_freq(self, mode=MODE_FILE):
        s = Summary()
        self._chk(self.L.vcfxg_allele_freq(self.h, mode, ctypes.byref(s)), "allele_freq")
        return s

    def allele_freq_region(self, data_start, mode=MODE_FILE):
        s = Summary()
        self._chk(self.L.vcfxg_allele_freq_region(self.h, data_start, mode, ctypes.byref(s)), "allele_freq_region")
        return s

    def last_af_depth(self):
        r = ctypes.c_int()
        d = self.L.vcfxg_last_af_depth(self.h, ctypes.byref(r))
        return d, bool(r.value)

    def genotype_query(self, query, strict=False, strip_cr=False):
        q = query.encode() if isinstance(query, str) else query
        s = Summary()
        self._chk(self.L.vcfxg_genotype_query(self.h, q, len(q), int(strict), int(strip_cr), ctypes.byref(s)),
                  "genotype_query")
        return s

    def nonref_filter(self, mode):
        s = Summary()
        self._chk(self.L.vcfxg_nonref_filter(self.h, int(mode), ctypes.byref(s)), "nonref_filter")
        return s

    def nonref_filter_region(self, data_start, mode):
        s = Summary()
        self._chk(self.L.vcfxg_nonref_filter_region(self.h, data_start, int(mode), ctypes.byref(s)),
                  "nonref_filter_region")
        return s

    def hwe_region(self, data_start, mode):
        s = Summary()
        self._chk(self.L.vcfxg_hwe_region(self.h, data_start, int(mode), ctypes.byref(s)), "hwe_region")
        return s

    def dosage_region(self, data_start, mode):
        s = Summary()
        self._chk(self.L.vcfxg_dosage_region(self.h, data_start, int(mode), ctypes.byref(s)), "dosage_region")
        return s

    def missing_region(self, data_start, mode):
        s = Summary()
        self._chk(self.L.vcfxg_missing_region(self.h, data_start, int(mode), ctypes.byref(s)), "missing_region")
        return s

    def allele_counter(self, l0, l1, samples, names, seq=0, kind=0):
        import numpy as np
        idx = np.ascontiguousarray(samples, np.uint32)
        nb = [x.encode() if isinstance(x, str) else bytes(x) for x in names]
        assert len(nb) == len(idx)
        off = np.zeros(len(nb) + 1, np.uint64)
        off[1:] = np.cumsum([len(x) for x in nb])
        p = AcParams(idx.ctypes.data, len(idx), b"".join(nb), off.ctypes.data, int(seq), int(kind))
        s = Summary()
        self._chk(self.L.vcfxg_allele_counter(self.h, l0, l1, ctypes.byref(p), ctypes.byref(s)), "allele_counter")
        return s

    def inbreeding_region(self, data_start, mode, names, freq_mode=0, skip_boundary=False,
                          count_boundary_as_used=False):
        import numpy as np
        nb = [x.encode() if isinstance(x, str) else bytes(x) for x in names]
        off = np.zeros(len(nb) + 1, np.uint64)
        off[1:] = np.cumsum([len(x) for x in nb])
        p = IbParams(len(nb), b"".join(nb), off.ctypes.data, int(freq_mode), int(skip_boundary),
                     int(count_boundary_as_used))
        s = Summary()
        self._ib_n = 0
        self._chk(self.L.vcfxg_inbreeding_region(self.h, data_start, int(mode), ctypes.byref(p), ctypes.byref(s)),
                  "inbreeding_region")
        self._ib_n = len(nb)
        return s

    def inbreeding_samples(self):
        import numpy as np
        n = getattr(self, "_ib_n", 0)
        if not n:
            raise EngineError("inbreeding_samples: no successful inbreeding_region call on this context")
        se, oh, us = np.zeros(n, np.float64), np.zeros(n, np.uint64), np.zeros(n, np.uint64)
        self._chk(self.L.vcfxg_inbreeding_samples(self.h, se.ctypes.data, oh.ctypes.data, us.ctypes.data),
                  "inbreeding_samples")
        return se, oh, us

    def sample_extract(self, l0, l1, cols, mode=MODE_FILE, seen_chrom=True):
        import numpy as np
        idx = np.ascontiguousarray(cols, np.uint32)
        p = SxParams(idx.ctypes.data if len(idx) else None, len(idx), int(mode), int(bool(seen_chrom)))
        s = Summary()
        self._chk(self.L.vcfxg_sample_extract(self.h, l0, l1, ctypes.byref(p), ctypes.byref(s)), "sample_extract")
        return s

    def sample_extract_all(self, l0, l1, cols, mode=MODE_FILE, seen_chrom=True):
        import numpy as np
        text, st, sums = [], [], []
        while l0 < l1:
            s = self.sample_extract(l0, l1, cols, mode, seen_chrom)
            text.append(self.text(s.text_bytes))
            b = np.zeros(max(int(s.n_lines), 1), np.uint8)
            self._chk(self.L.vcfxg_fetch_lines(self.h, l0, s.n_lines, None, None, b.ctypes.data), "fetch_lines")
            st.append(b[:s.n_lines])
            sums.append(s)
            l0 += s.n_lines
        return b"".join(text), (np.concatenate(st) if st else np.zeros(0, np.uint8)), sums

    def concordance(self, data_start, mode, n_samples=0, mult=None, threads=0):
        import numpy as np
        m = None if mult is None else np.ascontiguousarray(mult, np.uint32)
        if m is not None and not len(m):
            m = np.zeros(1, np.uint32)
        p = CcParams(int(n_samples), None if m is None else m.ctypes.data, 0 if m is None else len(m), int(threads))
        s = Summary()
        self._chk(self.L.vcfxg_concordance_region(self.h, data_start, int(mode), ctypes.byref(p), ctypes.byref(s)),
                  "concordance_region")
        t = np.zeros(4, np.uint64)
        self._chk(self.L.vcfxg_concordance_totals(self.h, t.ctypes.data), "concordance_totals")
        return s, tuple(int(x) for x in t), self.text(s.text_bytes)

    def dedup(self, mode, hash_bits=0):
        import numpy as np
        p = ctypes.c_uint32(int(hash_bits))
        s = Summary()
        self._chk(self.L.vcfxg_dedup(self.h, int(mode), ctypes.byref(p), ctypes.byref(s)), "dedup")
        st = np.zeros(max(int(s.n_lines), 1), np.uint8)
        self._chk(self.L.vcfxg_dedup_status(self.h, 0, s.n_lines, st.ctypes.data), "dedup_status")
        cnt = np.zeros(6, np.uint64)
        self._chk(self.L.vcfxg_dedup_counts(self.h, cnt.ctypes.data), "dedup_counts")
        return s, st[:s.n_lines], tuple(int(x) for x in cnt)

    def sort(self, mode, natural=False):
        import numpy as np
        p = ctypes.c_int(int(bool(natural)))
        s = Summary()
        self._chk(self.L.vcfxg_sort(self.h, int(mode), ctypes.byref(p), ctypes.byref(s)), "sort")
        st = np.zeros(max(int(s.n_lines), 1), np.uint8)
        self._chk(self.L.vcfxg_sort_status(self.h, 0, s.n_lines, st.ctypes.data), "sort_status")
        cnt = np.zeros(6, np.uint64)
        self._chk(self.L.vcfxg_sort_counts(self.h, cnt.ctypes.data), "sort_counts")
        order = np.zeros(max(int(s.rows), 1), np.uint32)
        self._chk(self.L.vcfxg_sort_order(self.h, 0, s.rows, order.ctypes.data), "sort_order")
        return s, st[:s.n_lines], tuple(int(x) for x in cnt), order[:s.rows]

    def sort_text(self, first):
        k, n = ctypes.c_uint64(), ctypes.c_uint64()
        self._chk(self.L.vcfxg_sort_text(self.h, int(first), ctypes.byref(k), ctypes.byref(n)), "sort_text")
        return k.value, self.text_range(0, n.value)

    def sorted_text(self, rows):
        out, j = [], 0
        while j < rows:
            k, text = self.sort_text(j)
            out.append(text)
            j += k
        return b"".join(out)

    def diff(self, second_start, assume_sorted=False, natural=False, hash_bits=0):
        import numpy as np
        p = DfParams(int(second_start), int(bool(assume_sorted)), int(bool(natural)), int(hash_bits))
        s = Summary()
        self._chk(self.L.vcfxg_diff(self.h, ctypes.byref(p), ctypes.byref(s)), "diff")
        st = np.zeros(max(int(s.n_lines), 1), np.uint8)
        self._chk(self.L.vcfxg_diff_status(self.h, 0, s.n_lines, st.ctypes.data), "diff_status")
        cnt = np.zeros(8, np.uint64)
        self._chk(self.L.vcfxg_diff_counts(self.h, cnt.ctypes.data), "diff_counts")
        return s, st[:s.n_lines], tuple(int(x) for x in cnt)

    def diff_text(self, side, first):
        k, n = ctypes.c_uint64(), ctypes.c_uint64()
        self._chk(self.L.vcfxg_diff_text(self.h, int(side), int(first), ctypes.byref(k), ctypes.byref(n)), "diff_text")
        return k.value, self.text_range(0, n.value)

    def diffed_text(self, side):
        cnt = (ctypes.c_uint64 * 8)()
        self._chk(self.L.vcfxg_diff_counts(self.h, ctypes.cast(cnt, ctypes.c_void_p)), "diff_counts")
        out, j = [], 0
        while j < cnt[int(side)]:
            k, text = self.diff_text(side, j)
            out.append(text)
            j += k
        return b"".join(out)

    def merge(self, file_starts, assume_sorted=False, natural=False):
        import numpy as np
        fs = np.ascontiguousarray(file_starts, np.uint64)
        p = MgParams(fs.ctypes.data, len(fs) - 1, int(bool(assume_sorted)), int(bool(natural)))
        s = Summary()
        self._chk(self.L.vcfxg_merge(self.h, ctypes.byref(p), ctypes.byref(s)), "merge")
        st = np.zeros(max(int(s.n_lines), 1), np.uint8)
        self._chk(self.L.vcfxg_merge_status(self.h, 0, s.n_lines, st.ctypes.data), "merge_status")
        cnt = np.zeros(8, np.uint64)
        self._chk(self.L.vcfxg_merge_counts(self.h, cnt.ctypes.data), "merge_counts")
        order = np.zeros(max(int(s.rows), 1), np.uint32)
        self._chk(self.L.vcfxg_merge_order(self.h, 0, s.rows, order.ctypes.data), "merge_order")
        return s, st[:s.n_lines], tuple(int(x) for x in cnt), order[:s.rows]

    def merge_files(self, n_files):
        import numpy as np
        first, bad = np.zeros(n_files + 1, np.uint64), np.zeros(max(n_files, 1), np.uint64)
        self._chk(self.L.vcfxg_merge_files(self.h, first.ctypes.data, bad.ctypes.data), "merge_files")
        return [int(x) for x in first], [int(x) for x in bad[:n_files]]

    def merge_text(self, first):
        k, n = ctypes.c_uint64(), ctypes.c_uint64()
        self._chk(self.L.vcfxg_merge_text(self.h, int(first), ctypes.byref(k), ctypes.byref(n)), "merge_text")
        return k.value, self.text_range(0, n.value)

    def merged_text(self, rows):
        out, j = [], 0
        while j < rows:
            k, text = self.merge_text(j)
            out.append(text)
            j += k
        return b"".join(out)

    def multiallelic_split(self, l0, l1, table, mode=MODE_FILE):
        import numpy as np
        ids = [bytes(t[0]) for t in table]
        ent = (MsEntry * max(len(ids), 1))()
        for e, i, t in zip(ent, ids, table):
            e.id, e.id_len, e.section, e.number = i, len(i), int(t[1]), int(t[2])
        p = MsParams(ctypes.cast(ent, ctypes.c_void_p) if ids else None, len(ids), int(mode))
        s = Summary()
        self._chk(self.L.vcfxg_multiallelic_split(self.h, l0, l1, ctypes.byref(p), ctypes.byref(s)),
                  "multiallelic_split")
        n = int(s.n_lines)
        st, alt, off = np.zeros(max(n, 1), np.uint8), np.zeros(max(n, 1), np.int32), np.zeros(n + 1, np.uint64)
        self._chk(self.L.vcfxg_fetch_lines(self.h, l0, n, alt.ctypes.data, None, st.ctypes.data), "fetch_lines")
        if n:
            self._chk(self.L.vcfxg_ms_line_ranges(self.h, l0, n, off.ctypes.data), "ms_line_ranges")
        return s, st[:n], alt[:n], off, self.text(s.text_bytes)

    def fasta_scan(self, l0, l1, n_samples, mode=MODE_FILE):
        import numpy as np
        s = Summary()
        self._chk(self.L.vcfxg_fasta_scan(self.h, l0, l1, int(mode), int(n_samples), ctypes.byref(s)), "fasta_scan")
        n = int(s.n_lines)
        st, col = np.zeros(max(n, 1), np.uint8), np.zeros(max(n, 1), np.uint64)
        if n:
            self._chk(self.L.vcfxg_fasta_status(self.h, l0, n, st.ctypes.data, col.ctypes.data), "fasta_status")
        return s, st[:n], col[:n]

    def fasta_begin(self, text_bytes):
        self._chk(self.L.vcfxg_fasta_begin(self.h, int(text_bytes)), "fasta_begin")

    def fasta(self, l0, l1, n_samples, first_col, total_cols, row_off, skip=None, mode=MODE_FILE):
        import numpy as np
        ro = np.ascontiguousarray(row_off, np.uint64)
        sk = None if skip is None else np.ascontiguousarray(skip, np.uint64)
        p = FaParams(int(mode), int(n_samples), int(first_col), int(total_cols), ro.ctypes.data,
                     None if sk is None else sk.ctypes.data)
        s = Summary()
        self._chk(self.L.vcfxg_fasta(self.h, l0, l1, ctypes.byref(p), ctypes.byref(s)), "fasta")
        return s

    def chrom_lines(self, data_start):
        import numpy as np
        n = ctypes.c_uint64(0)
        out = np.zeros(16, np.uint64)
        self._chk(self.L.vcfxg_chrom_lines(self.h, data_start, out.ctypes.data, len(out), ctypes.byref(n)), "chrom_lines")
        if n.value > len(out):
            out = np.zeros(n.value, np.uint64)
            self._chk(self.L.vcfxg_chrom_lines(self.h, data_start, out.ctypes.data, len(out), ctypes.byref(n)),
                      "chrom_lines")
        return out[:n.value]

    def haplotype_phaser(self, data_start, mode, threshold, n_samples):
        s = Summary()
        self._chk(self.L.vcfxg_haplotype_phaser(self.h, data_start, int(mode), float(threshold), int(n_samples),
                                                ctypes.byref(s)), "haplotype_phaser")
        return s

    def phaser_variants(self, n_var):
        import numpy as np
        f = np.zeros(max(n_var, 1), np.uint8)
        r2 = np.zeros(max(n_var, 1), np.float64)
        off = np.zeros(n_var + 1, np.uint64)
        self._chk(self.L.vcfxg_phaser_variants(self.h, f.ctypes.data, r2.ctypes.data, off.ctypes.data),
                  "phaser_variants")
        return f[:n_var], r2[:n_var], off

    def text_range(self, offset, n):
        b = ctypes.create_string_buffer(max(1, n))
        self._chk(self.L.vcfxg_fetch_text_range(self.h, offset, n, b), "fetch_text_range")
        return b.raw[:n]

    def hwe_rechecks(self):
        import numpy as np
        n = ctypes.c_uint64()
        self._chk(self.L.vcfxg_hwe_rechecks(self.h, None, 0, ctypes.byref(n)), "hwe_rechecks")
        a = np.zeros((max(n.value, 1), 3), np.uint64)
        self._chk(self.L.vcfxg_hwe_rechecks(self.h, a.ctypes.data, n.value, ctypes.byref(n)), "hwe_rechecks")
        v = a[:n.value].view(np.uint32).reshape(-1, 6)
        return [(int(r[0]) | (int(r[1]) << 32), int(r[2]), int(r[3]), int(r[4])) for r in v]

    def _criteria(self, crits):
        arr = (Criterion * max(1, len(crits)))()
        self._keep = []
        for i, (target, op, numeric, value, key, sval) in enumerate(crits):
            k = key.encode() if isinstance(key, str) else key
            s = sval.encode() if isinstance(sval, str) else sval
            self._keep += [k, s]
            arr[i] = Criterion(target, op, int(numeric), float(value), k, len(k), s, len(s))
        return arr

    def record_filter(self, crits, and_logic=True):
        s = Summary()
        arr = self._criteria(crits)
        self._chk(self.L.vcfxg_record_filter(self.h, ctypes.cast(arr, ctypes.c_void_p), len(crits), int(and_logic),
                                             ctypes.byref(s)), "record_filter")
        return s

    def filter_query(self, crits, query, and_logic=True, strict=False):
        s = Summary()
        arr = self._criteria(crits)
        q = query.encode() if isinstance(query, str) else query
        self._chk(self.L.vcfxg_filter_query(self.h, ctypes.cast(arr, ctypes.c_void_p), len(crits), int(and_logic), q,
# ... 163 lines not shown
```

Baseline: 576.9 million records/s.

## Size AF walk chunks to resident occupancy with tapered tail and XCD-contiguous ranges

Adds a walk layout planner that sizes per-walker chunks from occupancy-derived resident wave count. It uses larger main chunks with smaller tail chunks in a taper, so the final partial wave of walkers is balanced. It also assigns contiguous file ranges per XCD, meant to improve L2 locality on the multi-die GPU. The aim is to cut tail imbalance and launch overhead of many small walkers. In exchange the layout logic is more complex, and the per-walker output capacity grows with chunk size.

```diff
diff --git a/include/vcfx_gpu.h b/include/vcfx_gpu.h
--- a/include/vcfx_gpu.h
+++ b/include/vcfx_gpu.h
@@ -326,6 +326,7 @@
 int vcfxg_count_byte(vcfxg_ctx *ctx, uint64_t from, int byte, uint64_t *count);
 const char *vcfxg_last_schedule(const vcfxg_ctx *ctx);
 int vcfxg_last_af_depth(const vcfxg_ctx *ctx, int *rolling);
+int vcfxg_last_walk_layout(const vcfxg_ctx *ctx, int64_t out[8]);
 
 int vcfxg_fetch_text(vcfxg_ctx *ctx, char *host, size_t cap);
 int vcfxg_fetch_text_range(vcfxg_ctx *ctx, uint64_t offset, size_t n, void *host);
diff --git a/vcfx_amd/csrc/gpu/vcfxg_af_walk.hip b/vcfx_amd/csrc/gpu/vcfxg_af_walk.hip
--- a/vcfx_amd/csrc/gpu/vcfxg_af_walk.hip
+++ b/vcfx_amd/csrc/gpu/vcfxg_af_walk.hip
@@ -60,45 +60,45 @@
 
 int64_t af_walkers(int64_t lo, int64_t hi, int64_t chunk) { return hi > lo ? (hi - lo + chunk - 1) / chunk : 0; }
 
-hipError_t launch_af_walk(const char *buf, int64_t lo, int64_t hi, int64_t chunk, int mode, int64_t span0,
+int af_walk_waves_per_block() { return kWalkWaves; }
+
+typedef decltype(&k_af_walk<AfOp>) AfWalkKernel;
+static AfWalkKernel af_gt_only_kernel(int depth, bool roll) {
+    if (!roll) return depth == kWalkUnroll ? k_af_walk<AfOp> : nullptr;
+    return depth == 6 ? k_af_walk<AfOp, false, 6, true>
+         : depth == 8 ? k_af_walk<AfOp, false, 8, true>
+         : depth == 10 ? k_af_walk<AfOp, false, 10, true>
+         : depth == 12 ? k_af_walk<AfOp, false, 12, true>
+                       : nullptr;
+}
+
+int af_walk_resident_blocks(int depth, bool roll) {
+    const AfWalkKernel k = af_gt_only_kernel(depth, roll);
+    int blocks = 0;
+    if (!k || hipOccupancyMaxActiveBlocksPerMultiprocessor(&blocks, k, kWalkThreads, 0) != hipSuccess) return 0;
+    return blocks;
+}
+
+hipError_t launch_af_walk(const char *buf, int64_t lo, int64_t hi, const WalkLayout &lay, int mode, int64_t span0,
                           uint64_t cap_w, uint64_t *le_b, int32_t *alt_b, int32_t *tot_b, uint32_t *rowpre_b,
                           uint8_t *status_b, void *meta_b, uint64_t *wcount, uint32_t *wgt, unsigned *overflow,
                           hipStream_t s, int32_t *hwe_aux_b, const WalkTail *tail, bool dose, bool gt_first_walk,
                           bool dose_head, int depth, bool roll) {
     const WalkTail t = tail ? *tail : WalkTail{};
-    const int64_t nw = af_walkers(lo, hi, chunk);
-    if (!nw) return hipErrorInvalidValue;
+    if (!lay.nw || !lay.grid) return hipErrorInvalidValue;
     const bool af_gt_only = !gt_first_walk && !dose && !hwe_aux_b;
     if (roll ? !(af_gt_only && af_depth_compiled(depth)) : depth != kWalkUnroll) return hipErrorInvalidValue;
-    const unsigned grid = (unsigned)((nw + kWalkWaves - 1) / kWalkWaves);
-    if (gt_first_walk)
-        hipLaunchKernelGGL(HIP_KERNEL_NAME(k_af_walk<AfOp, true>), dim3(grid), dim3(kWalkThreads), 0, s, buf, lo, hi,
-                           chunk, nw, mode, span0, cap_w, le_b, alt_b, tot_b, nullptr, rowpre_b, status_b,
-                           static_cast<LineMeta *>(meta_b), wcount, wgt, overflow, t);
-    else if (dose && dose_head)
-        hipLaunchKernelGGL(k_af_walk<DoseHeadOp>, dim3(grid), dim3(kWalkThreads), 0, s, buf, lo, hi, chunk, nw, mode,
-                           span0, cap_w, le_b, alt_b, tot_b, nullptr, rowpre_b, status_b, static_cast<LineMeta *>(meta_b),
-                           wcount, wgt, overflow, t);
-    else if (dose)
-        hipLaunchKernelGGL(k_af_walk<DoseWalkOp>, dim3(grid), dim3(kWalkThreads), 0, s, buf, lo, hi, chunk, nw, mode,
-                           span0, cap_w, le_b, alt_b, tot_b, nullptr, rowpre_b, status_b, static_cast<LineMeta *>(meta_b),
-                           wcount, wgt, overflow, t);
-    else if (hwe_aux_b)
-        hipLaunchKernelGGL(k_af_walk<HweOp>, dim3(grid), dim3(kWalkThreads), 0, s, buf, lo, hi, chunk, nw, mode, span0,
-                           cap_w, le_b, alt_b, tot_b, hwe_aux_b, rowpre_b, status_b, static_cast<LineMeta *>(meta_b),
-                           wcount, wgt, overflow, t);
-    else {
-        auto go = [&](auto kernel) {
-            hipLaunchKernelGGL(kernel, dim3(grid), dim3(kWalkThreads), 0, s, buf, lo, hi, chunk, nw, mode, span0, cap_w,
-                               le_b, alt_b, tot_b, nullptr, rowpre_b, status_b, static_cast<LineMeta *>(meta_b), wcount,
-                               wgt, overflow, t);
-        };
-        if (!roll) go(k_af_walk<AfOp>);
-        else if (depth == 6) go(k_af_walk<AfOp, false, 6, true>);
-        else if (depth == 8) go(k_af_walk<AfOp, false, 8, true>);
-        else if (depth == 10) go(k_af_walk<AfOp, false, 10, true>);
-        else go(k_af_walk<AfOp, false, 12, true>);
-    }
+    if (!af_gt_only && lay.K1 != kWalkAllRounds) return hipErrorInvalidValue;
+    auto go = [&](auto kernel, int32_t *aux_b) {
+        hipLaunchKernelGGL(kernel, dim3(lay.grid), dim3(kWalkThreads), 0, s, buf, lo, hi, lay, mode, span0, cap_w, le_b,
+                           alt_b, tot_b, aux_b, rowpre_b, status_b, static_cast<LineMeta *>(meta_b), wcount, wgt,
+                           overflow, t);
+    };
+    if (gt_first_walk) go(k_af_walk<AfOp, true>, nullptr);
+    else if (dose && dose_head) go(k_af_walk<DoseHeadOp>, nullptr);
+    else if (dose) go(k_af_walk<DoseWalkOp>, nullptr);
+    else if (hwe_aux_b) go(k_af_walk<HweOp>, hwe_aux_b);
+    else go(af_gt_only_kernel(depth, roll), nullptr);
     return hipGetLastError();
 }
 
diff --git a/vcfx_amd/csrc/gpu/vcfxg_af_walk_kernel.h b/vcfx_amd/csrc/gpu/vcfxg_af_walk_kernel.h
--- a/vcfx_amd/csrc/gpu/vcfxg_af_walk_kernel.h
+++ b/vcfx_amd/csrc/gpu/vcfxg_af_walk_kernel.h
@@ -104,8 +104,7 @@
 #else
 __attribute__((amdgpu_waves_per_eu(af_walk_waves(kGF, kDepth))))
 #endif
-void k_af_walk(const char *__restrict__ buf, int64_t lo, int64_t hi, int64_t chunk, int64_t n_walkers, int mode,
-               int64_t span0, uint64_t cap_w, uint64_t *__restrict__ le_o, int32_t *__restrict__ alt_o,
+void k_af_walk(const char *__restrict__ buf, int64_t lo, int64_t hi, WalkLayout lay, int mode, int64_t span0, uint64_t cap_w, uint64_t *__restrict__ le_o, int32_t *__restrict__ alt_o,
                int32_t *__restrict__ tot_o, int32_t *__restrict__ aux_o, uint32_t *__restrict__ rowpre_o,
                uint8_t *__restrict__ status_o, LineMeta *__restrict__ meta_o, uint64_t *__restrict__ wcount,
                uint32_t *__restrict__ wgt, unsigned *overflow, WalkTail tail) {
@@ -120,13 +119,13 @@
     constexpr uint32_t kStgCap = kStageLds ? 2048u : 16u;
     __shared__ __attribute__((aligned(16))) char stg[kStageLds ? kWalkWaves : 1][kStgCap];
     const int wv = threadIdx.x / kWave;
-    const int64_t wk = uniform64((int64_t)walk_block() * kWalkWaves + wv);
-    if (wk >= n_walkers) return;
+    int64_t cs, ce, wsize;
+    const int64_t wk = walk_range(lay, blockIdx.x, gridDim.x, __builtin_amdgcn_readfirstlane(wv), kWalkWaves, hi,
+                                  VCFXG_WALK_XCD != 0, cs, ce, wsize);
+    if (wk >= lay.nw) return;
     const int strip_cr = mode == 0 ? 1 : 0;
-    const int64_t cs = lo + wk * chunk;
-    const int64_t ce = std::min<int64_t>(cs + chunk, hi);
     int64_t L, ce2;
-    walker_lines(buf, lo, hi, cs, ce, L, ce2, chunk);
+    walker_lines(buf, lo, hi, cs, ce, L, ce2, wsize);
     const int64_t L0 = L;
     uint64_t wtext = 0;
     int64_t span = span0;
diff --git a/vcfx_amd/csrc/gpu/vcfxg_api.hip b/vcfx_amd/csrc/gpu/vcfxg_api.hip
--- a/vcfx_amd/csrc/gpu/vcfxg_api.hip
+++ b/vcfx_amd/csrc/gpu/vcfxg_api.hip
@@ -575,6 +575,19 @@
     if (rolling) *rolling = c && c->last_af_roll ? 1 : 0;
     return c ? c->last_af_depth : 0;
 }
+int vcfxg_last_walk_layout(const vcfxg_ctx *c, int64_t out[8]) {
+    if (!c || !out) return 0;
+    const vcfxg::WalkLayout &l = c->last_walk_layout;
+    out[0] = l.C;
+    out[1] = l.Cs;
+    out[2] = l.K1 == vcfxg::kWalkAllRounds ? -1 : (int64_t)l.K1;
+    out[3] = l.grid;
+    out[4] = l.nw;
+    out[5] = c->last_walk_resident;
+    out[6] = c->last_walk_layout_kind.div;
+    out[7] = c->last_walk_layout_kind.g;
+    return c->last_walk_layout_kind.kind;
+}
 uint64_t vcfxg_bgzf_handed_over(const vcfxg_ctx *c) { return c ? c->bgz_handed : 0; }
 
 int vcfxg_fetch_text_range(vcfxg_ctx *c, uint64_t offset, size_t n, void *host) {
diff --git a/vcfx_amd/csrc/gpu/vcfxg_api_af.hip b/vcfx_amd/csrc/gpu/vcfxg_api_af.hip
--- a/vcfx_amd/csrc/gpu/vcfxg_api_af.hip
+++ b/vcfx_amd/csrc/gpu/vcfxg_api_af.hip
@@ -137,8 +137,8 @@
 static int af_region_walk(vcfxg_ctx *c, size_t data_start, int mode, vcfxg_summary *out, bool gf = false) {
     if (c) c->dense_pending = false;
     HIPCHK(c, hipSetDevice(c->device));
-    const WalkPlan pl = walk_plan(c, data_start);
-    const int64_t lo = pl.lo, hi = pl.hi, C = pl.C, nw = pl.nw;
+    const WalkPlan pl = walk_plan(c, data_start, 0, !gf);
+    const int64_t lo = pl.lo, hi = pl.hi, nw = pl.nw;
     if (!nw) {
         int r = vcfxg_index(c, data_start, nullptr);
         return r ? r : vcfxg_allele_freq(c, mode, out);
@@ -181,9 +181,12 @@
     tail.wdirty = P<uint8_t>(c->wk_dirty);
     const int depth = gf ? vcfxg::kAfDepthDefault : pl.af_depth;
     const bool roll = !gf && pl.af_roll;
-    if (!gf) c->last_af_depth = depth, c->last_af_roll = roll;
+    if (!gf) {
+        c->last_af_depth = depth, c->last_af_roll = roll;
+        c->last_walk_layout = pl.lay, c->last_walk_layout_kind = pl.lay_kind, c->last_walk_resident = pl.resident;
+    }
     prof_begin(c, "af_walk");
-    HIPCHK(c, vcfxg::launch_af_walk(buf, lo, hi, C, mode, c->hint_span, cap_w, P<uint64_t>(c->wk_le),
+    HIPCHK(c, vcfxg::launch_af_walk(buf, lo, hi, pl.lay, mode, c->hint_span, cap_w, P<uint64_t>(c->wk_le),
                                     P<int32_t>(c->wk_alt), P<int32_t>(c->wk_tot), P<uint32_t>(c->wk_rowpre),
                                     P<uint8_t>(c->wk_status), c->wk_meta.p, P<uint64_t>(c->wk_count),
                                     P<uint32_t>(c->wk_gt), ovf, c->stream, nullptr, &tail, false, gf, false, depth,
diff --git a/vcfx_amd/csrc/gpu/vcfxg_api_walk.hip b/vcfx_amd/csrc/gpu/vcfxg_api_walk.hip
--- a/vcfx_amd/csrc/gpu/vcfxg_api_walk.hip
+++ b/vcfx_amd/csrc/gpu/vcfxg_api_walk.hip
@@ -6,20 +6,56 @@
 
 namespace vcfxg {
 
-WalkPlan walk_plan(const vcfxg_ctx *c, size_t data_start, int64_t chunk) {
+static int64_t walk_resident(const vcfxg_ctx *c, int depth, bool roll) {
+    if (c->walk_resident_knob > 0) return c->walk_resident_knob;
+    if (depth < 0 || depth > kAfDepthMax) return 0;
+    int64_t &S = c->walk_resident[roll ? 1 : 0][depth];
+    if (!S) {
+        int cus = 0;
+        if (hipDeviceGetAttribute(&cus, hipDeviceAttributeMultiprocessorCount, c->device) != hipSuccess) cus = 0;
+        S = (int64_t)af_walk_resident_blocks(depth, roll) * cus * af_walk_waves_per_block();
+        if (S <= 0) S = -1;
+    }
+    return S > 0 ? S : 0;
+}
+
+static constexpr int64_t kAfMainChunk = 256 << 10;
+static constexpr WalkLayoutKnob kDefaultLayout = {kLayoutTaper, 2, 1};
+
+WalkPlan walk_plan(const vcfxg_ctx *c, size_t data_start, int64_t chunk, bool af_gt_only) {
     WalkPlan p;
     p.lo = (int64_t)data_start;
     p.hi = (int64_t)c->n;
-    p.C = chunk ? chunk : c->walk_chunk;
-    p.nw = af_walkers(p.lo, p.hi, p.C);
+    int64_t C0 = chunk ? chunk : c->walk_chunk;
+    int knob = c->af_depth_knob;
+    WalkLayoutKnob lk = c->walk_layout_knob;
+#if VCFXG_AF_DEPTH_LIVE
+    knob = getenv("VCFXG_AF_DEPTH") ? atoi(getenv("VCFXG_AF_DEPTH")) : 0;
+    lk = parse_walk_layout(getenv("VCFXG_WALK_LAYOUT"));
+    if (!chunk && getenv("VCFXG_WALK_CHUNK"))
+        C0 = std::min<int64_t>(std::max<int64_t>(atol(getenv("VCFXG_WALK_CHUNK")), 4096), 8 << 20);
+#endif
+    af_sweep_plan(c->hint_span, knob, p.af_depth, p.af_roll);
+    if (!af_gt_only) lk = WalkLayoutKnob{kLayoutUniform, 1, 0};
+    if (lk.kind == kLayoutDefault) {
+        const int64_t main = chunk || getenv("VCFXG_WALK_CHUNK") ? C0 : std::max(C0, kAfMainChunk);
+        const int64_t S = walk_resident(c, p.af_depth, p.af_roll);
+        if (S > 0 && (p.hi - p.lo + main - 1) / main >= S) {
+            lk = kDefaultLayout;
+            C0 = main;
+        } else {
+            lk = WalkLayoutKnob{kLayoutUniform, 1, 0};
+        }
+    }
+    p.resident = lk.kind == kLayoutFit || lk.kind == kLayoutTaper ? walk_resident(c, p.af_depth, p.af_roll) : 0;
+    p.lay_kind = lk;
+    p.lay = walk_layout_plan(p.lo, p.hi, C0, p.resident, lk, af_walk_waves_per_block(), VCFXG_WALK_XCD != 0,
+                             &p.lay_kind.kind);
+    p.C = p.lay.C;
+    p.nw = p.lay.nw;
     p.cap_w = (uint64_t)(2 * p.C / std::max<int64_t>(c->hint_line, 64)) + 16;
     p.cap = (uint64_t)p.nw * p.cap_w;
     p.fits_gt16 = p.cap_w <= 0xFFFF;
-    int knob = c->af_depth_knob;
-#if VCFXG_AF_DEPTH_LIVE
-    knob = getenv("VCFXG_AF_DEPTH") ? atoi(getenv("VCFXG_AF_DEPTH")) : 0;
-#endif
-    af_sweep_plan(c->hint_span, knob, p.af_depth, p.af_roll);
     return p;
 }
 
@@ -110,12 +146,12 @@
     HIPCHK(c, hipMemsetAsync(P<uint64_t>(c->wk_count) + p.nw, 0, 8, c->stream));
     prof_begin(c, prof_name);
     if (cc)
-        HIPCHK(c, launch_cc_walk(P<char>(c->input), p.lo, p.hi, p.C, mode, c->hint_span, p.cap_w, P<uint64_t>(c->wk_le),
+        HIPCHK(c, launch_cc_walk(P<char>(c->input), p.lo, p.hi, p.lay, mode, c->hint_span, p.cap_w, P<uint64_t>(c->wk_le),
                                  P<int32_t>(c->wk_alt), P<int32_t>(c->wk_tot), P<uint32_t>(c->wk_rowpre),
                                  P<uint8_t>(c->wk_status), c->wk_meta.p, P<uint64_t>(c->wk_count), P<uint32_t>(c->wk_gt),
                                  P<unsigned>(c->wk_small), c->stream));
     else
-        HIPCHK(c, launch_af_walk(P<char>(c->input), p.lo, p.hi, p.C, mode, c->hint_span, p.cap_w, P<uint64_t>(c->wk_le),
+        HIPCHK(c, launch_af_walk(P<char>(c->input), p.lo, p.hi, p.lay, mode, c->hint_span, p.cap_w, P<uint64_t>(c->wk_le),
                              P<int32_t>(c->wk_alt), P<int32_t>(c->wk_tot), P<uint32_t>(c->wk_rowpre),
                              P<uint8_t>(c->wk_status), c->wk_meta.p, P<uint64_t>(c->wk_count), P<uint32_t>(c->wk_gt),
                              P<unsigned>(c->wk_small), c->stream, aux ? P<int32_t>(c->wk_aux) : nullptr, nullptr, dose,
diff --git a/vcfx_amd/csrc/gpu/vcfxg_cc.hip b/vcfx_amd/csrc/gpu/vcfxg_cc.hip
--- a/vcfx_amd/csrc/gpu/vcfxg_cc.hip
+++ b/vcfx_amd/csrc/gpu/vcfxg_cc.hip
@@ -287,15 +287,14 @@
     return (unsigned)(g > cap ? cap : g);
 }
 
-hipError_t launch_cc_walk(const char *buf, int64_t lo, int64_t hi, int64_t chunk, int mode, int64_t span0,
+hipError_t launch_cc_walk(const char *buf, int64_t lo, int64_t hi, const WalkLayout &lay, int mode, int64_t span0,
                           uint64_t cap_w, uint64_t *le_b, int32_t *alt_b, int32_t *tot_b, uint32_t *rowpre_b,
                           uint8_t *status_b, void *meta_b, uint64_t *wcount, uint32_t *wgt, unsigned *overflow,
                           hipStream_t s) {
-    const int64_t nw = af_walkers(lo, hi, chunk);
-    if (!nw) return hipErrorInvalidValue;
-    hipLaunchKernelGGL(k_af_walk<CcOp>, dim3((unsigned)((nw + kWalkWaves - 1) / kWalkWaves)), dim3(kWalkThreads), 0, s,
-                       buf, lo, hi, chunk, nw, mode, span0, cap_w, le_b, alt_b, tot_b, nullptr, rowpre_b, status_b,
-                       static_cast<LineMeta *>(meta_b), wcount, wgt, overflow, WalkTail{});
+    if (!lay.nw || !lay.grid || lay.K1 != kWalkAllRounds) return hipErrorInvalidValue;
+    hipLaunchKernelGGL(k_af_walk<CcOp>, dim3(lay.grid), dim3(kWalkThreads), 0, s, buf, lo, hi, lay, mode, span0, cap_w,
+                       le_b, alt_b, tot_b, nullptr, rowpre_b, status_b, static_cast<LineMeta *>(meta_b), wcount, wgt,
+                       overflow, WalkTail{});
     return hipGetLastError();
 }
 
diff --git a/vcfx_amd/csrc/gpu/vcfxg_ctx.h b/vcfx_amd/csrc/gpu/vcfxg_ctx.h
--- a/vcfx_amd/csrc/gpu/vcfxg_ctx.h
+++ b/vcfx_amd/csrc/gpu/vcfxg_ctx.h
@@ -161,6 +161,12 @@
     int af_depth_knob = getenv("VCFXG_AF_DEPTH") ? atoi(getenv("VCFXG_AF_DEPTH")) : 0;
     int last_af_depth = 0;
     bool last_af_roll = false;
+    vcfxg::WalkLayoutKnob walk_layout_knob = vcfxg::parse_walk_layout(getenv("VCFXG_WALK_LAYOUT"));
+    mutable int64_t walk_resident[2][vcfxg::kAfDepthMax + 1] = {};
+    int64_t walk_resident_knob = getenv("VCFXG_WALK_RESIDENT") ? atoll(getenv("VCFXG_WALK_RESIDENT")) : 0;
+    vcfxg::WalkLayoutKnob last_walk_layout_kind;
+    vcfxg::WalkLayout last_walk_layout = {};
+    int64_t last_walk_resident = 0;
     int fq_path = getenv("VCFXG_FQ_WALK") ? atoi(getenv("VCFXG_FQ_WALK")) : 0;
     std::vector<uint8_t> ld_gflag_host;
     uint64_t ld_m = 0, ld_prefix_bytes = 0, ld_np = 0;
@@ -229,8 +235,11 @@
     bool fits_gt16;
     int af_depth;
     bool af_roll;
+    WalkLayout lay;
+    WalkLayoutKnob lay_kind;
+    int64_t resident;
 };
-WalkPlan walk_plan(const vcfxg_ctx *c, size_t data_start, int64_t chunk = 0);
+WalkPlan walk_plan(const vcfxg_ctx *c, size_t data_start, int64_t chunk = 0, bool af_gt_only = false);
 void af_sweep_plan(int64_t span, int knob, int &depth, bool &roll);
 bool walk_wanted(const vcfxg_ctx *c, bool need_gt_only);
 bool af_knob_allows_walk(const vcfxg_ctx *c);
diff --git a/vcfx_amd/csrc/gpu/vcfxg_kernels.h b/vcfx_amd/csrc/gpu/vcfxg_kernels.h
--- a/vcfx_amd/csrc/gpu/vcfxg_kernels.h
+++ b/vcfx_amd/csrc/gpu/vcfxg_kernels.h
@@ -1,6 +1,8 @@
 #pragma once
 #include <hip/hip_runtime.h>
 #include <stdint.h>
+
+#include "vcfxg_walk_layout.h"
 
 namespace vcfxg {
 
@@ -63,6 +65,8 @@
                                       hipStream_t s);
 int64_t idx_wchunk_bytes();
 int64_t af_walkers(int64_t lo, int64_t hi, int64_t chunk);
+int af_walk_waves_per_block();
+int af_walk_resident_blocks(int depth, bool roll);
 struct WalkTail {
     uint64_t *wtext = nullptr;
     uint64_t *wstart = nullptr;
@@ -76,13 +80,13 @@
 constexpr int kAfDepthDefault = 6, kAfDepthMax = 12;
 constexpr int kAfWaveStep = 1024;
 constexpr bool af_depth_compiled(int d) { return d == 6 || d == 8 || d == 10 || d == 12; }
-hipError_t launch_af_walk(const char *buf, int64_t lo, int64_t hi, int64_t chunk, int mode, int64_t span0,
+hipError_t launch_af_walk(const char *buf, int64_t lo, int64_t hi, const WalkLayout &lay, int mode, int64_t span0,
                           uint64_t cap_w, uint64_t *le_b, int32_t *alt_b, int32_t *tot_b, uint32_t *rowpre_b,
                           uint8_t *status_b, void *meta_b, uint64_t *wcount, uint32_t *wgt, unsigned *overflow,
                           hipStream_t s, int32_t *hwe_aux_b = nullptr, const WalkTail *tail = nullptr,
                           bool dose = false, bool gt_first_walk = false, bool dose_head = false,
                           int depth = kAfDepthDefault, bool roll = false);
-hipError_t launch_cc_walk(const char *buf, int64_t lo, int64_t hi, int64_t chunk, int mode, int64_t span0,
+hipError_t launch_cc_walk(const char *buf, int64_t lo, int64_t hi, const WalkLayout &lay, int mode, int64_t span0,
                           uint64_t cap_w, uint64_t *le_b, int32_t *alt_b, int32_t *tot_b, uint32_t *rowpre_b,
                           uint8_t *status_b, void *meta_b, uint64_t *wcount, uint32_t *wgt, unsigned *overflow,
                           hipStream_t s);
diff --git a/vcfx_amd/csrc/gpu/vcfxg_walk_layout.h b/vcfx_amd/csrc/gpu/vcfxg_walk_layout.h
--- /dev/null
+++ b/vcfx_amd/csrc/gpu/vcfxg_walk_layout.h
@@ -0,0 +1,147 @@
+#pragma once
+#include <algorithm>
+#include <cstdint>
+
+#if defined(__HIPCC__)
+#define VCFXG_LAYOUT_FN __host__ __device__ inline
+#else
+#define VCFXG_LAYOUT_FN inline
+#endif
+
+#ifndef VCFXG_WALK_XCD
+#define VCFXG_WALK_XCD 1
+#endif
+
+namespace vcfxg {
+
+constexpr uint32_t kWalkXcds = 8;
+constexpr uint32_t kWalkAllRounds = 0xFFFFFFFFu;
+
+struct WalkLayout {
+    int64_t base[kWalkXcds];
+    int64_t C, Cs;
+    int64_t nw;
+    uint32_t K1, grid;
+};
+
+VCFXG_LAYOUT_FN uint32_t walk_xcd_blocks(uint32_t n, uint32_t x) { return n / kWalkXcds + (x < n % kWalkXcds ? 1u : 0u); }
+VCFXG_LAYOUT_FN uint32_t walk_file_block(uint32_t b, uint32_t n) {
+    const uint32_t q = n / kWalkXcds, r = n % kWalkXcds, x = b % kWalkXcds, k = b / kWalkXcds;
+    return (x < r ? x * (q + 1) : r * (q + 1) + (x - r) * q) + k;
+}
+VCFXG_LAYOUT_FN int64_t walk_run_bytes(const WalkLayout &l, uint32_t rounds, int waves) {
+    const uint32_t full = rounds < l.K1 ? rounds : l.K1;
+    return (int64_t)waves * ((int64_t)full * l.C + (int64_t)(rounds - full) * l.Cs);
+}
+VCFXG_LAYOUT_FN int64_t walk_range(const WalkLayout &l, uint32_t b, uint32_t n, int wv, int waves, int64_t hi, bool xcd,
+                                   int64_t &cs, int64_t &ce, int64_t &size) {
+    const uint32_t x = xcd ? b % kWalkXcds : 0u, k = xcd ? b / kWalkXcds : b;
+    const uint32_t fb = xcd ? walk_file_block(b, n) : b;
+    size = k < l.K1 ? l.C : l.Cs;
+    cs = l.base[x] + walk_run_bytes(l, k, waves) + (int64_t)wv * size;
+    if (cs > hi) cs = hi;
+    ce = cs + size < hi ? cs + size : hi;
+    return (int64_t)fb * waves + wv;
+}
+
+inline WalkLayout walk_layout_make(int64_t lo, int64_t hi, int64_t C, int64_t Cs, uint32_t K1, int waves, bool xcd) {
+    WalkLayout l{};
+    l.C = C;
+    l.Cs = Cs;
+    l.K1 = K1;
+    const int64_t R = hi > lo ? hi - lo : 0, FB = (int64_t)waves * C, SB = (int64_t)waves * Cs;
+    const int64_t nfull = (int64_t)K1 * kWalkXcds;
+    const int64_t fullcap = xcd ? nfull : (int64_t)K1;
+    int64_t blocks;
+    if (R <= 0) blocks = 0;
+    else if ((R + FB - 1) / FB <= fullcap) blocks = (R + FB - 1) / FB;
+    else blocks = fullcap + (R - fullcap * FB + SB - 1) / SB;
+    l.grid = (uint32_t)blocks;
+    int64_t at = lo;
+    for (uint32_t x = 0; x < kWalkXcds; x++) {
+        l.base[x] = at;
+        at += walk_run_bytes(l, xcd ? walk_xcd_blocks(l.grid, x) : (x == 0 ? l.grid : 0u), waves);
+    }
+    l.nw = 0;
+    if (blocks) {
+        const uint32_t xl = !xcd ? 0u : l.grid < kWalkXcds ? l.grid - 1 : kWalkXcds - 1;
+        const uint32_t kl = (xcd ? walk_xcd_blocks(l.grid, xl) : l.grid) - 1;
+        const int64_t size = kl < K1 ? C : Cs, off = l.base[xl] + walk_run_bytes(l, kl, waves);
+        int64_t own = (hi - off + size - 1) / size;
+        if (own > waves) own = waves;
+        l.nw = (blocks - 1) * waves + own;
+    }
+    return l;
+}
+
+enum : int { kLayoutDefault = 0, kLayoutUniform, kLayoutFit, kLayoutTaper, kLayoutSplit };
+struct WalkLayoutKnob {
+    int kind = kLayoutDefault;
+    int div = 1;
+    int64_t g = 0;
+};
+
+inline WalkLayoutKnob parse_walk_layout(const char *e) {
+    WalkLayoutKnob k;
+    if (!e) return k;
+    auto is = [&](const char *w) {
+        size_t i = 0;
+        while (w[i] && e[i] == w[i]) i++;
+        return !w[i] && (!e[i] || e[i] == ':');
+    };
+    auto nums = [&](int64_t &a, int64_t &b) {
+        const char *p = e;
+        while (*p && *p != ':') p++;
+        int64_t v[2] = {-1, -1};
+        for (int i = 0; i < 2 && *p == ':'; i++) {
+            p++;
+            if (*p < '0' || *p > '9') return false;
+            v[i] = 0;
+            while (*p >= '0' && *p <= '9' && v[i] < (1ll << 40)) v[i] = v[i] * 10 + (*p++ - '0');
+        }
+        a = v[0];
+        b = v[1];
+        return !*p && a >= 0 && b >= 0;
+    };
+    int64_t a = 0, b = 0;
+    if (is("uniform") && !e[7]) k.kind = kLayoutUniform;
+    else if (is("fit") && !e[3]) k.kind = kLayoutFit;
+    else if ((is("taper") || is("split")) && nums(a, b) && a >= 1 && a <= 64 && b <= 0x7FFFFFFF) {
+        k.kind = is("taper") ? kLayoutTaper : kLayoutSplit;
+        k.div = (int)a;
+        k.g = b;
+    }
+    return k;
+}
+
+inline WalkLayout walk_layout_plan(int64_t lo, int64_t hi, int64_t C0, int64_t S, WalkLayoutKnob knob, int waves,
+                                   bool xcd, int *kind = nullptr) {
+    const int64_t R = hi > lo ? hi - lo : 0;
+    int got = kLayoutUniform;
+    WalkLayout l = walk_layout_make(lo, hi, C0, C0, kWalkAllRounds, waves, xcd);
+    if (knob.kind == kLayoutSplit) {
+        const int64_t Cs = std::max<int64_t>(C0 / knob.div & ~(int64_t)15, 16);
+        l = walk_layout_make(lo, hi, C0, Cs, (uint32_t)knob.g, waves, xcd);
+        got = kLayoutSplit;
+    } else if ((knob.kind == kLayoutFit || knob.kind == kLayoutTaper) && S >= waves && R > 0) {
+        const int64_t G = l.nw / S;
+        if (G >= 1) {
+            const int64_t div = knob.kind == kLayoutTaper ? knob.div : 1, unit = 16 * div;
+            int64_t C = (R + G * S - 1) / (G * S);
+            C = (std::max(C, C0) + unit - 1) / unit * unit;
+            const int64_t g = knob.kind == kLayoutTaper ? std::min<int64_t>(knob.g, G) : 0;
+            if (g > 0 && div > 1) {
+                const int64_t rounds = (G - g) * (S / waves) / (xcd ? (int64_t)kWalkXcds : 1);
+                l = walk_layout_make(lo, hi, C, C / div, (uint32_t)std::min<int64_t>(rounds, kWalkAllRounds - 1), waves, xcd);
+                got = kLayoutTaper;
+            } else {
+                l = walk_layout_make(lo, hi, C, C, kWalkAllRounds, waves, xcd);
+                got = kLayoutFit;
+            }
+        }
+    }
+    if (kind) *kind = got;
+    return l;
+}
+
+}
diff --git a/vcfx_amd/engine.py b/vcfx_amd/engine.py
--- a/vcfx_amd/engine.py
+++ b/vcfx_amd/engine.py
@@ -147,6 +147,7 @@
     "vcfxg_comm_rccl_stats": (_I, [_VP, ctypes.POINTER(_U64), ctypes.POINTER(_U64)]),
     "vcfxg_last_schedule": (_P, [_VP]),
     "vcfxg_last_af_depth": (_I, [_VP, ctypes.POINTER(_I)]),
+    "vcfxg_last_walk_layout": (_I, [_VP, ctypes.POINTER(ctypes.c_int64)]),
     "vcfxg_bgzf_handed_over": (_U64, [_VP]),
     "vcfxg_count_byte": (_I, [_VP, _U64, _I, ctypes.POINTER(_U64)]),
     "vcfxg_haplotype_phaser": (_I, [_VP, _S, _I, ctypes.c_double, ctypes.c_uint32, ctypes.POINTER(Summary)]),
@@ -303,6 +304,13 @@
         r = ctypes.c_int()
         d = self.L.vcfxg_last_af_depth(self.h, ctypes.byref(r))
         return d, bool(r.value)
+
+    def last_walk_layout(self):
+        out = (ctypes.c_int64 * 8)()
+        kind = self.L.vcfxg_last_walk_layout(self.h, out)
+        d = dict(zip(("C", "Cs", "K1", "grid", "walkers", "resident", "div", "g"), [int(v) for v in out]))
+        d["kind"] = (None, "uniform", "fit", "taper", "split")[kind]
+        return d
 
     def genotype_query(self, query, strict=False, strip_cr=False):
         q = query.encode() if isinstance(query, str) else query
```

After: 603.9 million records/s, median of 6. 4.7% higher.
